# frosinastojanovska/image-captioning

Hardware: AMD Instinct MI355X
Metric: captions/sec (train step) on 1024px x 32RoI x 15tok synth (higher is better)
Workload: dtype f32 (split-bf16x3 products, fp32 accumulate: 73 of 85 conv layers on the bf16 pipe, the rest and the decoder exact fp32 MFMA); 1 GPU; BASELINE configs[2] (configs[3] at 8 GPUs): frozen ResNet-101+FPN fwd + PyramidROIAlign + RoI head + v2-inject decoder fwd/bwd + AMSGrad, 1024x1024 synth images, 32 RoI/img, 15-token captions, V=10000; backbone=resnet101, images_per_gpu=2, global_batch_images=2, parallelism=dp1, stage4_blocks=22, pipeline=encoder(i+1) || decoder(i), 2 HIP streams, rccl_ranks=1

## Files before the change

### image-captioning_amd/_lib.py

```python
import ctypes as C
import os

_HERE = os.path.dirname(os.path.abspath(__file__))
LIB_PATH = os.path.join(_HERE, "csrc", "libdcap_hip.so")

c_float_p = C.POINTER(C.c_float)
c_int32_p = C.POINTER(C.c_int32)
c_uint8_p = C.POINTER(C.c_uint8)


class GemmDesc(C.Structure):
    _fields_ = [("M", C.c_int), ("N", C.c_int), ("K", C.c_int),
                ("A", C.c_void_p), ("lda", C.c_int), ("a_trans", C.c_int),
                ("a_gather", C.c_void_p),
                ("B", C.c_void_p), ("ldb", C.c_int), ("b_trans", C.c_int),
                ("C", C.c_void_p), ("ldc", C.c_int),
                ("scale", C.c_void_p), ("shift", C.c_void_p),
                ("residual", C.c_void_p), ("ldr", C.c_int), ("res_rows", C.c_int),
                ("relu", C.c_int), ("accumulate", C.c_int), ("split_k", C.c_int)]


class GemmBf16Desc(C.Structure):
    _fields_ = [("M", C.c_int), ("N", C.c_int), ("K", C.c_int),
                ("A", C.c_void_p), ("lda", C.c_int), ("a_trans", C.c_int),
                ("a_gather", C.c_void_p), ("a_gather_rows", C.c_int),
                ("B", C.c_void_p), ("ldb", C.c_int), ("b_trans", C.c_int),
                ("C", C.c_void_p), ("ldc", C.c_int),
                ("Cb", C.c_void_p), ("ldcb", C.c_int),
                ("scale", C.c_void_p), ("shift", C.c_void_p),
                ("residual", C.c_void_p), ("ldr", C.c_int), ("res_rows", C.c_int),
                ("relu", C.c_int), ("accumulate", C.c_int), ("split_k", C.c_int)]


class ConvDesc(C.Structure):
    _fields_ = [("N", C.c_int), ("H", C.c_int), ("W", C.c_int), ("Cin", C.c_int),
                ("Cout", C.c_int), ("kh", C.c_int), ("kw", C.c_int), ("stride", C.c_int),
                ("pad_t", C.c_int), ("pad_l", C.c_int), ("Ho", C.c_int), ("Wo", C.c_int),
                ("x", C.c_void_p), ("w", C.c_void_p), ("y", C.c_void_p),
                ("scale", C.c_void_p), ("shift", C.c_void_p),
                ("residual", C.c_void_p), ("res_mode", C.c_int),
                ("relu", C.c_int), ("split_k", C.c_int), ("accumulate", C.c_int), ("math", C.c_int), ("w_wino", C.c_void_p), ("w_wino_b3", C.c_void_p)]


class ConvWgradBf16Desc(C.Structure):
    _fields_ = [("N", C.c_int), ("H", C.c_int), ("W", C.c_int), ("Cin", C.c_int),
                ("Cout", C.c_int), ("kh", C.c_int), ("kw", C.c_int), ("stride", C.c_int),
                ("pad_t", C.c_int), ("pad_l", C.c_int), ("Ho", C.c_int), ("Wo", C.c_int),
                ("x", C.c_void_p), ("dy", C.c_void_p), ("dw", C.c_void_p), ("accumulate", C.c_int), ("split_k", C.c_int)]


class ConvBf16Desc(C.Structure):
    _fields_ = [("N", C.c_int), ("H", C.c_int), ("W", C.c_int), ("Cin", C.c_int),
                ("Cout", C.c_int), ("kh", C.c_int), ("kw", C.c_int), ("stride", C.c_int),
                ("pad_t", C.c_int), ("pad_l", C.c_int), ("Ho", C.c_int), ("Wo", C.c_int),
                ("x", C.c_void_p), ("w", C.c_void_p), ("y", C.c_void_p), ("y_bf16", C.c_void_p),
                ("scale", C.c_void_p), ("shift", C.c_void_p), ("residual", C.c_void_p), ("res_mode", C.c_int),
                ("relu", C.c_int), ("split_k", C.c_int), ("tile", C.c_int)]


MATH_F32, MATH_BF16X3, MATH_BF16X2, MATH_BF16 = 0, 1, 2, 3


class RoiAlignDesc(C.Structure):
    _fields_ = [("B", C.c_int), ("R", C.c_int), ("C", C.c_int), ("pool", C.c_int),
                ("maps", C.c_void_p * 4), ("Hs", C.c_int * 4), ("Ws", C.c_int * 4),
                ("boxes", C.c_void_p), ("image_area", C.c_float),
                ("out", C.c_void_p), ("levels_out", C.c_void_p)]


class LstmFwdDesc(C.Structure):
    _fields_ = [("B", C.c_int), ("T", C.c_int), ("U", C.c_int),
                ("z", C.c_void_p), ("U_rec", C.c_void_p), ("mask", C.c_void_p),
                ("h_seq", C.c_void_p), ("c_seq", C.c_void_p), ("rec_masks", C.c_void_p)]


class LstmBwdDesc(C.Structure):
    _fields_ = [("B", C.c_int), ("T", C.c_int), ("U", C.c_int),
                ("z", C.c_void_p), ("U_rec", C.c_void_p), ("mask", C.c_void_p),
                ("h_seq", C.c_void_p), ("c_seq", C.c_void_p),
                ("dh_seq", C.c_void_p), ("dh_last", C.c_void_p),
                ("dz", C.c_void_p), ("dU_rec", C.c_void_p), ("accumulate_dU", C.c_int), ("rec_masks", C.c_void_p)]


class SoftmaxCeDesc(C.Structure):
    _fields_ = [("M", C.c_int), ("V", C.c_int), ("ld", C.c_int),
                ("logits", C.c_void_p), ("targets", C.c_void_p),
                ("probs", C.c_void_p), ("loss_rows", C.c_void_p), ("dlogits", C.c_void_p),
                ("grad_scale", C.c_float), ("row_weights", C.c_void_p), ("keras_sparse", C.c_int)]


class VocabCeDesc(C.Structure):
    _fields_ = [("M", C.c_int), ("V", C.c_int), ("K", C.c_int), ("bf16", C.c_int),
                ("X", C.c_void_p), ("ldx", C.c_int), ("W", C.c_void_p), ("ldw", C.c_int),
                ("bias", C.c_void_p), ("targets", C.c_void_p), ("row_weights", C.c_void_p),
                ("grad_scale", C.c_float), ("keras_sparse", C.c_int), ("loss_rows", C.c_void_p),
                ("dlogits", C.c_void_p), ("lddl", C.c_int), ("dl_bf16", C.c_int), ("dbias", C.c_void_p), ("materialize_bf16", C.c_int)]


class VocabTop1Desc(C.Structure):
    _fields_ = [("M", C.c_int), ("V", C.c_int), ("K", C.c_int),
                ("X", C.c_void_p), ("ldx", C.c_int), ("W", C.c_void_p), ("ldw", C.c_int),
                ("bias", C.c_void_p), ("tokens", C.c_void_p),
                ("ids", C.c_void_p), ("ld_ids", C.c_int), ("probs", C.c_void_p), ("ld_probs", C.c_int), ("mask", C.c_void_p)]


class VocabTopkDesc(C.Structure):
    _fields_ = [("M", C.c_int), ("V", C.c_int), ("K", C.c_int), ("k", C.c_int),
                ("X", C.c_void_p), ("ldx", C.c_int), ("W", C.c_void_p), ("ldw", C.c_int),
                ("bias", C.c_void_p), ("ids", C.c_void_p), ("probs", C.c_void_p)]


class VocabTop1Bf16Desc(C.Structure):
    _fields_ = VocabTop1Desc._fields_ + [("tile", C.c_int)]


class VocabTopkBf16Desc(C.Structure):
    _fields_ = VocabTopkDesc._fields_ + [("tile", C.c_int)]


class BeamSelectDesc(C.Structure):
    _fields_ = [("R", C.c_int), ("k", C.c_int), ("nb", C.c_int), ("steps", C.c_int), ("j", C.c_int), ("log_score", C.c_int),
                ("cand_ids", C.c_void_p), ("cand_probs", C.c_void_p), ("scores_in", C.c_void_p), ("scores_out", C.c_void_p),
                ("parents", C.c_void_p), ("tokens_hist", C.c_void_p), ("tokens", C.c_void_p), ("mask", C.c_void_p),
                ("U", C.c_int), ("h_in", C.c_void_p), ("c_in", C.c_void_p), ("h_out", C.c_void_p), ("c_out", C.c_void_p)]


class LstmStepDesc(C.Structure):
    _fields_ = [("B", C.c_int), ("U", C.c_int),
                ("z", C.c_void_p), ("U_rec", C.c_void_p), ("U_packed", C.c_void_p),
                ("h_prev", C.c_void_p), ("c_prev", C.c_void_p), ("mask", C.c_void_p), ("h", C.c_void_p), ("c", C.c_void_p)]


class BnReluDesc(C.Structure):
    _fields_ = [("M", C.c_int), ("N", C.c_int), ("ld", C.c_int), ("acc", C.c_void_p),
                ("bias", C.c_void_p), ("gamma", C.c_void_p), ("beta", C.c_void_p), ("mean", C.c_void_p), ("var", C.c_void_p),
                ("eps", C.c_float), ("y", C.c_void_p), ("dy", C.c_void_p), ("dacc", C.c_void_p),
                ("dgamma", C.c_void_p), ("dbeta", C.c_void_p), ("dbias", C.c_void_p)]


class ProposalDesc(C.Structure):
    _fields_ = [("B", C.c_int), ("levels", C.c_int), ("anchors_per_loc", C.c_int),
                ("heads", C.c_void_p * 5), ("Hs", C.c_int * 5), ("Ws", C.c_int * 5), ("head_stride", C.c_int),
                ("anchors", C.c_void_p), ("A_total", C.c_int), ("std_dev", C.c_float * 4),
                ("image_h", C.c_float), ("image_w", C.c_float),
                ("pre_nms_limit", C.c_int), ("proposal_count", C.c_int), ("nms_threshold", C.c_float),
                ("proposals", C.c_void_p), ("scores_out", C.c_void_p), ("order_out", C.c_void_p), ("keep_out", C.c_void_p)]


class RpnLossDesc(C.Structure):
    _fields_ = [("levels", C.c_int), ("anchors_per_loc", C.c_int), ("head_stride", C.c_int),
                ("heads", C.c_void_p * 5), ("dheads", C.c_void_p * 5), ("Hs", C.c_int * 5), ("Ws", C.c_int * 5),
                ("n_sel", C.c_int), ("n_pos", C.c_int),
                ("sel_level", C.c_void_p), ("sel_index", C.c_void_p), ("sel_match", C.c_void_p),
                ("target_deltas", C.c_void_p), ("losses", C.c_void_p), ("counts_dev", C.c_void_p)]


class DetectionTargetsDesc(C.Structure):
    _fields_ = [("n_proposals", C.c_int), ("n_gt", C.c_int), ("n_rois", C.c_int), ("T", C.c_int),
                ("proposals", C.c_void_p), ("gt_boxes", C.c_void_p), ("gt_captions", C.c_void_p),
                ("max_positive", C.c_int), ("inv_ratio", C.c_float), ("shuffle", C.c_int),
                ("seed", C.c_uint32), ("offset", C.c_uint32), ("offset_dev", C.c_void_p),
                ("rois", C.c_void_p), ("captions", C.c_void_p), ("counts", C.c_void_p)]


class PwChainDesc(C.Structure):
    _fields_ = [("M", C.c_int), ("K1", C.c_int), ("N1", C.c_int), ("N2", C.c_int),
                ("x", C.c_void_p), ("w1", C.c_void_p), ("scale1", C.c_void_p), ("shift1", C.c_void_p), ("residual", C.c_void_p),
                ("relu1", C.c_int), ("y", C.c_void_p), ("w2", C.c_void_p), ("scale2", C.c_void_p), ("shift2", C.c_void_p),
                ("relu2", C.c_int), ("z", C.c_void_p), ("w1_b3", C.c_void_p), ("w2_b3", C.c_void_p)]


class RegSegments(C.Structure):
    _fields_ = [("start", C.c_void_p), ("coef", C.c_void_p), ("mask", C.c_void_p), ("nseg", C.c_int)]


class AmsgradDesc(C.Structure):
    _fields_ = [("n", C.c_size_t), ("p", C.c_void_p), ("g", C.c_void_p), ("m", C.c_void_p),
                ("v", C.c_void_p), ("vhat", C.c_void_p),
                ("lr_t", C.c_float), ("beta1", C.c_float), ("beta2", C.c_float), ("eps", C.c_float),
                ("grad_scale", C.c_float), ("gnorm_sq", C.c_void_p), ("clipnorm", C.c_float),
                ("p_bf16", C.c_void_p), ("n_bf16", C.c_size_t), ("lr_t_dev", C.c_void_p), ("reg", C.POINTER(RegSegments))]


SYMBOLS = {
    "dc_version": (C.c_int, []),
    "dc_last_error": (C.c_char_p, []),
    "dc_gemm_workspace_bytes": (C.c_size_t, [C.POINTER(GemmDesc)]),
    "dc_gemm_f32": (C.c_int, [C.POINTER(GemmDesc), C.c_void_p, C.c_size_t, C.c_void_p]),
    "dc_gemm_bf16_workspace_bytes": (C.c_size_t, [C.POINTER(GemmBf16Desc)]),
    "dc_gemm_bf16_tile": (C.c_int, [C.POINTER(GemmBf16Desc), C.POINTER(C.c_int)]),
    "dc_gemm_bf16": (C.c_int, [C.POINTER(GemmBf16Desc), C.c_void_p, C.c_size_t, C.c_void_p]),
    "dc_conv2d_wgrad_bf16_workspace_bytes": (C.c_size_t, [C.POINTER(ConvWgradBf16Desc)]),
    "dc_conv2d_wgrad_bf16_tile": (C.c_int, [C.POINTER(ConvWgradBf16Desc), C.POINTER(C.c_int)]),
    "dc_conv2d_wgrad_bf16": (C.c_int, [C.POINTER(ConvWgradBf16Desc), C.c_void_p, C.c_size_t, C.c_void_p]),
    "dc_conv2d_bf16_workspace_bytes": (C.c_size_t, [C.POINTER(ConvBf16Desc)]),
    "dc_conv2d_bf16_tile": (C.c_int, [C.POINTER(ConvBf16Desc), C.POINTER(C.c_int)]),
    "dc_conv2d_bf16": (C.c_int, [C.POINTER(ConvBf16Desc), C.c_void_p, C.c_size_t, C.c_void_p]),
    "dc_cast_f32_bf16": (C.c_int, [C.c_void_p, C.c_void_p, C.c_size_t, C.c_void_p]),
    "dc_cast_bf16_f32": (C.c_int, [C.c_void_p, C.c_void_p, C.c_size_t, C.c_void_p]),
    "dc_cast_f32_bf16_2d": (C.c_int, [C.c_void_p, C.c_int, C.c_void_p, C.c_int, C.c_int, C.c_int, C.c_int, C.c_void_p]),
    "dc_split_bf16x3_f32": (C.c_int, [C.c_void_p, C.c_void_p, C.c_size_t, C.c_void_p]),
    "dc_conv2d_workspace_bytes": (C.c_size_t, [C.POINTER(ConvDesc)]),
    "dc_conv2d_nhwc_f32": (C.c_int, [C.POINTER(ConvDesc), C.c_void_p, C.c_size_t, C.c_void_p]),
    "dc_conv2d_tile_config": (C.c_int, [C.POINTER(ConvDesc), C.POINTER(C.c_int), C.POINTER(C.c_int), C.POINTER(C.c_int)]),
    "dc_conv2d_is_pointwise": (C.c_int, [C.POINTER(ConvDesc)]),
    "dc_conv2d_winograd_weight_bytes": (C.c_size_t, [C.c_int, C.c_int]),
    "dc_conv2d_winograd_pack_f32": (C.c_int, [C.c_void_p, C.c_void_p, C.c_int, C.c_int, C.c_void_p]),
    "dc_pw_chain_supported": (C.c_int, [C.c_int, C.c_int, C.c_int]),
    "dc_pw_chain_pack_f32": (C.c_int, [C.c_void_p, C.c_void_p, C.c_int, C.c_int, C.c_void_p]),
    "dc_pw_chain_pack_b3": (C.c_int, [C.c_void_p, C.c_void_p, C.c_int, C.c_int, C.c_void_p]),
    "dc_pw_chain_f32": (C.c_int, [C.POINTER(PwChainDesc), C.c_void_p]),
    "dc_pw_chain_kernel_name": (C.c_int, [C.POINTER(PwChainDesc), C.c_char_p, C.c_size_t]),
    "dc_conv2d_winograd_b3_weight_bytes": (C.c_size_t, [C.c_int, C.c_int]),
    "dc_conv2d_winograd_pack_b3": (C.c_int, [C.c_void_p, C.c_void_p, C.c_int, C.c_int, C.c_void_p]),
    "dc_conv2d_kernel_name": (C.c_int, [C.POINTER(ConvDesc), C.c_char_p, C.c_size_t]),
    "dc_conv2d_wgrad_workspace_bytes": (C.c_size_t, [C.POINTER(ConvDesc)]),
    "dc_conv2d_wgrad_f32": (C.c_int, [C.POINTER(ConvDesc), C.c_void_p, C.c_size_t, C.c_void_p]),
    "dc_roi_align_pyramid_bwd_f32": (C.c_int, [C.POINTER(RoiAlignDesc), C.c_void_p]),
    "dc_downsample2x_sum_f32": (C.c_int, [C.c_void_p, C.c_void_p, C.c_int, C.c_int, C.c_int, C.c_int, C.c_int, C.c_void_p]),
    "dc_downsample2x_sum_dual_f32": (C.c_int, [C.c_void_p, C.c_void_p, C.c_void_p, C.c_int, C.c_int, C.c_int, C.c_int, C.c_int, C.c_void_p]),
    "dc_maxpool2x2s2_f32": (C.c_int, [C.c_void_p, C.c_void_p, C.c_int, C.c_int, C.c_int, C.c_int, C.c_void_p]),
    "dc_maxpool3x3s2_same_f32": (C.c_int, [C.c_void_p, C.c_void_p, C.c_int, C.c_int, C.c_int, C.c_int, C.c_void_p]),
    "dc_mold_image_padded_f32": (C.c_int, [C.c_void_p, C.c_void_p, C.c_int, C.c_int, C.c_int, C.c_int, C.c_float, C.c_float, C.c_float, C.c_void_p]),
    "dc_mold_image_rgbx_f32": (C.c_int, [C.c_void_p, C.c_void_p, C.c_int, C.c_int, C.c_int,
                                         C.c_float, C.c_float, C.c_float, C.c_void_p]),
    "dc_roi_align_pyramid_f32": (C.c_int, [C.POINTER(RoiAlignDesc), C.c_void_p]),
    "dc_subsample2_f32": (C.c_int, [C.c_void_p, C.c_void_p, C.c_int, C.c_int, C.c_int, C.c_int, C.c_void_p]),
    "dc_proposals_workspace_bytes": (C.c_size_t, [C.POINTER(ProposalDesc)]),
    "dc_proposals_f32": (C.c_int, [C.POINTER(ProposalDesc), C.c_void_p, C.c_size_t, C.c_void_p]),
    "dc_lstm_seq_workspace_bytes": (C.c_size_t, [C.c_int, C.c_int, C.c_int]),
    "dc_lstm_seq_fwd_f32": (C.c_int, [C.POINTER(LstmFwdDesc), C.c_void_p, C.c_size_t, C.c_void_p]),
    "dc_lstm_seq_bwd_f32": (C.c_int, [C.POINTER(LstmBwdDesc), C.c_void_p, C.c_size_t, C.c_void_p]),
    "dc_lstm_pack_urec_f32": (C.c_int, [C.c_void_p, C.c_int, C.c_void_p, C.c_void_p]),
    "dc_lstm_step_workspace_bytes": (C.c_size_t, [C.c_int, C.c_int]),
    "dc_lstm_step_f32": (C.c_int, [C.POINTER(LstmStepDesc), C.c_void_p, C.c_size_t, C.c_void_p]),
    "dc_softmax_ce_f32": (C.c_int, [C.POINTER(SoftmaxCeDesc), C.c_void_p]),
    "dc_vocab_ce_workspace_bytes": (C.c_size_t, [C.POINTER(VocabCeDesc)]),
    "dc_vocab_ce": (C.c_int, [C.POINTER(VocabCeDesc), C.c_void_p, C.c_size_t, C.c_void_p]),
    "dc_vocab_top1_workspace_bytes": (C.c_size_t, [C.c_int, C.c_int]),
    "dc_vocab_top1_f32": (C.c_int, [C.POINTER(VocabTop1Desc), C.c_void_p, C.c_size_t, C.c_void_p]),
    "dc_vocab_topk_workspace_bytes": (C.c_size_t, [C.c_int, C.c_int, C.c_int]),
    "dc_vocab_topk_f32": (C.c_int, [C.POINTER(VocabTopkDesc), C.c_void_p, C.c_size_t, C.c_void_p]),
    "dc_vocab_topk_bf16_tile": (C.c_int, [C.c_int, C.c_int, C.c_int]),
    "dc_vocab_top1_bf16_workspace_bytes": (C.c_size_t, [C.c_int, C.c_int, C.c_int, C.c_int]),
    "dc_vocab_topk_bf16_workspace_bytes": (C.c_size_t, [C.c_int, C.c_int, C.c_int, C.c_int, C.c_int]),
    "dc_vocab_top1_bf16": (C.c_int, [C.POINTER(VocabTop1Bf16Desc), C.c_void_p, C.c_size_t, C.c_void_p]),
    "dc_vocab_topk_bf16": (C.c_int, [C.POINTER(VocabTopkBf16Desc), C.c_void_p, C.c_size_t, C.c_void_p]),
    "dc_beam_select_f32": (C.c_int, [C.POINTER(BeamSelectDesc), C.c_void_p]),
    "dc_beam_backtrace": (C.c_int, [C.c_void_p, C.c_void_p, C.c_int, C.c_int, C.c_int, C.c_void_p, C.c_void_p]),
    "dc_argmax_rows_f32": (C.c_int, [C.c_void_p, C.c_int, C.c_int, C.c_int, C.c_void_p, C.c_void_p]),
    "dc_gather_rows_f32": (C.c_int, [C.c_void_p, C.c_int, C.c_void_p, C.c_void_p, C.c_int, C.c_int, C.c_int, C.c_void_p]),
    "dc_bn_relu_fwd_f32": (C.c_int, [C.POINTER(BnReluDesc), C.c_void_p]),
    "dc_bn_relu_bwd_f32": (C.c_int, [C.POINTER(BnReluDesc), C.c_void_p]),
    "dc_conv_weight_dgrad_pack_f32": (C.c_int, [C.c_void_p, C.c_void_p, C.c_int, C.c_int, C.c_int, C.c_int, C.c_void_p]),
    "dc_rpn_loss_grad_f32": (C.c_int, [C.POINTER(RpnLossDesc), C.c_void_p]),
    "dc_scatter2_add_f32": (C.c_int, [C.c_void_p, C.c_void_p, C.c_int, C.c_int, C.c_int, C.c_int, C.c_void_p]),
    "dc_detection_targets_f32": (C.c_int, [C.POINTER(DetectionTargetsDesc), C.c_void_p]),
    "dc_caption_tables_i32": (C.c_int, [C.c_void_p, C.c_int, C.c_int, C.c_void_p, C.c_void_p, C.c_void_p, C.c_void_p, C.c_void_p, C.c_void_p]),
    "dc_set_persistent_cus": (C.c_int, [C.c_int]),
    "dc_get_persistent_cus": (C.c_int, []),
    "dc_l2_reg_workspace_bytes": (C.c_size_t, [C.c_size_t]),
    "dc_l2_reg_f32": (C.c_int, [C.c_void_p, C.c_void_p, C.c_void_p, C.c_void_p, C.c_size_t, C.c_void_p, C.c_void_p, C.c_size_t, C.c_void_p]),
    "dc_axpy_f32": (C.c_int, [C.c_float, C.c_void_p, C.c_void_p, C.c_size_t, C.c_void_p]),
    "dc_relu_bwd_f32": (C.c_int, [C.c_void_p, C.c_void_p, C.c_void_p, C.c_int, C.c_int, C.c_int, C.c_void_p]),
    "dc_relu_bwd_dual_f32": (C.c_int, [C.c_void_p, C.c_void_p, C.c_void_p, C.c_void_p, C.c_size_t, C.c_void_p]),
    "dc_fold_time_f32": (C.c_int, [C.c_void_p, C.c_int, C.c_int, C.c_int, C.c_int, C.c_void_p, C.c_int, C.c_void_p]),
    "dc_colsum_workspace_bytes": (C.c_size_t, [C.c_int, C.c_int, C.c_int]),
    "dc_colsum_f32": (C.c_int, [C.c_void_p, C.c_int, C.c_int, C.c_int, C.c_void_p, C.c_int, C.c_void_p, C.c_size_t, C.c_void_p]),
    "dc_sumsq_workspace_bytes": (C.c_size_t, [C.c_size_t]),
    "dc_sumsq_f32": (C.c_int, [C.c_void_p, C.c_size_t, C.c_void_p, C.c_int, C.c_void_p, C.c_size_t, C.c_void_p]),
    "dc_mean_f32": (C.c_int, [C.c_void_p, C.c_size_t, C.c_void_p, C.c_void_p]),
    "dc_bn_fold_f32": (C.c_int, [C.c_void_p] * 5 + [C.c_float, C.c_void_p, C.c_void_p, C.c_int, C.c_void_p]),
    "dc_bn_bwd_f32": (C.c_int, [C.c_void_p] * 8 + [C.c_long, C.c_int, C.c_void_p]),
    "dc_mul_f32": (C.c_int, [C.c_void_p, C.c_void_p, C.c_void_p, C.c_size_t, C.c_void_p]),
    "dc_maxpool3x3s2_same_bwd_f32": (C.c_int, [C.c_void_p] * 4 + [C.c_int] * 4 + [C.c_void_p]),
    "dc_dropout_mask_f32": (C.c_int, [C.c_void_p, C.c_size_t, C.c_float, C.c_uint32, C.c_uint32, C.c_void_p, C.c_void_p]),
    "dc_amsgrad_step_f32": (C.c_int, [C.POINTER(AmsgradDesc), C.c_void_p]),
    "dc_zero_fill": (C.c_int, [C.c_void_p, C.c_size_t, C.c_void_p]),
    "dc_reg_sumsq_workspace_bytes": (C.c_size_t, [C.c_size_t]),
    "dc_reg_sumsq_f32": (C.c_int, [C.c_void_p, C.c_void_p, C.POINTER(RegSegments), C.c_size_t, C.c_void_p, C.c_void_p, C.c_void_p, C.c_size_t, C.c_void_p]),
}

ABI_VERSION = 600
_lib = None


class DcapError(RuntimeError):
    pass


def load():
    global _lib
    if _lib is not None:
        return _lib
    path = os.environ.get("DCAP_LIB", LIB_PATH)
    if not os.path.exists(path):
        raise DcapError("%s is missing: build it with `python __graft_entry__.py` "
                        "(hipcc --offload-arch=gfx950); there is no CPU fallback" % path)
    import torch
    lib = C.CDLL(path)
    for name, (res, args) in SYMBOLS.items():
        fn = getattr(lib, name)
        fn.restype = res
        fn.argtypes = args
    got = lib.dc_version()
    if got // 100 != ABI_VERSION // 100:
        raise DcapError("%s is ABI version %d, these bindings are for %d: rebuild it (python __graft_entry__.py)" % (path, got, ABI_VERSION))
    _lib = lib
    return lib


def check(rc, what):
    if rc != 0:
        msg = load().dc_last_error()
        raise DcapError("%s failed (code %d): %s" % (what, rc, msg.decode() if msg else ""))
```

### image-captioning_amd/csrc/conv_wino.hip

```cpp
#include "igemm_bf16s.h"
#include <algorithm>

namespace dcap {
namespace wino {

constexpr int NTHREADS = 256;

struct Args {
    const float* x;
    const f4* u;
    float* y;
    const float* scale;
    const float* shift;
    int N, H, W, Cin, Cout, relu;
    int gy, gx, groups;
    unsigned x_bytes, u_bytes;
};

__global__ void wino_pack_kernel(const float* __restrict__ w, float* __restrict__ u, int Cin, int Cout) {
    const long total = (long)Cin * Cout;
    const int NTG = Cout / 32, KC = Cin / 16;
    for (long idx = (long)blockIdx.x * blockDim.x + threadIdx.x; idx < total; idx += (long)gridDim.x * blockDim.x) {
        const int cin = (int)(idx % Cin), cout = (int)(idx / Cin);
        float g[3][3];
#pragma unroll
        for (int t = 0; t < 9; ++t) g[t / 3][t % 3] = w[((long)cout * 9 + t) * Cin + cin];
        float gg[4][3];
#pragma unroll
        for (int c = 0; c < 3; ++c) {
            gg[0][c] = g[0][c];
            gg[1][c] = 0.5f * (g[0][c] + g[1][c] + g[2][c]);
            gg[2][c] = 0.5f * (g[0][c] - g[1][c] + g[2][c]);
            gg[3][c] = g[2][c];
        }
        const int ntg = cout >> 5, i = cout & 31, kc = cin >> 4, kk = cin & 15, h = kk >> 3, j = (kk & 7) >> 2, e = kk & 3;
#pragma unroll
        for (int a = 0; a < 4; ++a) {
            const float r[4] = {gg[a][0], 0.5f * (gg[a][0] + gg[a][1] + gg[a][2]), 0.5f * (gg[a][0] - gg[a][1] + gg[a][2]), gg[a][2]};
#pragma unroll
            for (int b = 0; b < 4; ++b) {
                const int xi = 4 * a + b;
                u[((((long)(xi * NTG + ntg) * KC + kc) * 2 + j) * 64 + (h * 32 + i)) * 4 + e] = r[b];
            }
        }
    }
}

__global__ void wino_pack_b3_kernel(const float* __restrict__ w, unsigned short* __restrict__ u, int Cin, int Cout) {
    const long total = (long)Cin * Cout;
    const int NTG = Cout / 32, KC = Cin / 16;
    for (long idx = (long)blockIdx.x * blockDim.x + threadIdx.x; idx < total; idx += (long)gridDim.x * blockDim.x) {
        const int cin = (int)(idx % Cin), cout = (int)(idx / Cin);
        float g[3][3];
#pragma unroll
        for (int t = 0; t < 9; ++t) g[t / 3][t % 3] = w[((long)cout * 9 + t) * Cin + cin];
        float gg[4][3];
#pragma unroll
        for (int c = 0; c < 3; ++c) {
            gg[0][c] = g[0][c];
            gg[1][c] = 0.5f * (g[0][c] + g[1][c] + g[2][c]);
            gg[2][c] = 0.5f * (g[0][c] - g[1][c] + g[2][c]);
            gg[3][c] = g[2][c];
        }
        const int ntg = cout >> 5, i = cout & 31, kc = cin >> 4, kk = cin & 15, h = kk >> 3, jj = kk & 7;
#pragma unroll
        for (int a = 0; a < 4; ++a) {
            const float r[4] = {gg[a][0], 0.5f * (gg[a][0] + gg[a][1] + gg[a][2]), 0.5f * (gg[a][0] - gg[a][1] + gg[a][2]), gg[a][2]};
#pragma unroll
            for (int b = 0; b < 4; ++b) {
                const int xi = 4 * a + b;
                float x = r[b];
#pragma unroll
                for (int piece = 0; piece < 3; ++piece) {
                    const unsigned short pb = __builtin_bit_cast(unsigned short, (__bf16)x);
                    x -= __uint_as_float((unsigned)pb << 16);
                    u[((((long)(xi * NTG + ntg) * KC + kc) * 3 + piece) * 64 + (h * 32 + i)) * 8 + jj] = pb;
                }
            }
        }
    }
}

__device__ __forceinline__ unsigned img32_addr(int xi, int tile, int chunk) {
    return (unsigned)((((xi * 32 + tile) << 3) + (chunk ^ ((tile >> 1) & 7))) << 4);
}
__device__ __forceinline__ void bt_cols(const f4 (&t)[4], f4 (&v)[4]) {
    v[0] = t[0] - t[2];
    v[1] = t[1] + t[2];
    v[2] = t[2] - t[1];
    v[3] = t[1] - t[3];
}

namespace wp {
constexpr int PW = 18, NDMA = 6;
__device__ __forceinline__ int patch_index(int y, int x) { return y * PW + (x >> 1) + (PW / 2) * (x & 1); }
__device__ __forceinline__ int patch_swizzle(int y, int x) { return ((x >> 2) & 1) | (((y >> 1) & 3) << 1); }
template <int HALVES>
struct Cfg {
    static constexpr int NT = 256 * HALVES, TGY = 4 * HALVES, TGX = 8, PH = 2 * TGY + 2, NPIX = PH * PW, SLOTS = NPIX * 8;
    static constexpr int BUF = 32768 * HALVES;
    static constexpr int LDS_BYTES = 2 * BUF;
    static_assert(NDMA * NT >= SLOTS && NDMA * NT * 16 <= BUF, "patch buffer; the kernel issues the pieces three per step");
};
}

typedef unsigned u32x4 __attribute__((ext_vector_type(4)));

__device__ __forceinline__ void split8(const f4& va, const f4& vb, u32x4& p0, u32x4& p1, u32x4& p2) {
    unsigned a0, a1, a2, b0, b1, b2, c0, c1, c2, d0, d1, d2;
    split_pair(va[0], va[1], a0, a1, a2);
    split_pair(va[2], va[3], b0, b1, b2);
    split_pair(vb[0], vb[1], c0, c1, c2);
    split_pair(vb[2], vb[3], d0, d1, d2);
    p0 = u32x4{a0, b0, c0, d0};
    p1 = u32x4{a1, b1, c1, d1};
    p2 = u32x4{a2, b2, c2, d2};
}
__device__ __forceinline__ f32x16 mfma_b(const u32x4& a, const u32x4& b, const f32x16& c) {
    return __builtin_amdgcn_mfma_f32_32x32x16_bf16(__builtin_bit_cast(bf16x8, a), __builtin_bit_cast(bf16x8, b), c, 0, 0, 0);
}

template <int HALVES, bool B3, int NCH = 1>
__device__ __forceinline__ void wino_body(const Args& a) {
    static_assert(NCH == 1 || (NCH == 2 && HALVES == 1 && B3), "64-channel items: the split-bf16 32-tile kernel only");
    using namespace wp;
    typedef Cfg<HALVES> C;
    constexpr int NT64 = C::NT, SLOTS = C::SLOTS, BUF = C::BUF;
    extern __shared__ __attribute__((aligned(16))) char smem[];
    const int tid = threadIdx.x, lane = tid & 63;
    const int wave = __builtin_amdgcn_readfirstlane(tid >> 6);
    const int wa = wave & 3, th = wave >> 2;
    const int gpi = a.gy * a.gx;
    const int NTG = a.Cout >> 5, KC = a.Cin >> 4, KP = a.Cin >> 5;
    const int total = a.groups * (NTG / NCH);
    const __amdgpu_buffer_rsrc_t rsrc = __builtin_amdgcn_make_buffer_rsrc(const_cast<float*>(a.x), 0, (int)a.x_bytes, 0x00020000);

    int nb, img, gyi, gxi;
    unsigned doff[NDMA];
    const f4* ubase;
    unsigned ubyte3;
    auto setup = [&](int item) {
        const int bid = xcd_remap(item, total);
        nb = bid / a.groups;
        const int g = bid - nb * a.groups;
        img = g / gpi;
        const int gr = g - img * gpi;
        gyi = gr / a.gx;
        gxi = gr - gyi * a.gx;
#pragma unroll
        for (int n = 0; n < NDMA; ++n) {
            const int s = n * NT64 + tid, pq = s >> 3, py = pq / PW, rem = pq - py * PW;
            const int px = rem < PW / 2 ? 2 * rem : 2 * (rem - PW / 2) + 1;
            const int iy = gyi * 2 * C::TGY - 1 + py, ix = gxi * 2 * C::TGX - 1 + px;
            const bool in = s < SLOTS && (unsigned)iy < (unsigned)a.H && (unsigned)ix < (unsigned)a.W;
            const int c8 = (s & 7) ^ patch_swizzle(py, px);
            doff[n] = in ? (unsigned)(((((long)img * a.H + iy) * a.W + ix) * a.Cin + 4 * c8) * 4) : kOobOffset;
        }
        ubase = a.u + lane + (((long)(4 * wa) * NTG + nb) * KC << 7);
        ubyte3 = (unsigned)((4 * wa) * NTG + NCH * nb) * (unsigned)KC * 3072u;
    };
    auto issue_dma_pieces = [&](int pair, int buf, int n0, int n1) {
#pragma unroll
        for (int n = n0; n < n1; ++n)
            __builtin_amdgcn_raw_ptr_buffer_load_lds(rsrc, (__attribute__((address_space(3))) void*)(smem + buf * BUF + (n * NT64 + wave * 64) * 16), 16,
                                                     (int)doff[n], pair * 128, 0, 0);
    };
    auto issue_dma = [&](int pair, int buf) { issue_dma_pieces(pair, buf, 0, NDMA); };
    const long ustep = (long)NTG * KC << 7;
    auto load_u_part = [&](f4 (&dst)[4][2], int kc, int b0, int b1) {
#pragma unroll
        for (int b = b0; b < b1; ++b) {
            const f4* p = ubase + b * ustep + ((long)kc << 7);
            dst[b][0] = p[0];
            dst[b][1] = p[64];
        }
    };
    auto load_u = [&](f4 (&dst)[4][2], int kc) { load_u_part(dst, kc, 0, 4); };
    const __amdgpu_buffer_rsrc_t rsrc_u = __builtin_amdgcn_make_buffer_rsrc(const_cast<f4*>(a.u), 0, (int)a.u_bytes, 0x00020000);
    const unsigned ustep3 = (unsigned)NTG * KC * 3 * 1024u;
    auto load_u3 = [&](u32x4 (&dst)[3], int kc, int b, int hc) {
        const unsigned so = __builtin_amdgcn_readfirstlane(ubyte3 + (unsigned)b * ustep3 + (unsigned)(hc * KC + kc) * 3072u);
        dst[0] = __builtin_bit_cast(u32x4, buf_f4s(rsrc_u, (unsigned)lane * 16u, so));
        dst[1] = __builtin_bit_cast(u32x4, buf_f4s(rsrc_u, (unsigned)lane * 16u, so + 1024u));
        dst[2] = __builtin_bit_cast(u32x4, buf_f4s(rsrc_u, (unsigned)lane * 16u, so + 2048u));
    };

    const int fi = lane & 31, fh = lane >> 5;
    const int tile = 32 * th + fi, tyl = tile >> 3, txl = tile & 7;
    const int r1 = (wa == 0) ? 0 : (wa == 2 ? 2 : 1), r2 = (wa == 0 || wa == 1) ? 2 : (wa == 2 ? 1 : 3);
    const float sgn = (wa == 1) ? 1.f : -1.f;
    unsigned paddr[2][4];
#pragma unroll
    for (int rr = 0; rr < 2; ++rr)
#pragma unroll
        for (int c = 0; c < 4; ++c) {
            const int py = 2 * tyl + (rr ? r2 : r1), px = 2 * txl + c;
            paddr[rr][c] = (unsigned)(patch_index(py, px) * 128 + (((2 * fh) ^ patch_swizzle(py, px)) << 4));
        }
    auto read_d = [&](f4 (&d)[2][4], int st) {
        const unsigned k = (unsigned)(((st & 1) << 4) ^ ((st >> 1) << 6));
#pragma unroll
        for (int rr = 0; rr < 2; ++rr)
#pragma unroll
            for (int c = 0; c < 4; ++c) d[rr][c] = *reinterpret_cast<const f4*>(smem + (paddr[rr][c] ^ k));
    };
    auto transform = [&](const f4 (&d)[2][4], f4 (&v)[4]) {
        f4 t[4];
#pragma unroll
        for (int c = 0; c < 4; ++c) t[c] = d[1][c] * sgn + d[0][c];
        bt_cols(t, v);
    };

    int item = blockIdx.x;
    if (item >= total) return;
    setup(item);
    issue_dma(0, 0);
    f4 ub[2][4][2];
    u32x4 u3[4][3];
    u32x4 w0[2][2], w1[2], w2[2];
    auto load_piece = [&](u32x4& dst, int kc, int b, int hc, int piece) {
        const unsigned so = __builtin_amdgcn_readfirstlane(ubyte3 + (unsigned)b * ustep3 + (unsigned)(hc * KC + kc) * 3072u + (unsigned)piece * 1024u);
        dst = __builtin_bit_cast(u32x4, buf_f4s(rsrc_u, (unsigned)lane * 16u, so));
    };
    auto load_u3_first = [&]() {
        if constexpr (NCH == 2) {
#pragma unroll
            for (int hc = 0; hc < 2; ++hc) {
                load_piece(w0[0][hc], 0, 0, hc, 0);
                load_piece(w1[hc], 0, 0, hc, 1);
                load_piece(w2[hc], 0, 0, hc, 2);
                load_piece(w0[1][hc], 0, 1, hc, 0);
            }
        } else {
#pragma unroll
            for (int b = 0; b < 4; ++b) load_u3(u3[b], 0, b, 0);
        }
    };
    if constexpr (B3) {
        load_u3_first();
    } else {
        load_u(ub[0], 0);
    }
    for (;;) {
        f32x16 acc[NCH][4];
#pragma unroll
        for (int hc = 0; hc < NCH; ++hc)
#pragma unroll
            for (int b = 0; b < 4; ++b)
#pragma unroll
                for (int r = 0; r < 16; ++r) acc[hc][b][r] = 0.f;
        auto pair = [&](int p, auto more_c) {
            constexpr bool more = decltype(more_c)::value;
            asm volatile("s_waitcnt vmcnt(0)" ::: "memory");
            __syncthreads();
            if constexpr (B3 && NCH == 2) {
                f4 t0[4], t1[4];
                u32x4 V[2][3];
                auto fetch_col = [&](int hf, int c) {
                    const unsigned ka = (unsigned)(hf << 6), kb = ka ^ 16u;
                    const f4 a0 = *reinterpret_cast<const f4*>(smem + (paddr[0][c] ^ ka));
                    const f4 a1 = *reinterpret_cast<const f4*>(smem + (paddr[1][c] ^ ka));
                    const f4 b0 = *reinterpret_cast<const f4*>(smem + (paddr[0][c] ^ kb));
                    const f4 b1 = *reinterpret_cast<const f4*>(smem + (paddr[1][c] ^ kb));
                    t0[c] = a1 * sgn + a0;
                    t1[c] = b1 * sgn + b0;
                };
                auto prep = [&](u32x4 (&dst)[3], int b) {
                    const f4 va = b == 0 ? t0[0] - t0[2] : (b == 1 ? t0[1] + t0[2] : (b == 2 ? t0[2] - t0[1] : t0[1] - t0[3]));
                    const f4 vb = b == 0 ? t1[0] - t1[2] : (b == 1 ? t1[1] + t1[2] : (b == 2 ? t1[2] - t1[1] : t1[1] - t1[3]));
                    split8(va, vb, dst[0], dst[1], dst[2]);
                };
                fetch_col(0, 0);
                fetch_col(0, 2);
                prep(V[0], 0);
#pragma unroll
                for (int q = 0; q < 8; ++q) {
                    const int b = q & 3;
                    __builtin_amdgcn_sched_barrier(0);
                    if constexpr (more) if (q < NDMA) issue_dma_pieces(p + 1, (p + 1) & 1, q, q + 1);
                    const u32x4 (&vq)[3] = V[q & 1];
                    const int kc1 = min(2 * p + ((q + 1) >> 2), KC - 1), kc2 = min(2 * p + ((q + 2) >> 2), KC - 1);
#pragma unroll
                    for (int hc = 0; hc < 2; ++hc) acc[hc][b] = mfma_b(w0[q & 1][hc], vq[2], acc[hc][b]);
#pragma unroll
                    for (int hc = 0; hc < 2; ++hc) acc[hc][b] = mfma_b(w1[hc], vq[1], acc[hc][b]);
#pragma unroll
                    for (int hc = 0; hc < 2; ++hc) acc[hc][b] = mfma_b(w2[hc], vq[0], acc[hc][b]);
#pragma unroll
                    for (int hc = 0; hc < 2; ++hc) load_piece(w2[hc], kc1, (q + 1) & 3, hc, 2);
#pragma unroll
                    for (int hc = 0; hc < 2; ++hc) acc[hc][b] = mfma_b(w1[hc], vq[0], acc[hc][b]);
#pragma unroll
                    for (int hc = 0; hc < 2; ++hc) load_piece(w1[hc], kc1, (q + 1) & 3, hc, 1);
#pragma unroll
                    for (int hc = 0; hc < 2; ++hc) acc[hc][b] = mfma_b(w0[q & 1][hc], vq[1], acc[hc][b]);
#pragma unroll
                    for (int hc = 0; hc < 2; ++hc) acc[hc][b] = mfma_b(w0[q & 1][hc], vq[0], acc[hc][b]);
#pragma unroll
                    for (int hc = 0; hc < 2; ++hc) load_piece(w0[q & 1][hc], kc2, (q + 2) & 3, hc, 0);
                    if (q == 0) fetch_col(0, 1);
                    if (q == 1) { fetch_col(0, 3); fetch_col(1, 0); }
                    if (q == 2) fetch_col(1, 2);
                    if (q == 3) fetch_col(1, 1);
                    if (q == 4) fetch_col(1, 3);
                    if (q < 7) prep(V[(q + 1) & 1], (q + 1) & 3);
#pragma unroll
                    for (int m = 0; m < 12; ++m) {
                        __builtin_amdgcn_sched_group_barrier(0x008, 1, 0);
                        __builtin_amdgcn_sched_group_barrier(0x020, 1, 0);
                        __builtin_amdgcn_sched_group_barrier(0x002, 6, 0);
                    }
                    __builtin_amdgcn_sched_barrier(0);
                }
#pragma unroll
                for (int rr = 0; rr < 2; ++rr)
#pragma unroll
                    for (int c = 0; c < 4; ++c) paddr[rr][c] ^= (unsigned)BUF;
                return;
            } else if constexpr (B3) {
                f4 dA[2][4], dB[2][4], t0[4], t1[4];
                u32x4 V[2][3];
                auto make_t = [&]() {
#pragma unroll
                    for (int c = 0; c < 4; ++c) {
                        t0[c] = dA[1][c] * sgn + dA[0][c];
                        t1[c] = dB[1][c] * sgn + dB[0][c];
                    }
                };
                auto prep = [&](u32x4 (&dst)[3], int b) {
                    const f4 va = b == 0 ? t0[0] - t0[2] : (b == 1 ? t0[1] + t0[2] : (b == 2 ? t0[2] - t0[1] : t0[1] - t0[3]));
                    const f4 vb = b == 0 ? t1[0] - t1[2] : (b == 1 ? t1[1] + t1[2] : (b == 2 ? t1[2] - t1[1] : t1[1] - t1[3]));
                    split8(va, vb, dst[0], dst[1], dst[2]);
                };
                read_d(dA, 0);
                read_d(dB, 1);
                make_t();
                prep(V[0], 0);
#pragma unroll
                for (int q = 0; q < 8; ++q) {
                    const int half = q >> 2, b = q & 3;
                    if (q == 1) read_d(dA, 2);
                    if (q == 2) read_d(dB, 3);
                    __builtin_amdgcn_sched_barrier(0);
                    if constexpr (more) if (q < NDMA) issue_dma_pieces(p + 1, (p + 1) & 1, q, q + 1);
                    const u32x4 (&vq)[3] = V[q & 1];
                    acc[0][b] = mfma_b(u3[b][0], vq[2], acc[0][b]);
                    acc[0][b] = mfma_b(u3[b][1], vq[1], acc[0][b]);
                    acc[0][b] = mfma_b(u3[b][2], vq[0], acc[0][b]);
                    acc[0][b] = mfma_b(u3[b][1], vq[0], acc[0][b]);
                    acc[0][b] = mfma_b(u3[b][0], vq[1], acc[0][b]);
                    acc[0][b] = mfma_b(u3[b][0], vq[0], acc[0][b]);
                    if (q == 3) make_t();
                    if (q < 7) prep(V[(q + 1) & 1], (q + 1) & 3);
                    load_u3(u3[b], min(2 * p + half + 1, KC - 1), b, 0);
#pragma unroll
                    for (int m = 0; m < 6; ++m) {
                        __builtin_amdgcn_sched_group_barrier(0x008, 1, 0);
                        __builtin_amdgcn_sched_group_barrier(0x020, 1, 0);
                        if (q == 3) __builtin_amdgcn_sched_group_barrier(0x002, 15, 0);
                        else __builtin_amdgcn_sched_group_barrier(0x002, 9, 0);
                    }
                    __builtin_amdgcn_sched_barrier(0);
                }
#pragma unroll
                for (int rr = 0; rr < 2; ++rr)
#pragma unroll
                    for (int c = 0; c < 4; ++c) paddr[rr][c] ^= (unsigned)BUF;
                return;
            }
            f4 d[2][4], vcur[4], vnext[4];
            read_d(d, 0);
            transform(d, vcur);
#pragma unroll
            for (int st = 0; st < 4; ++st) {
                const int half = st >> 1, j = st & 1;
                if (st < 3) read_d(d, st + 1);
                __builtin_amdgcn_sched_barrier(0);
                if constexpr (more) if (st < 2) issue_dma_pieces(p + 1, (p + 1) & 1, 3 * st, 3 * st + 3);
                load_u_part(ub[half ^ 1], min(2 * p + half + 1, KC - 1), 2 * j, 2 * j + 2);
#pragma unroll
                for (int e = 0; e < 2; ++e)
#pragma unroll
                    for (int b = 0; b < 4; ++b) acc[0][b] = __builtin_amdgcn_mfma_f32_32x32x2f32(ub[half][b][j][e], vcur[b][e], acc[0][b], 0, 0, 0);
#pragma unroll
                for (int m = 0; m < 8; ++m) {
                    __builtin_amdgcn_sched_group_barrier(0x008, 1, 0);
                    __builtin_amdgcn_sched_group_barrier(0x020, 1, 0);
                }
                __builtin_amdgcn_sched_barrier(0);
                if (st < 3) transform(d, vnext);
#pragma unroll
                for (int e = 2; e < 4; ++e)
#pragma unroll
                    for (int b = 0; b < 4; ++b) acc[0][b] = __builtin_amdgcn_mfma_f32_32x32x2f32(ub[half][b][j][e], vcur[b][e], acc[0][b], 0, 0, 0);
                if (st < 3) {
#pragma unroll
                    for (int m = 0; m < 8; ++m) {
                        __builtin_amdgcn_sched_group_barrier(0x008, 1, 0);
                        __builtin_amdgcn_sched_group_barrier(0x002, 4, 0);
                    }
                }
                __builtin_amdgcn_sched_barrier(0);
                if (st < 3) {
#pragma unroll
                    for (int b = 0; b < 4; ++b) vcur[b] = vnext[b];
                }
            }
#pragma unroll
            for (int rr = 0; rr < 2; ++rr)
#pragma unroll
                for (int c = 0; c < 4; ++c) paddr[rr][c] ^= (unsigned)BUF;
        };
        for (int p = 0; p < KP - 1; ++p) pair(p, std::true_type{});
        pair(KP - 1, std::false_type{});
        if (KP & 1) {
#pragma unroll
            for (int rr = 0; rr < 2; ++rr)
#pragma unroll
                for (int c = 0; c < 4; ++c) paddr[rr][c] ^= (unsigned)BUF;
        }

        const int onb = nb, oimg = img, ogy = gyi, ogx = gxi;
        const int next = item + (int)gridDim.x;
        const int oq = tid & 7, ocout = onb * (32 * NCH) + 4 * oq;
        f4 sc[NCH], sh[NCH];
#pragma unroll
        for (int hc = 0; hc < NCH; ++hc) {
            sc[hc] = a.scale ? *reinterpret_cast<const f4*>(a.scale + ocout + 32 * hc) : (f4)(1.f);
            sh[hc] = a.shift ? *reinterpret_cast<const f4*>(a.shift + ocout + 32 * hc) : (f4)(0.f);
        }
        __syncthreads();
        if (next < total) {
            setup(next);
            issue_dma(0, 0);
            if constexpr (B3) {
                load_u3_first();
            } else {
                load_u(ub[0], 0);
            }
        }
#pragma unroll
        for (int hc = 0; hc < NCH; ++hc) {
            if (hc) __syncthreads();
            {
                const f32x16 s0 = acc[hc][0] + acc[hc][1] + acc[hc][2], s1 = acc[hc][1] - acc[hc][2] - acc[hc][3];
#pragma unroll
                for (int gq = 0; gq < 4; ++gq) {
                    const f4 m0 = {s0[4 * gq], s0[4 * gq + 1], s0[4 * gq + 2], s0[4 * gq + 3]};
                    const f4 m1 = {s1[4 * gq], s1[4 * gq + 1], s1[4 * gq + 2], s1[4 * gq + 3]};
                    *reinterpret_cast<f4*>(smem + BUF + th * 32768 + img32_addr(2 * wa, fi, 2 * gq + fh)) = m0;
                    *reinterpret_cast<f4*>(smem + BUF + th * 32768 + img32_addr(2 * wa + 1, fi, 2 * gq + fh)) = m1;
                }
            }
            __syncthreads();
            {
                const int oth = tid >> 8, ti = (tid >> 3) & 31;
                f4 sv[4][2];
#pragma unroll
                for (int r = 0; r < 4; ++r)
#pragma unroll
                    for (int qx = 0; qx < 2; ++qx) sv[r][qx] = *reinterpret_cast<const f4*>(smem + BUF + oth * 32768 + img32_addr(2 * r + qx, ti, oq));
                const int otile = 32 * oth + ti, ty = ogy * C::TGY + (otile >> 3), tx = ogx * C::TGX + (otile & 7), cout = ocout + 32 * hc;
#pragma unroll
                for (int qx = 0; qx < 2; ++qx) {
                    const f4 o[2] = {sv[0][qx] + sv[1][qx] + sv[2][qx], sv[1][qx] - sv[2][qx] - sv[3][qx]};
#pragma unroll
                    for (int pr = 0; pr < 2; ++pr) {
                        f4 val = o[pr] * sc[hc] + sh[hc];
                        if (a.relu) val = f4{fmaxf(val[0], 0.f), fmaxf(val[1], 0.f), fmaxf(val[2], 0.f), fmaxf(val[3], 0.f)};
                        if (2 * ty + pr < a.H && 2 * tx + qx < a.W)
                            *reinterpret_cast<f4*>(a.y + (((long)oimg * a.H + 2 * ty + pr) * a.W + 2 * tx + qx) * a.Cout + cout) = val;
                    }
                }
            }
        }
        if (next >= total) break;
        item = next;
    }
}

__global__ __launch_bounds__(512, 1) void wino64_kernel(Args a) { wino_body<2, false>(a); }
__global__ __launch_bounds__(256, 2) void wino32_kernel(Args a) { wino_body<1, false>(a); }
__global__ __launch_bounds__(512, 1) void wino64b_kernel(Args a) { wino_body<2, true>(a); }
template <int NCH>
__global__ __launch_bounds__(256, 2) void wino32b_kernel(Args a) { wino_body<1, true, NCH>(a); }
template __global__ void wino32b_kernel<1>(Args);
template __global__ void wino32b_kernel<2>(Args);

}

static bool wino_shape_ok(const dc_conv_desc* d, const void* u) {
    return u != nullptr && d->math == DC_MATH_F32 && d->kh == 3 && d->kw == 3 && d->stride == 1 && d->pad_t == 1 && d->pad_l == 1 &&
           d->Ho == d->H && d->Wo == d->W && d->Cin % 32 == 0 && d->Cout % 32 == 0 && d->res_mode == 0 && d->split_k <= 1 && aligned16(d->y) &&
           aligned16(u) && (!d->scale || aligned16(d->scale)) && (!d->shift || aligned16(d->shift)) &&
           (size_t)d->N * d->H * d->W * d->Cin * sizeof(float) < (1ull << 31);
}

static bool wino_b3(const dc_conv_desc* d) { return wino_shape_ok(d, d->w_wino_b3); }
bool conv_winograd_supported(const dc_conv_desc* d) { return wino_b3(d) || wino_shape_ok(d, d->w_wino); }
bool conv_winograd_split_bf16(const dc_conv_desc* d) { return wino_b3(d); }

static int wino_force() {
    static const int force = env_int("DCAP_WINO_TILES", 0);
    return force;
}

static std::atomic<int> g_persistent_cus{-1};
static int persistent_cus() {
    int v = g_persistent_cus.load(std::memory_order_relaxed);
    if (v < 0) {
        static const int env = env_int("DCAP_WINO_CUS", kNumCU);
        v = env;
    }
    v = std::max(8, std::min(v, kNumCU));
    return v / 8 * 8;
}

int conv_winograd_tiles(const dc_conv_desc* d) {
    const int force = wino_force();
    if (force == 32 || force == 64) return force;
    if (wino_b3(d)) return 32;
    const int th = (d->H + 1) / 2, tw = (d->W + 1) / 2;
    const long items64 = (long)d->N * ((th + 7) / 8) * ((tw + 7) / 8) * (d->Cout / 32);
    return items64 >= kNumCU ? 64 : 32;
}

static int wino_cout_force() {
    static const int force = env_int("DCAP_WINO_COUT", 0);
    return force;
}

static int conv_winograd_cout(const dc_conv_desc* d) {
    if (!wino_b3(d) || conv_winograd_tiles(d) != 32 || d->Cout % 64) return 32;
    const int force = wino_cout_force();
    if (force == 32 || force == 64) return force;
    const int th = (d->H + 1) / 2, tw = (d->W + 1) / 2;
    const long items = (long)d->N * ((th + 3) / 4) * ((tw + 7) / 8) * (d->Cout / 64);
    return items >= 2 * kNumCU ? 64 : 32;
}

int conv2d_winograd(const dc_conv_desc* d, hipStream_t s) {
    wino::Args a;
    a.x = d->x;
    const bool b3 = wino_b3(d);
    a.u = b3 ? reinterpret_cast<const f4*>(d->w_wino_b3) : reinterpret_cast<const f4*>(d->w_wino);
    a.y = d->y;
    a.scale = d->scale;
    a.shift = d->shift;
    a.N = d->N; a.H = d->H; a.W = d->W; a.Cin = d->Cin; a.Cout = d->Cout; a.relu = d->relu;
    const int th = (d->H + 1) / 2, tw = (d->W + 1) / 2;
    const size_t x_bytes = (size_t)d->N * d->H * d->W * d->Cin * sizeof(float);
    DC_REQUIRE(x_bytes < (1ull << 31), DC_EINVAL, "dc_conv2d (winograd): the input tensor has %zu bytes, the kernel addresses < 2 GiB", x_bytes);
    a.x_bytes = (unsigned)x_bytes;
    a.u_bytes = (unsigned)((size_t)16 * d->Cin * d->Cout * (b3 ? 6 : 4));
    const bool big = conv_winograd_tiles(d) == 64;
    a.gy = (th + (big ? 8 : 4) - 1) / (big ? 8 : 4);
    a.gx = (tw + 7) / 8;
    a.groups = d->N * a.gy * a.gx;
    const bool wide = b3 && !big && conv_winograd_cout(d) == 64;
    const long items = (long)a.groups * (d->Cout / (wide ? 64 : 32));
    DC_REQUIRE(items < (1l << 31), DC_EINVAL, "dc_conv2d (winograd): grid too large");
    const int per_cu = big ? 1 : 2;
    const long full = (long)per_cu * kNumCU;
    const long slots = items >= 8 * full ? per_cu * persistent_cus() : full;
    const unsigned grid = items >= slots ? (unsigned)slots : (unsigned)std::max<long>(8, items / 8 * 8);
    if (b3 && big) {
        DC_ENSURE_DYN_LDS(wino::wino64b_kernel, wino::wp::Cfg<2>::LDS_BYTES);
        hipLaunchKernelGGL(wino::wino64b_kernel, dim3(grid), dim3(wino::wp::Cfg<2>::NT), wino::wp::Cfg<2>::LDS_BYTES, s, a);
    } else if (wide) {
        DC_ENSURE_DYN_LDS((&wino::wino32b_kernel<2>), wino::wp::Cfg<1>::LDS_BYTES);
        hipLaunchKernelGGL((wino::wino32b_kernel<2>), dim3(grid), dim3(wino::wp::Cfg<1>::NT), wino::wp::Cfg<1>::LDS_BYTES, s, a);
    } else if (b3) {
        DC_ENSURE_DYN_LDS((&wino::wino32b_kernel<1>), wino::wp::Cfg<1>::LDS_BYTES);
        hipLaunchKernelGGL((wino::wino32b_kernel<1>), dim3(grid), dim3(wino::wp::Cfg<1>::NT), wino::wp::Cfg<1>::LDS_BYTES, s, a);
    } else if (big) {
        DC_ENSURE_DYN_LDS(wino::wino64_kernel, wino::wp::Cfg<2>::LDS_BYTES);
        hipLaunchKernelGGL(wino::wino64_kernel, dim3(grid), dim3(wino::wp::Cfg<2>::NT), wino::wp::Cfg<2>::LDS_BYTES, s, a);
    } else {
        DC_ENSURE_DYN_LDS(wino::wino32_kernel, wino::wp::Cfg<1>::LDS_BYTES);
        hipLaunchKernelGGL(wino::wino32_kernel, dim3(grid), dim3(wino::wp::Cfg<1>::NT), wino::wp::Cfg<1>::LDS_BYTES, s, a);
    }
    return check_launch("dc_conv2d (winograd)");
}

}

using namespace dcap;

extern "C" size_t dc_conv2d_winograd_weight_bytes(int Cin, int Cout) {
    if (Cin <= 0 || Cout <= 0 || Cin % 32 || Cout % 32) return 0;
    return (size_t)16 * Cin * Cout * sizeof(float);
}

extern "C" int dc_conv2d_winograd_pack_f32(const float* w, float* u, int Cin, int Cout, void* stream) {
    DC_REQUIRE(w && u, DC_EINVAL, "dc_conv2d_winograd_pack: null pointer");
    DC_REQUIRE(Cin > 0 && Cout > 0 && Cin % 32 == 0 && Cout % 32 == 0, DC_EINVAL, "dc_conv2d_winograd_pack: Cin and Cout must be multiples of 32");
    DC_REQUIRE(aligned16(u), DC_EALIGN, "dc_conv2d_winograd_pack: u must be 16-byte aligned");
    const long total = (long)Cin * Cout;
    const int blocks = (int)std::min<long>((total + 255) / 256, 4096);
    hipLaunchKernelGGL(wino::wino_pack_kernel, dim3(blocks), dim3(256), 0, static_cast<hipStream_t>(stream), w, u, Cin, Cout);
    return check_launch("dc_conv2d_winograd_pack_f32");
}

extern "C" size_t dc_conv2d_winograd_b3_weight_bytes(int Cin, int Cout) {
    if (Cin <= 0 || Cout <= 0 || Cin % 32 || Cout % 32) return 0;
    return (size_t)16 * Cin * Cout * 3 * sizeof(uint16_t);
}

extern "C" int dc_conv2d_winograd_pack_b3(const float* w, uint16_t* u, int Cin, int Cout, void* stream) {
    DC_REQUIRE(w && u, DC_EINVAL, "dc_conv2d_winograd_pack_b3: null pointer");
    DC_REQUIRE(Cin > 0 && Cout > 0 && Cin % 32 == 0 && Cout % 32 == 0, DC_EINVAL, "dc_conv2d_winograd_pack_b3: Cin and Cout must be multiples of 32");
    DC_REQUIRE(aligned16(u), DC_EALIGN, "dc_conv2d_winograd_pack_b3: u must be 16-byte aligned");
    const long total = (long)Cin * Cout;
    const int blocks = (int)std::min<long>((total + 255) / 256, 4096);
    hipLaunchKernelGGL(wino::wino_pack_b3_kernel, dim3(blocks), dim3(256), 0, static_cast<hipStream_t>(stream), w, u, Cin, Cout);
    return check_launch("dc_conv2d_winograd_pack_b3");
}

extern "C" int dc_set_persistent_cus(int n) {
    DC_REQUIRE(n == 0 || (n >= 8 && n <= kNumCU), DC_EINVAL, "dc_set_persistent_cus: 0 (default: DCAP_WINO_CUS or all 256) or 8..256, got %d", n);
    dcap::g_persistent_cus.store(n == 0 ? -1 : n, std::memory_order_relaxed);
    return DC_OK;
}

extern "C" int dc_get_persistent_cus(void) { return dcap::persistent_cus(); }
```

### image-captioning_amd/csrc/dcap_internal.h

```cpp
#pragma once
#include <hip/hip_runtime.h>
#include <stdint.h>
#include <stdio.h>
#include <stdarg.h>
#include <stdlib.h>
#include <atomic>
#include "../../include/dcap.h"

namespace dcap {

void set_error(const char* fmt, ...);

#define DC_ENSURE_DYN_LDS(fn, bytes)                                                                                                  \
    do {                                                                                                                              \
        static std::atomic<unsigned long long> dc_done_{0};                                                                           \
        int dc_dev_ = 0;                                                                                                              \
        (void)hipGetDevice(&dc_dev_);                                                                                                 \
        const unsigned long long dc_bit_ = 1ull << (dc_dev_ & 63);                                                                    \
        if (!(dc_done_.load(std::memory_order_acquire) & dc_bit_)) {                                                                  \
            (void)hipFuncSetAttribute(reinterpret_cast<const void*>(fn), hipFuncAttributeMaxDynamicSharedMemorySize, (bytes));        \
            dc_done_.fetch_or(dc_bit_, std::memory_order_release);                                                                    \
        }                                                                                                                             \
    } while (0)

inline int check_launch(const char* what) {
    hipError_t e = hipGetLastError();
    if (e != hipSuccess) {
        set_error("%s: %s", what, hipGetErrorString(e));
        return DC_ELAUNCH;
    }
    return DC_OK;
}

inline int env_int(const char* name, int dflt) {
    const char* e = getenv(name);
    return e ? atoi(e) : dflt;
}

inline bool aligned16(const void* p) { return (reinterpret_cast<uintptr_t>(p) & 15u) == 0; }

#define DC_REQUIRE(cond, code, ...)            \
    do {                                       \
        if (!(cond)) {                         \
            ::dcap::set_error(__VA_ARGS__);    \
            return (code);                     \
        }                                      \
    } while (0)

constexpr int kNumCU = 256;
constexpr int kNumXCD = 8;

__device__ __forceinline__ int xcd_remap(int bid, int nblk) {
    const int q = nblk / kNumXCD, r = nblk % kNumXCD, xcd = bid % kNumXCD;
    return (xcd < r ? xcd * (q + 1) : r * (q + 1) + (xcd - r) * q) + bid / kNumXCD;
}

static __global__ __launch_bounds__(256) void zero_fill_kernel(unsigned* __restrict__ p, size_t words) {
    for (size_t i = (size_t)blockIdx.x * 256 + threadIdx.x; i < words; i += (size_t)gridDim.x * 256) p[i] = 0u;
}
inline int zero_fill_async(void* p, size_t bytes, hipStream_t s) {
    if (bytes == 0) return DC_OK;
    if ((reinterpret_cast<uintptr_t>(p) & 3u) || (bytes & 3u)) {
        set_error("zero_fill: pointer and size must be multiples of 4");
        return DC_EALIGN;
    }
    const size_t words = bytes / 4;
    const int blocks = (int)((words + 1023) / 1024 < 2048 ? (words + 1023) / 1024 : 2048);
    hipLaunchKernelGGL(zero_fill_kernel, dim3(blocks > 0 ? blocks : 1), dim3(256), 0, s, static_cast<unsigned*>(p), words);
    return check_launch("zero_fill_kernel");
}

__device__ __forceinline__ unsigned philox2x32(unsigned c0, unsigned c1, unsigned key) {
#pragma unroll
    for (int r = 0; r < 10; ++r) {
        const unsigned long long p = (unsigned long long)0xD256D193u * c0;
        const unsigned hi = (unsigned)(p >> 32), lo = (unsigned)p;
        c0 = hi ^ key ^ c1;
        c1 = lo;
        key += 0x9E3779B9u;
    }
    return c0;
}

}
```

### image-captioning_amd/csrc/roialign.hip

```cpp
#include "dcap_internal.h"
#include <math.h>
#include <algorithm>

#pragma clang fp contract(off)
namespace dcap {
__device__ __forceinline__ float mul_rn(float a, float b) { return a * b; }
__device__ __forceinline__ float add_rn(float a, float b) { return a + b; }
__device__ __forceinline__ float sub_rn(float a, float b) { return a - b; }
__device__ __forceinline__ float div_rn(float a, float b) { return a / b; }
}

namespace dcap {

__device__ __forceinline__ int roi_level(float y1, float x1, float y2, float x2, float image_area) {
    const float h = sub_rn(y2, y1), w = sub_rn(x2, x1);
    const float ratio = div_rn(__fsqrt_rn(mul_rn(h, w)), div_rn(224.0f, __fsqrt_rn(image_area)));
    const float lvl = div_rn(logf(ratio), logf(2.0f));
    if (!(lvl > -100.f)) return 2;
    const int r = (int)rintf(lvl);
    return min(5, max(2, 4 + r));
}

__global__ __launch_bounds__(256) void roi_align_kernel(dc_roialign_desc d) {
    const int wave = (blockIdx.x * 256 + threadIdx.x) >> 6, lane = threadIdx.x & 63;
    const int bins = d.pool * d.pool;
    const int total = d.B * d.R * bins;
    if (wave >= total) return;
    const int box = wave / bins, bin = wave - box * bins;
    const int py = bin / d.pool, px = bin - py * d.pool;
    const float4 bx = reinterpret_cast<const float4*>(d.boxes)[box];
    const int lvl = roi_level(bx.x, bx.y, bx.z, bx.w, d.image_area);
    if (d.levels_out && bin == 0 && lane == 0) d.levels_out[box] = lvl;
    const int li = lvl - 2;
    const int H = d.Hs[li], W = d.Ws[li], C4 = d.C >> 2;
    const float* fm = d.maps[li] + (long)(box / d.R) * H * W * d.C;
    float4* out = reinterpret_cast<float4*>(d.out) + (long)wave * C4;

    const float hs = (d.pool > 1) ? div_rn(mul_rn(sub_rn(bx.z, bx.x), (float)(H - 1)), (float)(d.pool - 1)) : 0.f;
    const float ws = (d.pool > 1) ? div_rn(mul_rn(sub_rn(bx.w, bx.y), (float)(W - 1)), (float)(d.pool - 1)) : 0.f;
    const float in_y = (d.pool > 1) ? add_rn(mul_rn(bx.x, (float)(H - 1)), mul_rn((float)py, hs))
                                    : mul_rn(mul_rn(0.5f, add_rn(bx.x, bx.z)), (float)(H - 1));
    const float in_x = (d.pool > 1) ? add_rn(mul_rn(bx.y, (float)(W - 1)), mul_rn((float)px, ws))
                                    : mul_rn(mul_rn(0.5f, add_rn(bx.y, bx.w)), (float)(W - 1));
    const bool ok = (in_y >= 0.f) && (in_y <= (float)(H - 1)) && (in_x >= 0.f) && (in_x <= (float)(W - 1));
    if (!ok) {
        for (int c = lane; c < C4; c += 64) out[c] = make_float4(0.f, 0.f, 0.f, 0.f);
        return;
    }
    const int top = (int)floorf(in_y), bot = (int)ceilf(in_y), left = (int)floorf(in_x), right = (int)ceilf(in_x);
    const float ly = in_y - (float)top, lx = in_x - (float)left;
    const float4* tl = reinterpret_cast<const float4*>(fm + ((long)top * W + left) * d.C);
    const float4* tr = reinterpret_cast<const float4*>(fm + ((long)top * W + right) * d.C);
    const float4* bl = reinterpret_cast<const float4*>(fm + ((long)bot * W + left) * d.C);
    const float4* br = reinterpret_cast<const float4*>(fm + ((long)bot * W + right) * d.C);
    for (int c = lane; c < C4; c += 64) {
        const float4 a = tl[c], b = tr[c], e = bl[c], f = br[c];
        float4 o;
#define DC_LERP(k)                                  \
    {                                               \
        const float t = a.k + (b.k - a.k) * lx;     \
        const float u = e.k + (f.k - e.k) * lx;     \
        o.k = t + (u - t) * ly;                     \
    }
        DC_LERP(x) DC_LERP(y) DC_LERP(z) DC_LERP(w)
        out[c] = o;
    }
}

__device__ __forceinline__ float roi_sample(float lo, float hi, int p, int n, int pool) {
    if (pool > 1) {
        const float step = div_rn(mul_rn(sub_rn(hi, lo), (float)(n - 1)), (float)(pool - 1));
        return add_rn(mul_rn(lo, (float)(n - 1)), mul_rn((float)p, step));
    }
    return mul_rn(mul_rn(0.5f, add_rn(lo, hi)), (float)(n - 1));
}

constexpr int RA_MAX_POOL = 16;

__global__ __launch_bounds__(256) void roi_align_bwd_gather_kernel(dc_roialign_desc d, int li, long wave0) {
    const int lane = threadIdx.x & 63;
    const long wv = wave0 + (((long)blockIdx.x * 256 + threadIdx.x) >> 6);
    const int H = d.Hs[li], W = d.Ws[li];
    const long per_img = (long)H * W;
    if (wv >= (long)d.B * per_img) return;
    const int img = (int)(wv / per_img);
    const int pix = (int)(wv - (long)img * per_img);
    const int y = pix / W, x = pix - y * W;
    const float4* boxes = reinterpret_cast<const float4*>(d.boxes) + (long)img * d.R;
    const int bins = d.pool * d.pool;
    float4 acc[4];
    const int C4 = d.C >> 2, nchunk = (C4 + 63) >> 6;
#pragma unroll
    for (int k = 0; k < 4; ++k) acc[k] = make_float4(0.f, 0.f, 0.f, 0.f);
    bool any = false;
    for (int b0 = 0; b0 < d.R; b0 += 64) {
        const int bi = b0 + lane;
        bool hit = false;
        if (bi < d.R) {
            const float4 bx = boxes[bi];
            if (roi_level(bx.x, bx.y, bx.z, bx.w, d.image_area) - 2 == li) {
                const float ya = roi_sample(bx.x, bx.z, 0, H, d.pool), yb = roi_sample(bx.x, bx.z, d.pool - 1, H, d.pool);
                const float xa = roi_sample(bx.y, bx.w, 0, W, d.pool), xb = roi_sample(bx.y, bx.w, d.pool - 1, W, d.pool);
                hit = fminf(ya, yb) < (float)y + 1.f && fmaxf(ya, yb) > (float)y - 1.f && fminf(xa, xb) < (float)x + 1.f && fmaxf(xa, xb) > (float)x - 1.f;
            }
        }
        unsigned long long m = __ballot(hit);
        while (m) {
            const int j = __ffsll((long long)m) - 1;
            m &= m - 1;
            const int box = b0 + j;
            const float4 bx = boxes[box];
            float wys[RA_MAX_POOL], wxs[RA_MAX_POOL];
#pragma unroll 1
            for (int p = 0; p < d.pool; ++p) {
                const float iy = roi_sample(bx.x, bx.z, p, H, d.pool), ix = roi_sample(bx.y, bx.w, p, W, d.pool);
                float wy = 0.f, wx = 0.f;
                if (iy >= 0.f && iy <= (float)(H - 1)) {
                    const float ly = iy - floorf(iy);
                    if ((int)floorf(iy) == y) wy += 1.f - ly;
                    if ((int)ceilf(iy) == y) wy += ly;
                } else {
                    wy = -1.f;
                }
                if (ix >= 0.f && ix <= (float)(W - 1)) {
                    const float lx = ix - floorf(ix);
                    if ((int)floorf(ix) == x) wx += 1.f - lx;
                    if ((int)ceilf(ix) == x) wx += lx;
                } else {
                    wx = -1.f;
                }
                wys[p] = wy;
                wxs[p] = wx;
            }
            const float* go = d.out + ((long)(img * d.R + box) * bins) * d.C;
#pragma unroll 1
            for (int py = 0; py < d.pool; ++py) {
                if (!(wys[py] > 0.f)) continue;
#pragma unroll 1
                for (int px = 0; px < d.pool; ++px) {
                    if (!(wxs[px] > 0.f)) continue;
                    const float wgt = wys[py] * wxs[px];
                    const float4* row = reinterpret_cast<const float4*>(go + (long)(py * d.pool + px) * d.C);
#pragma unroll
                    for (int k = 0; k < 4; ++k)
                        if (k < nchunk && lane + 64 * k < C4) {
                            const float4 g = row[lane + 64 * k];
                            acc[k].x += g.x * wgt; acc[k].y += g.y * wgt; acc[k].z += g.z * wgt; acc[k].w += g.w * wgt;
                        }
                    any = true;
                }
            }
        }
    }
    if (!any) return;
    float4* dst = reinterpret_cast<float4*>(const_cast<float*>(d.maps[li]) + ((long)img * per_img + pix) * d.C);
#pragma unroll
    for (int k = 0; k < 4; ++k)
        if (k < nchunk && lane + 64 * k < C4) {
            float4 v = dst[lane + 64 * k];
            v.x += acc[k].x; v.y += acc[k].y; v.z += acc[k].z; v.w += acc[k].w;
            dst[lane + 64 * k] = v;
        }
}

}

using namespace dcap;

extern "C" int dc_roi_align_pyramid_bwd_f32(const dc_roialign_desc* d, void* stream) {
    DC_REQUIRE(d && d->boxes && d->out, DC_EINVAL, "dc_roi_align_pyramid_bwd: null pointer");
    DC_REQUIRE(d->B > 0 && d->R > 0 && d->pool > 0 && d->pool <= RA_MAX_POOL && d->C > 0 && (d->C & 3) == 0 && d->C <= 1024, DC_EINVAL,
               "dc_roi_align_pyramid_bwd: bad B/R/pool/C (pool <= 16, C a multiple of 4 and <= 1024)");
    for (int l = 0; l < 4; ++l) {
        DC_REQUIRE(d->maps[l] && d->Hs[l] > 0 && d->Ws[l] > 0, DC_EINVAL, "dc_roi_align_pyramid_bwd: bad map %d", l);
        DC_REQUIRE(aligned16(d->maps[l]), DC_EALIGN, "dc_roi_align_pyramid_bwd: gradient map %d not 16-byte aligned", l);
    }
    DC_REQUIRE(aligned16(d->boxes) && aligned16(d->out), DC_EALIGN, "dc_roi_align_pyramid_bwd: boxes / dout not 16-byte aligned");
    for (int l = 0; l < 4; ++l) {
        const long waves = (long)d->B * d->Hs[l] * d->Ws[l];
        for (long w0 = 0; w0 < waves; w0 += 4L * 0x40000000) {
            const long n = std::min(waves - w0, 4L * 0x40000000);
            hipLaunchKernelGGL(roi_align_bwd_gather_kernel, dim3((unsigned)((n + 3) / 4)), dim3(256), 0, static_cast<hipStream_t>(stream), *d, l, w0);
        }
        int rc = check_launch("roi_align_bwd_gather_kernel");
        if (rc) return rc;
    }
    return DC_OK;
}

extern "C" int dc_roi_align_pyramid_f32(const dc_roialign_desc* d, void* stream) {
    DC_REQUIRE(d && d->boxes && d->out, DC_EINVAL, "dc_roi_align_pyramid: null pointer");
    DC_REQUIRE(d->B > 0 && d->R > 0 && d->pool > 0 && d->C > 0 && (d->C & 3) == 0, DC_EINVAL, "dc_roi_align_pyramid: bad B/R/pool/C");
    for (int l = 0; l < 4; ++l) {
        DC_REQUIRE(d->maps[l] && d->Hs[l] > 0 && d->Ws[l] > 0, DC_EINVAL, "dc_roi_align_pyramid: bad feature map %d", l);
        DC_REQUIRE(aligned16(d->maps[l]), DC_EALIGN, "dc_roi_align_pyramid: feature map %d not 16-byte aligned", l);
    }
    DC_REQUIRE(aligned16(d->boxes) && aligned16(d->out), DC_EALIGN, "dc_roi_align_pyramid: boxes/out not 16-byte aligned");
    const long waves = (long)d->B * d->R * d->pool * d->pool;
    const int blocks = (int)((waves + 3) / 4);
    hipLaunchKernelGGL(roi_align_kernel, dim3(blocks), dim3(256), 0, static_cast<hipStream_t>(stream), *d);
    return check_launch("roi_align_kernel");
}
```

### image-captioning_amd/encoder.py

```python
import ctypes as C

import numpy as np
import torch

from . import _lib, ops, step_graph
from ._lib import ConvBf16Desc, ConvDesc, PwChainDesc, check
from .layers import ConvSpec, resnet_fpn_convs
from .packing import fold_bn, pack_conv_kernel, pack_stem_kernel


DEFAULT_CONV_MATH = "f32"


def conv_math_mode(math=None):
    import os
    name = math if math is not None else os.environ.get("DCAP_CONV_MATH", DEFAULT_CONV_MATH)
    try:
        return {"f32": _lib.MATH_F32, "bf16x3": _lib.MATH_BF16X3, "bf16x2": _lib.MATH_BF16X2, "bf16": _lib.MATH_BF16}[name]
    except KeyError:
        raise ValueError("conv math must be 'f32', 'bf16x3', 'bf16x2' or 'bf16', got %r" % (name,))


def conv_math_name(mode):
    return {_lib.MATH_F32: "f32", _lib.MATH_BF16X3: "bf16x3", _lib.MATH_BF16X2: "bf16x2", _lib.MATH_BF16: "bf16"}.get(mode, str(mode))


def fuse_rpn_head(weights, channels=None):
    k = np.concatenate([weights["rpn_class_raw/kernel"], weights["rpn_bbox_pred/kernel"]], axis=3).astype(np.float32)
    b = np.concatenate([weights["rpn_class_raw/bias"], weights["rpn_bbox_pred/bias"]]).astype(np.float32)
    pad = (channels or k.shape[3]) - k.shape[3]
    if pad < 0:
        raise ValueError("rpn head needs %d channels, got %d" % (k.shape[3], channels))
    if pad:
        k = np.concatenate([k, np.zeros(k.shape[:3] + (pad,), np.float32)], axis=3)
        b = np.concatenate([b, np.zeros(pad, np.float32)])
    return k, b


class EncoderPlan:
    feat_channels = 256
    fast_bf16 = False

    def __init__(self, weights, batch, height, width, device, stage4_blocks=22,
                 mean_pixel=(123.7, 116.8, 103.9), use_graph=True, rpn=None, external=None, math=None, external_bn=None, train_stages=(),
                 winograd=None, wino_products=None, pw_chain=None, layer_math=None):
        if height % 64 or width % 64:
            raise ValueError("Image size must be dividable by 2 at least 6 times (got %dx%d)" % (height, width))
        self.lib = _lib.load()
        self.math = conv_math_mode(math)
        import os
        self.fast_bf16 = self.math == _lib.MATH_BF16
        self.winograd = (os.environ.get("DCAP_WINOGRAD", "1") != "0") if winograd is None else bool(winograd)
        self.wino_products = wino_products or os.environ.get("DCAP_WINO_PRODUCTS", "b3")
        if self.wino_products not in ("b3", "f32"):
            raise ValueError("wino_products must be 'b3' or 'f32'")
        self.pw_chain = (os.environ.get("DCAP_PW_CHAIN", "1") != "0") if pw_chain is None else bool(pw_chain)
        self.layer_math = (os.environ.get("DCAP_LAYER_MATH", "1") != "0") if layer_math is None else bool(layer_math)
        self._wchain = {}
        self._wwino = {}
        self._twin = {}
        self._wb = {}
        self.B, self.H, self.W = batch, height, width
        self.device = torch.device(device)
        self.mean_pixel = [float(v) for v in mean_pixel]
        self.stage4_blocks = stage4_blocks
        self.use_graph = bool(use_graph)
        self._steps = {}
        self._specs = {s.name: s for s in resnet_fpn_convs(stage4_blocks)}
        self.rpn = rpn
        self._external = dict(external or {})
        self._external_bn = dict(external_bn or {})
        self.train_stages = tuple(sorted(train_stages))
        self.saved = {}
        for name, bnp in self._external_bn.items():
            n = bnp["gamma"].numel()
            sc, sh = torch.empty(n, dtype=torch.float32, device=self.device), torch.empty(n, dtype=torch.float32, device=self.device)
            kern = self._external[name][0]
            self._external[name] = (kern, sc, sh)
        if rpn is not None:
            a = len(rpn["ratios"])
            self.head_channels = hc = int(rpn.get("head_channels", 6 * a))
            self._specs["rpn_conv_shared"] = ConvSpec("rpn_conv_shared", None, 3, 256, 512, 1, "same")
            self._specs["rpn_head"] = ConvSpec("rpn_head", None, 1, 512, hc, 1, "valid")
            if "rpn_head" not in self._external:
                weights = dict(weights)
                weights["rpn_head/kernel"], weights["rpn_head/bias"] = fuse_rpn_head(weights, hc)
        self._w = {}
        self._upload(weights)
        self._build()

    def _upload(self, W):
        dev = self.device
        for s in self._specs.values():
            if s.name in self._external:
                self._w[s.name] = self._external[s.name]
                continue
            k = np.asarray(W[s.name + "/kernel"], np.float32)
            if tuple(k.shape) != (s.k, s.k, s.cin, s.cout):
                raise ValueError("%s/kernel has shape %s, expected %s" % (s.name, k.shape, (s.k, s.k, s.cin, s.cout)))
            packed = pack_stem_kernel(k) if s.name == "conv1" else pack_conv_kernel(k)
            bias = np.asarray(W[s.name + "/bias"], np.float32)
            if s.bn:
                scale, shift = fold_bn(W[s.bn + "/gamma"], W[s.bn + "/beta"], W[s.bn + "/moving_mean"],
                                       W[s.bn + "/moving_variance"], bias)
                sc = torch.tensor(scale, device=dev)
            else:
                sc, shift = None, bias
            self._w[s.name] = (torch.tensor(packed, device=dev), sc, torch.tensor(shift, device=dev))

    def _buf(self, h, w, c):
        t = torch.empty((self.B, h, w, c), dtype=torch.float32, device=self.device)
        self._bufs.append(t)
        return t

    def _bf(self, t):
        k = t.data_ptr()
        if k not in self._twin:
            self._twin[k] = torch.empty(tuple(t.shape), dtype=torch.bfloat16, device=self.device)
        return self._twin[k]

    def bf16_of(self, t):
        return self._twin.get(t.data_ptr()) if self.fast_bf16 else None

    def _conv_bf16(self, name, x, y, residual, res_mode, relu, f32, bf16):
        s = self._specs[name]
        wp, sc, sh = self._w[name]
        N, H, W, Cin = x.shape
        _, Ho, Wo, Cout = y.shape
        if x.data_ptr() not in self._twin:
            raise RuntimeError("%s: its input has no bf16 twin (the producing op must be built with bf16=True)" % name)
        if name not in self._wb:
            if name in self._external:
                self._wb[name] = torch.empty(tuple(wp.shape), dtype=torch.bfloat16, device=self.device)
                self._ops.append(("cast", wp, self._wb[name]))
            else:
                self._wb[name] = ops.to_bf16(wp)
        pad = (s.k - 1) // 2 if s.padding == "same" else (3 if s.padding == "pad3" else 0)
        d = ConvBf16Desc()
        d.N, d.H, d.W, d.Cin = N, H, W, Cin
        d.Cout, d.kh, d.kw, d.stride, d.pad_t, d.pad_l, d.Ho, d.Wo = Cout, s.k, s.k, s.stride, pad, pad, Ho, Wo
        d.x, d.w = self._twin[x.data_ptr()].data_ptr(), self._wb[name].data_ptr()
        d.y = y.data_ptr() if f32 else None
        d.y_bf16 = self._bf(y).data_ptr() if bf16 else None
        d.scale = None if sc is None else sc.data_ptr()
        d.shift = sh.data_ptr()
        d.residual = None if residual is None else residual.data_ptr()
        d.res_mode, d.relu, d.split_k = res_mode, int(relu), 0
        self._ws_bytes = max(self._ws_bytes, self.lib.dc_conv2d_bf16_workspace_bytes(C.byref(d)))
        self._ops.append(("bconv", d, name))
        self.flops += 2.0 * N * Ho * Wo * Cout * s.k * s.k * s.cin

    def _conv(self, name, x, y, residual=None, res_mode=0, relu=True, f32=True, bf16=False):
        s = self._specs[name]
        if self.fast_bf16 and s.cin % 64 == 0 and s.stride in (1, 2) and (s.padding != "same" or s.stride == 1):
            return self._conv_bf16(name, x, y, residual, res_mode, relu, f32, bf16)
        wp, sc, sh = self._w[name]
        N, H, W, Cin = x.shape
        _, Ho, Wo, Cout = y.shape
        d = ConvDesc()
        d.N, d.H, d.W, d.Cin = N, H, W, Cin
        if s.padding == "same":
            pad = (s.k - 1) // 2 if s.stride == 1 else None
            if pad is None:
                raise ValueError("strided SAME conv is not on this path")
        elif s.padding == "pad3":
            pad = 3
        else:
            pad = 0
        d.Cout, d.kh, d.kw, d.stride, d.pad_t, d.pad_l, d.Ho, d.Wo = Cout, s.k, s.k, s.stride, pad, pad, Ho, Wo
        d.x, d.w, d.y = x.data_ptr(), wp.data_ptr(), y.data_ptr()
        d.scale = None if sc is None else sc.data_ptr()
        d.shift = sh.data_ptr()
        d.residual = None if residual is None else residual.data_ptr()
        d.res_mode, d.relu, d.split_k, d.math = res_mode, int(relu), 0, self._layer_math(s, name)
        use_wino = (self.winograd and self.math in (_lib.MATH_F32, _lib.MATH_BF16X3, _lib.MATH_BF16X2) and s.k == 3 and s.stride == 1 and
                    s.padding == "same" and residual is None and name not in self._external and Cin % 32 == 0 and Cout % 32 == 0 and
                    wp.shape[1] == 9 * Cin)
        if use_wino:
            if name not in self._wwino:
                self._wwino[name] = (ops.winograd_pack_b3 if self.wino_products == "b3" else ops.winograd_pack)(wp, Cin, Cout)
            if self.wino_products == "b3":
                d.w_wino_b3 = self._wwino[name].data_ptr()
            else:
                d.w_wino = self._wwino[name].data_ptr()
            d.math = _lib.MATH_F32
        self._ws_bytes = max(self._ws_bytes, self.lib.dc_conv2d_workspace_bytes(C.byref(d)))
        self._ops.append(("conv", d, name))
        if self.fast_bf16 and bf16:
            self._ops.append(("cast", y, self._bf(y)))
        self.flops += 2.0 * N * Ho * Wo * Cout * s.k * s.k * s.cin

    def _layer_math(self, s, name):
        if self.math != _lib.MATH_F32 or not self.layer_math or name in self._external:
            return self.math
        if s.k == 7 and s.cin == 3:
            return _lib.MATH_BF16X3
        if s.k != 1:
            return self.math
        if s.stride == 2 and s.cout >= 512 and s.cout > s.cin:
            return _lib.MATH_BF16X3
        if s.stride == 1 and 128 <= s.cin <= 512 and s.cout >= 256:
            return _lib.MATH_BF16X3
        return self.math

    def _chain_ok(self, name_c, name_a, mid, cout, pixels):
        sc, sa = self._specs[name_c], self._specs[name_a]
        if cout >= 512 and pixels < 32 * 192:
            return False
        return (self.pw_chain and self.math == _lib.MATH_F32 and not self.fast_bf16 and sc.k == 1 and sa.k == 1 and sc.stride == 1 and sa.stride == 1
                and name_c not in self._external and name_a not in self._external and ops.pw_chain_supported(mid, cout, mid))

    def _chain(self, name_c, x, y, residual, name_a, z):
        (w1, sc1, sh1), (w2, sc2, sh2) = self._w[name_c], self._w[name_a]
        b3 = self.wino_products == "b3" and x.shape[3] >= 128
        for n, w in ((name_c, w1), (name_a, w2)):
            if n not in self._wchain:
                self._wchain[n] = (ops.pw_chain_pack_b3 if b3 else ops.pw_chain_pack)(w)
        N, H, W, K1 = x.shape
        d = PwChainDesc()
        d.M, d.K1, d.N1, d.N2 = N * H * W, K1, y.shape[3], z.shape[3]
        d.x, d.shift1, d.y = x.data_ptr(), sh1.data_ptr(), y.data_ptr()
        if b3:
            d.w1_b3, d.w2_b3 = self._wchain[name_c].data_ptr(), self._wchain[name_a].data_ptr()
        else:
            d.w1, d.w2 = self._wchain[name_c].data_ptr(), self._wchain[name_a].data_ptr()
        d.scale1 = None if sc1 is None else sc1.data_ptr()
        d.residual = None if residual is None else residual.data_ptr()
        d.shift2, d.z = sh2.data_ptr(), z.data_ptr()
        d.scale2 = None if sc2 is None else sc2.data_ptr()
        d.relu1 = d.relu2 = 1
        self._ops.append(("chain", d, name_c + "+" + name_a))
        self.flops += 2.0 * d.M * (d.K1 * d.N1 + d.N1 * d.N2)

    def _build(self):
        B, H, W = self.B, self.H, self.W
        self._ops, self._ws_bytes, self.flops, self._bufs = [], 0, 0.0, []
        self._twin, self._wb = {}, {}
        self.images = torch.empty((B, H, W, 3), dtype=torch.uint8, device=self.device)
        rgbx = torch.empty((B, H, W, 4), dtype=torch.float32, device=self.device)
        for name, bnp in self._external_bn.items():
            _, sc, sh = self._external[name]
            self._ops.append(("bnfold", bnp, sc, sh))
        self._ops.append(("mold", self.images, rgbx))
        c1 = self._buf(H // 2, W // 2, 64)
        self._conv("conv1", rgbx, c1)
        x = self._buf(H // 4, W // 4, 64)
        self._ops.append(("pool", c1, x))
        if self.fast_bf16:
            self._ops.append(("cast", x, self._bf(x)))
        self.saved[1] = dict(rgbx=rgbx, c1=c1, pooled=x)

        def stage(s, blocks, mid, cout, stride, x):
            h, w = x.shape[1] // stride, x.shape[2] // stride
            keep = s in self.train_stages
            if not keep:
                m1, m2, sc = self._buf(h, w, mid), self._buf(h, w, mid), self._buf(h, w, cout)
                pp = [self._buf(h, w, cout), self._buf(h, w, cout)]
            final = self._buf(h, w, cout)
            self.saved[s] = []
            pending = None
            for i, blk in enumerate(blocks):
                cn = "res%d%s_branch" % (s, blk)
                if keep:
                    m1, m2 = self._buf(h, w, mid), self._buf(h, w, mid)
                    sc = self._buf(h, w, cout) if i == 0 else None
                    out = final if i == len(blocks) - 1 else self._buf(h, w, cout)
                    self.saved[s].append(dict(name=cn, x=x, m1=m1, m2=m2, sc=sc, out=out, stride=stride if i == 0 else 1))
                else:
                    out = final if i == len(blocks) - 1 else pp[i & 1]
                if pending is not None:
                    self._chain(pending[0], pending[1], x, pending[2], cn + "2a", m1)
                    pending = None
                else:
                    self._conv(cn + "2a", x, m1, f32=keep, bf16=True)
                self._conv(cn + "2b", m1, m2, f32=keep, bf16=True)
                res = x
                if i == 0:
                    self._conv(cn + "1", x, sc, relu=False)
                    res = sc
                nxt = "res%d%s_branch2a" % (s, blocks[i + 1]) if i + 1 < len(blocks) else None
                if nxt is not None and not keep and self._chain_ok(cn + "2c", nxt, mid, cout, x.shape[0] * m2.shape[1] * m2.shape[2]):
                    pending = (cn + "2c", m2, res)
                else:
                    self._conv(cn + "2c", m2, out, residual=res, res_mode=1, bf16=True)
                x = out
            return x

        C2 = stage(2, "abc", 64, 256, 1, x)
        C3 = stage(3, "abcd", 128, 512, 2, C2)
        C4 = stage(4, ["a"] + [chr(98 + i) for i in range(self.stage4_blocks)], 256, 1024, 2, C3)
        C5 = stage(5, "abc", 512, 2048, 2, C4)
        self.C = (C2, C3, C4, C5)
        self._n_trunk = len(self._ops)
        self.pre = None
        t5, t4 = self._buf(H // 32, W // 32, 256), self._buf(H // 16, W // 16, 256)
        t3, t2 = self._buf(H // 8, W // 8, 256), self._buf(H // 4, W // 4, 256)
        self._conv("fpn_c5p5", C5, t5, relu=False, bf16=True)
        self._conv("fpn_c4p4", C4, t4, residual=t5, res_mode=2, relu=False, bf16=True)
        self._conv("fpn_c3p3", C3, t3, residual=t4, res_mode=2, relu=False, bf16=True)
        self._conv("fpn_c2p2", C2, t2, residual=t3, res_mode=2, relu=False, bf16=True)
        P2, P3 = self._buf(H // 4, W // 4, 256), self._buf(H // 8, W // 8, 256)
        P4, P5 = self._buf(H // 16, W // 16, 256), self._buf(H // 32, W // 32, 256)
        rp = self.rpn is not None
        self._conv("fpn_p2", t2, P2, relu=False, bf16=rp)
        self._conv("fpn_p3", t3, P3, relu=False, bf16=rp)
        self._conv("fpn_p4", t4, P4, relu=False, bf16=rp)
        self._conv("fpn_p5", t5, P5, relu=False, bf16=rp)
        self.P = (P2, P3, P4, P5)
        self.pre = (t2, t3, t4, t5)
        if self.rpn is not None:
            from .utils import generate_pyramid_anchors
            P6 = self._buf(H // 64, W // 64, 256)
            self._ops.append(("sub2", P5, P6))
            if self.fast_bf16:
                self._ops.append(("cast", P6, self._bf(P6)))
            self.P6 = P6
            self.rpn_heads, self.rpn_shared = [], []
            for p in (P2, P3, P4, P5, P6):
                sh = self._buf(p.shape[1], p.shape[2], 512)
                hd = self._buf(p.shape[1], p.shape[2], self.head_channels)
                self._conv("rpn_conv_shared", p, sh, bf16=True)
                self._conv("rpn_head", sh, hd, relu=False)
                self.rpn_heads.append(hd)
                self.rpn_shared.append(sh)
            shapes = [[-(-H // st), -(-W // st)] for st in self.rpn["strides"]]
            anchors = generate_pyramid_anchors(self.rpn["scales"], self.rpn["ratios"], shapes, self.rpn["strides"],
                                               self.rpn.get("anchor_stride", 1)).astype(np.float32)
            self.anchors = torch.tensor(anchors, device=self.device)
        self._bufs.append(rgbx)
        self._ws = torch.empty(max(self._ws_bytes, 16), dtype=torch.uint8, device=self.device)

    def _run_ops(self, lo=0, hi=None):
        lib = self.lib
        stream = C.c_void_p(torch.cuda.current_stream().cuda_stream)
        wsp, wsb = C.c_void_p(self._ws.data_ptr()), self._ws.numel()
        for op in self._ops[lo:hi]:
            kind = op[0]
            if kind == "conv":
                rc = lib.dc_conv2d_nhwc_f32(C.byref(op[1]), wsp, wsb, stream)
                if rc:
                    check(rc, "dc_conv2d_nhwc_f32(%s)" % op[2])
            elif kind == "chain":
                rc = lib.dc_pw_chain_f32(C.byref(op[1]), stream)
                if rc:
                    check(rc, "dc_pw_chain_f32(%s)" % op[2])
            elif kind == "bconv":
                rc = lib.dc_conv2d_bf16(C.byref(op[1]), wsp, wsb, stream)
                if rc:
                    check(rc, "dc_conv2d_bf16(%s)" % op[2])
            elif kind == "cast":
                ops.to_bf16(op[1], out=op[2])
            elif kind == "bnfold":
                b = op[1]
                ops.bn_fold(b["gamma"], b["beta"], b["bias"], b["mean"], b["var"], op[2], op[3])
            elif kind == "mold":
                ops.mold_image_rgbx(op[1], self.mean_pixel, out=op[2])
            elif kind == "sub2":
                ops.subsample2(op[1], out=op[2])
            else:
                ops.maxpool3x3s2_same(op[1], out=op[2])

    def conv_table(self):
        rows = []
        for op in self._ops:
            if op[0] == "chain":
                d, buf = op[1], C.create_string_buffer(64)
                check(self.lib.dc_pw_chain_kernel_name(C.byref(d), buf, 64), "dc_pw_chain_kernel_name")
                rows.append((op[2], 2.0 * d.M * (d.K1 * d.N1 + d.N1 * d.N2), 32, d.N1, 1, buf.value.decode()))
                continue
            if op[0] != "conv":
                continue
            d, bm, bn, sk = op[1], C.c_int(), C.c_int(), C.c_int()
            check(self.lib.dc_conv2d_tile_config(C.byref(d), C.byref(bm), C.byref(bn), C.byref(sk)), "dc_conv2d_tile_config")
            buf = C.create_string_buffer(128)
            check(self.lib.dc_conv2d_kernel_name(C.byref(d), buf, 128), "dc_conv2d_kernel_name")
            s = self._specs[op[2]]
            rows.append((op[2], 2.0 * d.N * d.Ho * d.Wo * d.Cout * s.k * s.k * s.cin, bm.value, bn.value, sk.value, buf.value.decode()))
        return rows

    def conv_algorithmic_bytes(self):
        out = {}
        for op in self._ops:
            if op[0] == "chain":
                d = op[1]
                out[op[2]] = 4.0 * (d.M * (d.K1 + (2 if d.residual else 1) * d.N1 + d.N2) + d.K1 * d.N1 + d.N1 * d.N2)
                continue
            if op[0] != "conv":
                continue
            d, s = op[1], self._specs[op[2]]
            wbytes = ((16 * (6 if self.wino_products == "b3" else 4)) if op[2] in self._wwino else s.k * s.k * 4) * d.Cin * s.cout
            b = 4.0 * d.N * d.H * d.W * d.Cin + 4.0 * d.N * d.Ho * d.Wo * d.Cout + wbytes
            if d.res_mode == 1:
                b += 4.0 * d.N * d.Ho * d.Wo * d.Cout
            elif d.res_mode == 2:
                b += 1.0 * d.N * d.Ho * d.Wo * d.Cout
            out[op[2]] = b
        return out

    def time_convs(self, reps=3, beside=None):
        lib = self.lib
        stream = C.c_void_p(torch.cuda.current_stream().cuda_stream)
        wsp, wsb = C.c_void_p(self._ws.data_ptr()), self._ws.numel()
        convs = [op for op in self._ops if op[0] in ("conv", "chain")]
        acc = [0.0] * len(convs)
        for _ in range(reps):
            self._run_ops()
            torch.cuda.synchronize()
            if beside is not None:
                beside()
            evs = []
            for op in convs:
                e0, e1 = torch.cuda.Event(enable_timing=True), torch.cuda.Event(enable_timing=True)
                e0.record()
                rc = lib.dc_pw_chain_f32(C.byref(op[1]), stream) if op[0] == "chain" else lib.dc_conv2d_nhwc_f32(C.byref(op[1]), wsp, wsb, stream)
                e1.record()
                if rc:
                    check(rc, "dc_conv2d_nhwc_f32(%s)" % op[2])
                evs.append((e0, e1))
            torch.cuda.synchronize()
            for i, (e0, e1) in enumerate(evs):
                acc[i] += e0.elapsed_time(e1)
        return [(op[2], a / reps) for op, a in zip(convs, acc)]

    def time_bconvs(self, reps=3):
        lib = self.lib
        stream = C.c_void_p(torch.cuda.current_stream().cuda_stream)
        wsp, wsb = C.c_void_p(self._ws.data_ptr()), self._ws.numel()
        convs = [op for op in self._ops if op[0] == "bconv"]
        acc = [0.0] * len(convs)
        for _ in range(reps):
            self._run_ops()
            torch.cuda.synchronize()
            evs = []
            for op in convs:
                e0, e1 = torch.cuda.Event(enable_timing=True), torch.cuda.Event(enable_timing=True)
                e0.record()
                rc = lib.dc_conv2d_bf16(C.byref(op[1]), wsp, wsb, stream)
                e1.record()
                if rc:
                    check(rc, "dc_conv2d_bf16(%s)" % op[2])
                evs.append((e0, e1))
            torch.cuda.synchronize()
            for i, (e0, e1) in enumerate(evs):
                acc[i] += e0.elapsed_time(e1)
        rows = []
        for op, a in zip(convs, acc):
            d, sk = op[1], C.c_int(0)
            tile = int(lib.dc_conv2d_bf16_tile(C.byref(d), C.byref(sk)))
            rows.append((op[2], 2.0 * d.N * d.Ho * d.Wo * d.Cout * d.kh * d.kw * d.Cin, a / reps, tile, int(sk.value)))
        return rows

    def forward(self, images_u8=None):
        if images_u8 is not None:
            self.images.copy_(images_u8, non_blocking=bool(images_u8.is_cuda or images_u8.is_pinned()))
        self._run_part("all", self._run_ops)
        return self.P

    def _run_part(self, part, body):
        if not self.use_graph:
            body()
            return
        cs = self._steps.get(part)
        if cs is None:
            cs = self._steps[part] = step_graph.CapturedStep()
        cs.run(body, warm_calls=1, propagate=True)

    def forward_trunk(self, images_u8=None):
        if self._external_bn:
            raise RuntimeError("forward_trunk: this plan folds trainable BatchNorm layers inside the backbone pass; use forward()")
        if images_u8 is not None:
            self.images.copy_(images_u8, non_blocking=bool(images_u8.is_cuda or images_u8.is_pinned()))
        self._run_part("trunk", lambda: self._run_ops(0, self._n_trunk))
        return self.C

    def forward_top(self):
        self._run_part("top", lambda: self._run_ops(self._n_trunk, None))
        return self.P

    def proposals(self, debug=False):
        if self.rpn is None:
            raise RuntimeError("this plan was built without the RPN")
        r = self.rpn
        return ops.rpn_proposals(self.rpn_heads, self.anchors, (self.H, self.W), r["proposal_count"], r["nms_threshold"],
                                 r.get("bbox_std", (0.1, 0.1, 0.2, 0.2)), anchors_per_loc=len(r["ratios"]), debug=debug,
                                 head_stride=self.head_channels)

    def normalize_boxes(self, rois_px):
        hw = np.array([self.H, self.W, self.H, self.W], np.float32)
        if isinstance(rois_px, torch.Tensor):
            rois_px = rois_px.detach().cpu().numpy()
        return torch.tensor(np.asarray(rois_px, np.float32) / hw, device=self.device).contiguous()

    def roi_features(self, rois_px=None, out=None, boxes_norm=None):
        boxes = boxes_norm if boxes_norm is not None else self.normalize_boxes(rois_px)
        return ops.roi_align_pyramid(list(self.P), boxes, float(self.H * self.W), 7, out=out)


class Vgg16Plan(EncoderPlan):
    feat_channels = 512

    def __init__(self, weights, batch, height, width, device, mean_pixel=(123.7, 116.8, 103.9), use_graph=True, math=None, winograd=None,
                 wino_products=None):
        from .layers import vgg16_convs
        import os
        if height % 16 or width % 16:
            raise ValueError("Image size must be dividable by 16 (got %dx%d)" % (height, width))
        self.lib = _lib.load()
        self.math = conv_math_mode(math)
        self.winograd = (os.environ.get("DCAP_WINOGRAD", "1") != "0") if winograd is None else bool(winograd)
        self.wino_products = wino_products or os.environ.get("DCAP_WINO_PRODUCTS", "b3")
        self._wwino = {}
        self.layer_math = False
        self.B, self.H, self.W = batch, height, width
        self.device = torch.device(device)
        self.mean_pixel = [float(v) for v in mean_pixel]
        self.use_graph = use_graph
        self._steps = {}
        self._specs = {s.name: s for s in vgg16_convs()}
        self.rpn = None
        self._external = {}
        self._w = {}
        self._upload(weights)
        self._build()

    def _upload(self, W):
        dev = self.device
        for s in self._specs.values():
            k = np.asarray(W[s.name + "/kernel"], np.float32)
            if tuple(k.shape) != (s.k, s.k, s.cin, s.cout):
                raise ValueError("%s/kernel has shape %s, expected %s" % (s.name, k.shape, (s.k, s.k, s.cin, s.cout)))
            if s.cin == 3:
                k = np.concatenate([k, np.zeros((s.k, s.k, 29, s.cout), np.float32)], axis=2)
            self._w[s.name] = (torch.tensor(pack_conv_kernel(k), device=dev), None,
                               torch.tensor(np.asarray(W[s.name + "/bias"], np.float32), device=dev))

    def _build(self):
        B, H, W = self.B, self.H, self.W
        self._ops, self._ws_bytes, self.flops, self._bufs = [], 0, 0.0, []
        self.images = torch.empty((B, H, W, 3), dtype=torch.uint8, device=self.device)
        x32 = torch.empty((B, H, W, 32), dtype=torch.float32, device=self.device)
        self._bufs += [x32]
        self._ops.append(("mold32", self.images, x32))
        x, h, w = x32, H, W
        for b, (n, cout) in enumerate(((2, 64), (2, 128), (3, 256), (3, 512), (3, 512)), 1):
            for i in range(1, n + 1):
                y = self._buf(h, w, cout)
                self._conv("block%d_conv%d" % (b, i), x, y)
                x = y
            if b < 5:
                h, w = h // 2, w // 2
                y = self._buf(h, w, cout)
                self._ops.append(("pool2", x, y))
                x = y
        self.C = (x,)
        self.P = (x, x, x, x)
        self.pre = None
        self._ws = torch.empty(max(self._ws_bytes, 16), dtype=torch.uint8, device=self.device)

    def _run_ops(self):
        lib = self.lib
        stream = C.c_void_p(torch.cuda.current_stream().cuda_stream)
        wsp, wsb = C.c_void_p(self._ws.data_ptr()), self._ws.numel()
        for op in self._ops:
            kind = op[0]
            if kind == "conv":
                rc = lib.dc_conv2d_nhwc_f32(C.byref(op[1]), wsp, wsb, stream)
                if rc:
                    check(rc, "dc_conv2d_nhwc_f32(%s)" % op[2])
            elif kind == "mold32":
                ops.mold_image_padded(op[1], self.mean_pixel, out=op[2])
            else:
                ops.maxpool2x2s2(op[1], out=op[2])

    def roi_features(self, rois_px=None, out=None, boxes_norm=None):
        boxes = boxes_norm if boxes_norm is not None else self.normalize_boxes(rois_px)
        return ops.roi_align_pyramid(list(self.P), boxes, float(self.H * self.W), 7, out=out)
```

### image-captioning_amd/modified_dense_model.py

```python
import numpy as np
import torch

from . import utils
from .encoder import EncoderPlan
from .layers import resnet_fpn_convs


class BatchNorm(object):
    """Marker for the reference's BatchNorm(training=False) layer (modified_dense_model.py BatchNorm):
    frozen statistics are folded into the conv epilogue (packing.fold_bn); nothing to run."""


def compose_image_meta(image_id, image_shape, window):
    return utils.compose_image_meta(image_id, image_shape, window)


def mold_image(images, config):
    return utils.mold_image(images, config)


def load_weight_file(filepath):
    if filepath.endswith(".npz"):
        with np.load(filepath) as z:
            return {k: z[k] for k in z.files}
    if filepath.endswith(".h5") or filepath.endswith(".hdf5"):
        from .hdf5_lite import load_keras_weights
        return load_keras_weights(filepath)
    raise ValueError("unknown weight file type: %s" % filepath)


def save_weight_file(filepath, weights, layer_groups=None, group_member_order=None):
    if filepath.endswith(".h5") or filepath.endswith(".hdf5"):
        from .hdf5_lite import save_keras_weights
        save_keras_weights(filepath, weights, layer_groups=layer_groups, group_member_order=group_member_order)
    else:
        np.savez(filepath, **weights)


class DenseImageCapRCNN(object):
    def __init__(self, mode, config, model_dir, use_generated_rois=False, device=None, stage4_blocks=22, conv_math=None):
        assert mode in ['training', 'inference']
        if mode == 'training':
            raise NotImplementedError("the joint training graph (dense_img_cap/dense_model.py) is a SURVEY 8(f) 'next' row")
        self.mode = mode
        self.config = config
        self.model_dir = model_dir
        self.use_generated_rois = use_generated_rois
        self.stage4_blocks = stage4_blocks
        self.conv_math = conv_math
        self.device = torch.device(device if device is not None else "cuda:%d" % torch.cuda.current_device())
        self._weights = None
        self._plans = {}

    def weight_names(self):
        names = []
        for s in resnet_fpn_convs(self.stage4_blocks):
            names += [s.name + "/kernel", s.name + "/bias"]
            if s.bn:
                names += [s.bn + "/" + w for w in ("gamma", "beta", "moving_mean", "moving_variance")]
        if self.use_generated_rois:
            for n in ("rpn_conv_shared", "rpn_class_raw", "rpn_bbox_pred"):
                names += [n + "/kernel", n + "/bias"]
        return names

    def _rpn_config(self):
        if not self.use_generated_rois:
            return None
        c = self.config
        return dict(scales=c.RPN_ANCHOR_SCALES, ratios=c.RPN_ANCHOR_RATIOS, strides=c.BACKBONE_STRIDES,
                    anchor_stride=c.RPN_ANCHOR_STRIDE, bbox_std=[float(v) for v in c.RPN_BBOX_STD_DEV],
                    nms_threshold=c.RPN_NMS_THRESHOLD, proposal_count=c.POST_NMS_ROIS_INFERENCE)

    def set_weights(self, weights):
        missing = [n for n in self.weight_names() if n not in weights]
        if missing:
            raise KeyError("encoder weights missing: %s ..." % missing[:5])
        self._weights = {n: np.asarray(weights[n], np.float32) for n in self.weight_names()}
        self._plans = {}

    def load_weights(self, filepath, by_name=False, exclude=None):
        loaded = load_weight_file(filepath)
        cur = dict(self._weights or {})
        for k, v in loaded.items():
            if exclude and k.split("/")[0] in exclude:
                continue
            cur[k] = v
        self.set_weights(cur)

    def plan(self, batch, h, w):
        key = (batch, h, w)
        if key not in self._plans:
            if self._weights is None:
                raise RuntimeError("load_weights()/set_weights() must be called before inference")
            self._plans[key] = EncoderPlan(self._weights, batch, h, w, self.device, self.stage4_blocks,
                                           self.config.MEAN_PIXEL, rpn=self._rpn_config(), math=self.conv_math)
        return self._plans[key]

    def extract_features(self, images_u8, rois_px=None):
        imgs = torch.as_tensor(images_u8)
        B, H, W, _ = imgs.shape
        p = self.plan(B, H, W)
        p.forward(imgs)
        if self.use_generated_rois:
            self.last_proposals = p.proposals()
            return p.roi_features(boxes_norm=self.last_proposals)
        return p.roi_features(rois_px)

    def mold_inputs(self, images):
        molded, metas, windows = [], [], []
        for image in images:
            m, window, scale, padding = utils.resize_image(image, min_dim=self.config.IMAGE_MIN_DIM,
                                                           max_dim=self.config.IMAGE_MAX_DIM,
                                                           padding=self.config.IMAGE_PADDING)
            molded.append(m)
            metas.append(compose_image_meta(0, image.shape, window))
            windows.append(window)
        return np.stack(molded), np.stack(metas), np.stack(windows)

    def generate_captions(self, images, rois=None, verbose=0, device_features=False):
        assert self.mode == "inference", "Create model in inference mode."
        assert len(images) == self.config.BATCH_SIZE, "len(images) must be equal to BATCH_SIZE"
        molded, metas, windows = self.mold_inputs(images)
        rois = None if self.use_generated_rois else np.asarray(rois, np.float32)
        feats = self.extract_features(molded, rois)
        feats = feats.clone() if device_features else feats.cpu().numpy()
        n = self.config.POST_NMS_ROIS_INFERENCE
        results = [{"features": feats[i][:n]} for i in range(len(images))]
        if self.use_generated_rois:
            props = self.last_proposals.cpu().numpy()
            for i, r in enumerate(results):
                r["rois"] = props[i][:n]
        return results

    def train(self, *a, **k):
        raise NotImplementedError("joint training is a SURVEY 8(f) 'next' row")
```

### image-captioning_amd/ops.py

```python
import contextlib
import ctypes as C
import os

import numpy as np

import torch

from . import _lib
from ._lib import (PwChainDesc, ConvBf16Desc, AmsgradDesc, DetectionTargetsDesc, BnReluDesc, ConvDesc, ConvWgradBf16Desc, GemmBf16Desc, VocabCeDesc, ProposalDesc, RpnLossDesc, GemmDesc, LstmBwdDesc, LstmFwdDesc, RoiAlignDesc,
                   SoftmaxCeDesc, VocabTop1Desc, VocabTopkDesc, VocabTop1Bf16Desc, VocabTopkBf16Desc, BeamSelectDesc, LstmStepDesc, check)


def _stream():
    return C.c_void_p(torch.cuda.current_stream().cuda_stream)


def _ptr(t):
    return None if t is None else C.c_void_p(t.data_ptr())


def _chk(t, dtype=torch.float32, name="tensor"):
    if not t.is_cuda:
        raise _lib.DcapError("%s must live on the GPU (no CPU path exists)" % name)
    if t.dtype != dtype:
        raise _lib.DcapError("%s must be %s, got %s" % (name, dtype, t.dtype))
    if t.dim() > 0 and t.stride(-1) != 1:
        raise _lib.DcapError("%s must be contiguous along its last dimension" % name)
    return t


class no_gc_during_capture(object):

    def __enter__(self):
        import gc
        gc.collect()
        self._was = gc.isenabled()
        gc.disable()
        return self

    def __exit__(self, *exc):
        import gc
        if self._was:
            gc.enable()
        return False


class _Workspace:

    def __init__(self):
        self.buf = {}
        self.hi = {}
        self._seen = None

    def get(self, nbytes, device):
        if nbytes == 0:
            return None, 0
        device = torch.device(device)
        if device.index is None:
            device = torch.device("cuda", torch.cuda.current_device())
        key = (device, torch.cuda.current_stream(device).cuda_stream)
        hi = max(self.hi.get(device, 0), nbytes)
        self.hi[device] = hi
        b = self.buf.get(key)
        if b is None or b.numel() < nbytes:
            want = hi if torch.cuda.is_current_stream_capturing() else nbytes + nbytes // 4
            b = torch.empty(max(want, 1 << 20), dtype=torch.uint8, device=device)
            self.buf[key] = b
        if self._seen is not None:
            held = self._seen.setdefault(key, [])
            if not any(h is b for h in held):
                held.append(b)
        return b, b.numel()

    @contextlib.contextmanager
    def handed_out(self):
        self._seen = seen = {}
        try:
            yield seen
        finally:
            self._seen = None

    def release(self, stream):
        for key in [k for k in self.buf if k[1] == stream.cuda_stream]:
            del self.buf[key]


WORKSPACE = _Workspace()


def gemm(A, B, out=None, a_trans=False, b_trans=False, gather=None, scale=None, shift=None,
         residual=None, res_rows=0, relu=False, accumulate=False, split_k=0):
    lib = _lib.load()
    _chk(A, name="A"), _chk(B, name="B")
    if a_trans:
        K, M = (gather.numel() if gather is not None else A.shape[0]), A.shape[1]
    elif gather is not None:
        M, K = gather.numel(), A.shape[1]
    else:
        M, K = A.shape
    N = B.shape[0] if b_trans else B.shape[1]
    kb = B.shape[1] if b_trans else B.shape[0]
    if kb != K:
        raise _lib.DcapError("gemm: inner dimensions differ (%d vs %d)" % (K, kb))
    if out is None:
        out = torch.empty((M, N), dtype=torch.float32, device=A.device)
    _chk(out, name="out")
    if tuple(out.shape) != (M, N):
        raise _lib.DcapError("gemm: out has shape %s, expected %s" % (tuple(out.shape), (M, N)))
    d = GemmDesc()
    d.M, d.N, d.K = M, N, K
    d.A, d.lda, d.a_trans = A.data_ptr(), A.stride(0), int(a_trans)
    d.a_gather = None if gather is None else _chk(gather, torch.int32, "gather").data_ptr()
    d.B, d.ldb, d.b_trans = B.data_ptr(), B.stride(0), int(b_trans)
    d.C, d.ldc = out.data_ptr(), out.stride(0)
    d.scale = None if scale is None else _chk(scale, name="scale").data_ptr()
    d.shift = None if shift is None else _chk(shift, name="shift").data_ptr()
    if residual is not None:
        _chk(residual, name="residual")
        d.residual, d.ldr, d.res_rows = residual.data_ptr(), residual.stride(0), int(res_rows)
    d.relu, d.accumulate, d.split_k = int(relu), int(accumulate), int(split_k)
    ws, wsb = WORKSPACE.get(lib.dc_gemm_workspace_bytes(C.byref(d)), A.device)
    check(lib.dc_gemm_f32(C.byref(d), _ptr(ws), wsb, _stream()), "dc_gemm_f32")
    return out


BF16 = torch.bfloat16


def from_bf16(x, out):
    lib = _lib.load()
    if not (x.is_contiguous() and out.is_contiguous()) or x.numel() != out.numel():
        raise _lib.DcapError("from_bf16: contiguous tensors of one size")
    check(lib.dc_cast_bf16_f32(_ptr(_chk(x, BF16, "x")), _ptr(_chk(out, name="out")), x.numel(), _stream()), "dc_cast_bf16_f32")
    return out


def to_bf16(x, out=None, pad_cols=None):
    lib = _lib.load()
    _chk(x, name="x")
    if pad_cols is not None or (x.dim() == 2 and not x.is_contiguous()):
        rows, cols = x.shape
        co = cols if pad_cols is None else int(pad_cols)
        if out is None:
            out = torch.empty((rows, co), dtype=BF16, device=x.device)
        check(lib.dc_cast_f32_bf16_2d(_ptr(x), x.stride(0), _ptr(out), out.stride(0), rows, cols, co, _stream()), "dc_cast_f32_bf16_2d")
        return out
    if not x.is_contiguous():
        raise _lib.DcapError("to_bf16: x must be contiguous (or 2-D with unit column stride)")
    if out is None:
        out = torch.empty(x.shape, dtype=BF16, device=x.device)
    check(lib.dc_cast_f32_bf16(_ptr(x), _ptr(out), x.numel(), _stream()), "dc_cast_f32_bf16")
    return out


def gemm_bf16(A, B, out=None, out_bf16=None, a_trans=False, b_trans=False, gather=None, scale=None, shift=None,
              residual=None, res_rows=0, relu=False, accumulate=False, split_k=0, info=None):
    lib = _lib.load()
    _chk(A, BF16, "A"), _chk(B, BF16, "B")
    if a_trans:
        K, M = (gather.numel() if gather is not None else A.shape[0]), A.shape[1]
    elif gather is not None:
        M, K = gather.numel(), A.shape[1]
    else:
        M, K = A.shape
    N = B.shape[0] if b_trans else B.shape[1]
    kb = B.shape[1] if b_trans else B.shape[0]
    if kb != K:
        raise _lib.DcapError("gemm_bf16: inner dimensions differ (%d vs %d)" % (K, kb))
    if out is None and out_bf16 is None:
        out = torch.empty((M, N), dtype=torch.float32, device=A.device)
    d = GemmBf16Desc()
    d.M, d.N, d.K = M, N, K
    d.A, d.lda, d.a_trans = A.data_ptr(), A.stride(0), int(a_trans)
    if gather is not None:
        d.a_gather, d.a_gather_rows = _chk(gather, torch.int32, "gather").data_ptr(), A.shape[0]
    d.B, d.ldb, d.b_trans = B.data_ptr(), B.stride(0), int(b_trans)
    for t, name, dt in ((out, "out", torch.float32), (out_bf16, "out_bf16", BF16)):
        if t is not None and tuple(_chk(t, dt, name).shape) != (M, N):
            raise _lib.DcapError("gemm_bf16: %s has shape %s, expected %s" % (name, tuple(t.shape), (M, N)))
    if out is not None:
        d.C, d.ldc = out.data_ptr(), out.stride(0)
    if out_bf16 is not None:
        d.Cb, d.ldcb = out_bf16.data_ptr(), out_bf16.stride(0)
    d.scale = None if scale is None else _chk(scale, name="scale").data_ptr()
    d.shift = None if shift is None else _chk(shift, name="shift").data_ptr()
    if residual is not None:
        _chk(residual, name="residual")
        d.residual, d.ldr, d.res_rows = residual.data_ptr(), residual.stride(0), int(res_rows)
    d.relu, d.accumulate, d.split_k = int(relu), int(accumulate), int(split_k)
    if info is not None:
        sk = C.c_int(0)
        info["tile"] = int(lib.dc_gemm_bf16_tile(C.byref(d), C.byref(sk)))
        info["split_k"] = int(sk.value)
    ws, wsb = WORKSPACE.get(lib.dc_gemm_bf16_workspace_bytes(C.byref(d)), A.device)
    check(lib.dc_gemm_bf16(C.byref(d), _ptr(ws), wsb, _stream()), "dc_gemm_bf16")
    return out if out is not None else out_bf16


def conv2d(x, w_packed, kh, kw, stride, pad_t, pad_l, Ho, Wo, scale=None, shift=None, residual=None,
           res_mode=0, relu=False, out=None, split_k=0, math=0, w_wino=None, w_wino_b3=None, _name_only=False):
    lib = _lib.load()
    _chk(x, name="x"), _chk(w_packed, name="w")
    N, H, W, Cin = x.shape
    Cout = w_packed.shape[0]
    if not x.is_contiguous() or not w_packed.is_contiguous():
        raise _lib.DcapError("conv2d: x and w must be contiguous")
    if out is None:
        out = torch.empty((N, Ho, Wo, Cout), dtype=torch.float32, device=x.device)
    d = ConvDesc()
    d.N, d.H, d.W, d.Cin = N, H, W, Cin
    d.Cout, d.kh, d.kw, d.stride, d.pad_t, d.pad_l, d.Ho, d.Wo = Cout, kh, kw, stride, pad_t, pad_l, Ho, Wo
    d.x, d.w, d.y = x.data_ptr(), w_packed.data_ptr(), _chk(out, name="out").data_ptr()
    d.scale = None if scale is None else scale.data_ptr()
    d.shift = None if shift is None else shift.data_ptr()
    d.residual = None if residual is None else _chk(residual, name="residual").data_ptr()
    d.res_mode, d.relu, d.split_k, d.math = int(res_mode), int(relu), int(split_k), int(math)
    if w_wino is not None:
        if not w_wino.is_contiguous() or w_wino.numel() != 16 * Cin * Cout:
            raise _lib.DcapError("conv2d: w_wino must be the contiguous winograd_pack() of this layer's kernel (16*Cin*Cout floats)")
        d.w_wino = _chk(w_wino, name="w_wino").data_ptr()
    if w_wino_b3 is not None:
        if not w_wino_b3.is_contiguous() or w_wino_b3.numel() != 48 * Cin * Cout:
            raise _lib.DcapError("conv2d: w_wino_b3 must be the contiguous winograd_pack_b3() of this layer's kernel (48*Cin*Cout bf16)")
        d.w_wino_b3 = _chk(w_wino_b3, torch.int16, "w_wino_b3").data_ptr()
    if _name_only:
        buf = C.create_string_buffer(128)
        check(lib.dc_conv2d_kernel_name(C.byref(d), buf, 128), "dc_conv2d_kernel_name")
        return buf.value.decode()
    ws, wsb = WORKSPACE.get(lib.dc_conv2d_workspace_bytes(C.byref(d)), x.device)
    check(lib.dc_conv2d_nhwc_f32(C.byref(d), _ptr(ws), wsb, _stream()), "dc_conv2d_nhwc_f32")
    return out


def conv2d_kernel_name(*args, **kw):
    return conv2d(*args, _name_only=True, **kw)


def pw_chain_supported(k1, n1, n2):
    return bool(_lib.load().dc_pw_chain_supported(int(k1), int(n1), int(n2)))


def pw_chain_pack(w_packed, out=None):
    lib = _lib.load()
    _chk(w_packed, name="w")
    if w_packed.dim() != 2 or not w_packed.is_contiguous():
        raise _lib.DcapError("pw_chain_pack: w must be the contiguous packed 1x1 kernel [Cout, Cin]")
    if out is None:
        out = torch.empty_like(w_packed)
    check(lib.dc_pw_chain_pack_f32(_ptr(w_packed), _ptr(out), w_packed.shape[0], w_packed.shape[1], _stream()), "dc_pw_chain_pack_f32")
    return out


def pw_chain_pack_b3(w_packed, out=None):
    lib = _lib.load()
    _chk(w_packed, name="w")
    if w_packed.dim() != 2 or not w_packed.is_contiguous():
        raise _lib.DcapError("pw_chain_pack_b3: w must be the contiguous packed 1x1 kernel [Cout, Cin]")
    if out is None:
        out = torch.empty((w_packed.shape[0], 3 * w_packed.shape[1]), dtype=torch.int16, device=w_packed.device)
    check(lib.dc_pw_chain_pack_b3(_ptr(w_packed), _ptr(out), w_packed.shape[0], w_packed.shape[1], _stream()), "dc_pw_chain_pack_b3")
    return out


def pw_chain(x, w1f, shift1, w2f, shift2, scale1=None, scale2=None, residual=None, relu1=True, relu2=True, y=None, z=None):
    lib = _lib.load()
    K1 = x.shape[-1]
    M = x.numel() // K1
    N1, N2 = w1f.shape[0], w2f.shape[0]
    b3 = w1f.dtype == torch.int16
    if b3 != (w2f.dtype == torch.int16):
        raise _lib.DcapError("pw_chain: both kernels in the same form (pw_chain_pack or pw_chain_pack_b3)")
    if w1f.shape[1] != (3 if b3 else 1) * K1 or w2f.shape[1] != (3 if b3 else 1) * N1:
        raise _lib.DcapError("pw_chain: kernel shapes do not chain: x [.., %d], w1 %s, w2 %s" % (K1, tuple(w1f.shape), tuple(w2f.shape)))
    if y is None:
        y = torch.empty(tuple(x.shape[:-1]) + (N1,), dtype=torch.float32, device=x.device)
    if z is None:
        z = torch.empty(tuple(x.shape[:-1]) + (N2,), dtype=torch.float32, device=x.device)
    for t in (x, y, z) + (() if residual is None else (residual,)):
        if not t.is_contiguous():
            raise _lib.DcapError("pw_chain: tensors must be contiguous")
    d = PwChainDesc()
    d.M, d.K1, d.N1, d.N2 = M, K1, N1, N2
    d.x, d.shift1, d.y = _chk(x, name="x").data_ptr(), _chk(shift1, name="shift1").data_ptr(), _chk(y, name="y").data_ptr()
    d.shift2, d.z = _chk(shift2, name="shift2").data_ptr(), _chk(z, name="z").data_ptr()
    if b3:
        d.w1_b3, d.w2_b3 = _chk(w1f, torch.int16, "w1").data_ptr(), _chk(w2f, torch.int16, "w2").data_ptr()
    else:
        d.w1, d.w2 = _chk(w1f, name="w1").data_ptr(), _chk(w2f, name="w2").data_ptr()
    d.scale1 = None if scale1 is None else _chk(scale1, name="scale1").data_ptr()
    d.scale2 = None if scale2 is None else _chk(scale2, name="scale2").data_ptr()
    d.residual = None if residual is None else _chk(residual, name="residual").data_ptr()
    d.relu1, d.relu2 = int(relu1), int(relu2)
    check(lib.dc_pw_chain_f32(C.byref(d), _stream()), "dc_pw_chain_f32")
    return y, z


def winograd_pack_b3(w_packed, cin, cout, out=None):
    lib = _lib.load()
    _chk(w_packed, name="w")
    if not w_packed.is_contiguous() or w_packed.numel() != 9 * cin * cout:
        raise _lib.DcapError("winograd_pack_b3: w must be the contiguous packed 3x3 kernel [Cout, 9*Cin]")
    nbytes = lib.dc_conv2d_winograd_b3_weight_bytes(cin, cout)
    if nbytes == 0:
        raise _lib.DcapError("winograd_pack_b3: Cin and Cout must be multiples of 32")
    if out is None:
        out = torch.empty((nbytes // 2,), dtype=torch.int16, device=w_packed.device)
    check(lib.dc_conv2d_winograd_pack_b3(_ptr(w_packed), _ptr(out), cin, cout, _stream()), "dc_conv2d_winograd_pack_b3")
    return out


def winograd_pack(w_packed, cin, cout, out=None):
    lib = _lib.load()
    _chk(w_packed, name="w")
    if not w_packed.is_contiguous() or w_packed.numel() != 9 * cin * cout:
        raise _lib.DcapError("winograd_pack: w must be the contiguous packed 3x3 kernel [Cout, 9*Cin]")
    nbytes = lib.dc_conv2d_winograd_weight_bytes(cin, cout)
    if nbytes == 0:
        raise _lib.DcapError("winograd_pack: Cin and Cout must be multiples of 32")
    if out is None:
        out = torch.empty((nbytes // 4,), dtype=torch.float32, device=w_packed.device)
    check(lib.dc_conv2d_winograd_pack_f32(_ptr(w_packed), _ptr(out), cin, cout, _stream()), "dc_conv2d_winograd_pack_f32")
    return out


def split_bf16x3(x, out=None):
    lib = _lib.load()
    _chk(x, name="x")
    if not x.is_contiguous():
        raise _lib.DcapError("split_bf16x3: x must be contiguous")
    if out is None:
        out = torch.empty((3,) + tuple(x.shape), dtype=torch.int16, device=x.device)
    check(lib.dc_split_bf16x3_f32(_ptr(x), _ptr(out), x.numel(), _stream()), "dc_split_bf16x3_f32")
    return out


def conv2d_wgrad(x, dy, kh, kw, stride, pad_t, pad_l, out=None, split_k=0, accumulate=False):
    lib = _lib.load()
    _chk(x, name="x"), _chk(dy, name="dy")
    N, H, W, Cin = x.shape
    _, Ho, Wo, Cout = dy.shape
    if not x.is_contiguous() or not dy.is_contiguous():
        raise _lib.DcapError("conv2d_wgrad: x and dy must be contiguous")
    if out is None:
        out = torch.empty((Cout, kh * kw * Cin), dtype=torch.float32, device=x.device)
    d = ConvDesc()
    d.N, d.H, d.W, d.Cin = N, H, W, Cin
    d.Cout, d.kh, d.kw, d.stride, d.pad_t, d.pad_l, d.Ho, d.Wo = Cout, kh, kw, stride, pad_t, pad_l, Ho, Wo
    d.x, d.y, d.w, d.split_k = x.data_ptr(), dy.data_ptr(), _chk(out, name="dw").data_ptr(), int(split_k)
    d.accumulate = int(accumulate)
    ws, wsb = WORKSPACE.get(lib.dc_conv2d_wgrad_workspace_bytes(C.byref(d)), x.device)
    check(lib.dc_conv2d_wgrad_f32(C.byref(d), _ptr(ws), wsb, _stream()), "dc_conv2d_wgrad_f32")
    return out


def conv2d_wgrad_bf16(x, dy, kh, kw, stride, pad_t, pad_l, out=None, split_k=0, accumulate=False, info=None):
    lib = _lib.load()
    _chk(x, BF16, "x"), _chk(dy, BF16, "dy")
    N, H, W, Cin = x.shape
    _, Ho, Wo, Cout = dy.shape
    if not x.is_contiguous() or not dy.is_contiguous():
        raise _lib.DcapError("conv2d_wgrad_bf16: x and dy must be contiguous")
    if out is None:
        out = torch.empty((Cout, kh * kw * Cin), dtype=torch.float32, device=x.device)
    d = ConvWgradBf16Desc()
    d.N, d.H, d.W, d.Cin = N, H, W, Cin
    d.Cout, d.kh, d.kw, d.stride, d.pad_t, d.pad_l, d.Ho, d.Wo = Cout, kh, kw, stride, pad_t, pad_l, Ho, Wo
    d.x, d.dy, d.dw = x.data_ptr(), dy.data_ptr(), _chk(out, name="dw").data_ptr()
    d.accumulate, d.split_k = int(accumulate), int(split_k)
    if info is not None:
        sk = C.c_int(0)
        info["tile"] = int(lib.dc_conv2d_wgrad_bf16_tile(C.byref(d), C.byref(sk)))
        info["split_k"] = int(sk.value)
    ws, wsb = WORKSPACE.get(lib.dc_conv2d_wgrad_bf16_workspace_bytes(C.byref(d)), x.device)
    check(lib.dc_conv2d_wgrad_bf16(C.byref(d), _ptr(ws), wsb, _stream()), "dc_conv2d_wgrad_bf16")
    return out


def conv2d_bf16(x, w, kh, kw, stride, pad_t, pad_l, Ho, Wo, scale=None, shift=None, residual=None, res_mode=0, relu=False,
                out=None, out_bf16=None, want_f32=True, want_bf16=False, split_k=0, info=None, tile=0):
    lib = _lib.load()
    _chk(x, BF16, "x"), _chk(w, BF16, "w")
    N, H, W, Cin = x.shape
    Cout = w.shape[0]
    if not x.is_contiguous() or not w.is_contiguous() or w.shape[1] != kh * kw * Cin:
        raise _lib.DcapError("conv2d_bf16: x must be contiguous NHWC, w contiguous [Cout, kh*kw*Cin]")
    if out is None and want_f32:
        out = torch.empty((N, Ho, Wo, Cout), dtype=torch.float32, device=x.device)
    if out_bf16 is None and want_bf16:
        out_bf16 = torch.empty((N, Ho, Wo, Cout), dtype=BF16, device=x.device)
    d = ConvBf16Desc()
    d.N, d.H, d.W, d.Cin = N, H, W, Cin
    d.Cout, d.kh, d.kw, d.stride, d.pad_t, d.pad_l, d.Ho, d.Wo = Cout, kh, kw, stride, pad_t, pad_l, Ho, Wo
    d.x, d.w = x.data_ptr(), w.data_ptr()
    d.y = None if out is None else _chk(out, name="out").data_ptr()
    d.y_bf16 = None if out_bf16 is None else _chk(out_bf16, BF16, "out_bf16").data_ptr()
    d.scale = None if scale is None else _chk(scale, name="scale").data_ptr()
    d.shift = None if shift is None else _chk(shift, name="shift").data_ptr()
    d.residual = None if residual is None else _chk(residual, name="residual").data_ptr()
    d.res_mode, d.relu, d.split_k, d.tile = int(res_mode), int(relu), int(split_k), int(tile)
    if info is not None:
        sk = C.c_int(0)
        info["tile"] = int(lib.dc_conv2d_bf16_tile(C.byref(d), C.byref(sk)))
        info["split_k"] = int(sk.value)
    ws, wsb = WORKSPACE.get(lib.dc_conv2d_bf16_workspace_bytes(C.byref(d)), x.device)
    check(lib.dc_conv2d_bf16(C.byref(d), _ptr(ws), wsb, _stream()), "dc_conv2d_bf16")
    return out, out_bf16


def conv_bf16_supported(cin):
    return cin % 64 == 0


def wgrad_bf16_supported(x_shape, dy_shape):
    return x_shape[-1] % 128 == 0 and dy_shape[-1] % 8 == 0


def downsample2x_sum(fine, out=None, accumulate=False, out_bf16=None):
    lib = _lib.load()
    _chk(fine, name="fine")
    N, H, W, Cc = fine.shape
    if out is None:
        out = torch.empty((N, H // 2, W // 2, Cc), dtype=torch.float32, device=fine.device)
    check(lib.dc_downsample2x_sum_dual_f32(_ptr(fine), _ptr(out), None if out_bf16 is None else _ptr(_chk(out_bf16, BF16, "out_bf16")), N, H // 2, W // 2, Cc,
                                           int(accumulate), _stream()), "dc_downsample2x_sum_dual_f32")
    return out


def roi_align_pyramid_bwd(dmaps, boxes, image_area, dout, pool=7):
    lib = _lib.load()
    B, R, _ = boxes.shape
    d = RoiAlignDesc()
    d.B, d.R, d.C, d.pool = B, R, dmaps[0].shape[-1], pool
    for i, m in enumerate(dmaps):
        if not _chk(m, name="dmap").is_contiguous():
            raise _lib.DcapError("roi_align_bwd: gradient maps must be contiguous")
        d.maps[i] = m.data_ptr()
        d.Hs[i], d.Ws[i] = m.shape[1], m.shape[2]
    d.boxes, d.image_area = _chk(boxes, name="boxes").data_ptr(), float(image_area)
    d.out = _chk(dout, name="dout").data_ptr()
    check(lib.dc_roi_align_pyramid_bwd_f32(C.byref(d), _stream()), "dc_roi_align_pyramid_bwd_f32")
    return dmaps


def maxpool3x3s2_same(x, out=None):
    lib = _lib.load()
    _chk(x, name="x")
    N, H, W, Cc = x.shape
    if out is None:
        out = torch.empty((N, (H + 1) // 2, (W + 1) // 2, Cc), dtype=torch.float32, device=x.device)
    check(lib.dc_maxpool3x3s2_same_f32(_ptr(x), _ptr(out), N, H, W, Cc, _stream()), "dc_maxpool3x3s2_same_f32")
    return out


def maxpool2x2s2(x, out=None):
    lib = _lib.load()
    _chk(x, name="x")
    N, H, W, Cc = x.shape
    if out is None:
        out = torch.empty((N, H // 2, W // 2, Cc), dtype=torch.float32, device=x.device)
    check(lib.dc_maxpool2x2s2_f32(_ptr(x), _ptr(out), N, H, W, Cc, _stream()), "dc_maxpool2x2s2_f32")
    return out


def mold_image_rgbx(img_u8, mean_pixel, out=None):
    lib = _lib.load()
    _chk(img_u8, torch.uint8, "images")
    N, H, W, c = img_u8.shape
    if c != 3 or not img_u8.is_contiguous():
        raise _lib.DcapError("mold_image: images must be contiguous [N,H,W,3] uint8")
    if out is None:
        out = torch.empty((N, H, W, 4), dtype=torch.float32, device=img_u8.device)
    check(lib.dc_mold_image_rgbx_f32(_ptr(img_u8), _ptr(out), N, H, W, float(mean_pixel[0]), float(mean_pixel[1]),
                                     float(mean_pixel[2]), _stream()), "dc_mold_image_rgbx_f32")
    return out


def mold_image_padded(img_u8, mean_pixel, out):
    lib = _lib.load()
    _chk(img_u8, torch.uint8, "images"), _chk(out, name="out")
    N, H, W, c = img_u8.shape
    if c != 3 or not img_u8.is_contiguous() or not out.is_contiguous() or tuple(out.shape[:3]) != (N, H, W):
        raise _lib.DcapError("mold_image_padded: images contiguous [N,H,W,3] uint8, out contiguous [N,H,W,C]")
    check(lib.dc_mold_image_padded_f32(_ptr(img_u8), _ptr(out), N, H, W, out.shape[3], float(mean_pixel[0]), float(mean_pixel[1]),
                                       float(mean_pixel[2]), _stream()), "dc_mold_image_padded_f32")
    return out


def roi_align_pyramid(maps, boxes, image_area, pool=7, out=None, levels_out=None):
    lib = _lib.load()
    B, R, _ = boxes.shape
    Cc = maps[0].shape[-1]
    _chk(boxes, name="boxes")
    if not boxes.is_contiguous():
        raise _lib.DcapError("roi_align: boxes must be contiguous")
    if out is None:
        out = torch.empty((B, R, pool, pool, Cc), dtype=torch.float32, device=boxes.device)
    d = RoiAlignDesc()
    d.B, d.R, d.C, d.pool = B, R, Cc, pool
    for i, m in enumerate(maps):
        _chk(m, name="map")
        if not m.is_contiguous() or m.shape[0] != B or m.shape[-1] != Cc:
            raise _lib.DcapError("roi_align: feature maps must be contiguous [B,H,W,C]")
        d.maps[i] = m.data_ptr()
        d.Hs[i], d.Ws[i] = m.shape[1], m.shape[2]
    d.boxes, d.image_area, d.out = boxes.data_ptr(), float(image_area), out.data_ptr()
    d.levels_out = None if levels_out is None else _chk(levels_out, torch.int32, "levels").data_ptr()
    check(lib.dc_roi_align_pyramid_f32(C.byref(d), _stream()), "dc_roi_align_pyramid_f32")
    return out


def subsample2(x, out=None):
    lib = _lib.load()
    _chk(x, name="x")
    N, H, W, Cc = x.shape
    if out is None:
        out = torch.empty((N, (H + 1) // 2, (W + 1) // 2, Cc), dtype=torch.float32, device=x.device)
    check(lib.dc_subsample2_f32(_ptr(x), _ptr(out), N, H, W, Cc, _stream()), "dc_subsample2_f32")
    return out


def rpn_proposals(heads, anchors, image_hw, proposal_count, nms_threshold, std_dev=(0.1, 0.1, 0.2, 0.2), pre_nms_limit=6000,
                  anchors_per_loc=3, out=None, debug=False, head_stride=0):
    lib = _lib.load()
    B = heads[0].shape[0]
    d = ProposalDesc()
    d.B, d.levels, d.anchors_per_loc = B, len(heads), anchors_per_loc
    for i, h in enumerate(heads):
        if not _chk(h, name="head").is_contiguous() or h.shape[-1] != (head_stride or anchors_per_loc * 6):
            raise _lib.DcapError("rpn_proposals: heads must be contiguous [B,H,W,A*6] (or [B,H,W,head_stride])")
        d.heads[i] = h.data_ptr()
        d.Hs[i], d.Ws[i] = h.shape[1], h.shape[2]
    d.head_stride = int(head_stride)
    d.anchors, d.A_total = _chk(anchors, name="anchors").data_ptr(), anchors.shape[0]
    for i in range(4):
        d.std_dev[i] = float(std_dev[i])
    d.image_h, d.image_w = float(image_hw[0]), float(image_hw[1])
    d.pre_nms_limit, d.proposal_count, d.nms_threshold = int(pre_nms_limit), int(proposal_count), float(nms_threshold)
    dev = heads[0].device
    if out is None:
        out = torch.empty((B, proposal_count, 4), dtype=torch.float32, device=dev)
    d.proposals = out.data_ptr()
    extra = None
    if debug:
        k = min(pre_nms_limit, anchors.shape[0])
        extra = (torch.empty((B, anchors.shape[0]), dtype=torch.float32, device=dev),
                 torch.empty((B, k), dtype=torch.int32, device=dev),
                 torch.empty((B, proposal_count), dtype=torch.int32, device=dev))
        d.scores_out, d.order_out, d.keep_out = (t.data_ptr() for t in extra)
    ws, wsb = WORKSPACE.get(lib.dc_proposals_workspace_bytes(C.byref(d)), dev)
    check(lib.dc_proposals_f32(C.byref(d), _ptr(ws), wsb, _stream()), "dc_proposals_f32")
    return (out, extra) if debug else out


def _rec_masks(rec_masks, B, U):
    if rec_masks is None:
        return None
    if tuple(_chk(rec_masks, name="rec_masks").shape) != (4, B, U) or not rec_masks.is_contiguous():
        raise _lib.DcapError("rec_masks must be a contiguous float32 [4,B,U] tensor")
    return rec_masks.data_ptr()


def lstm_seq_fwd(z, U_rec, mask, B, T, h_seq=None, c_seq=None, rec_masks=None):
    lib = _lib.load()
    U = U_rec.shape[0]
    _chk(z, name="z"), _chk(U_rec, name="U_rec")
    if not z.is_contiguous() or not U_rec.is_contiguous() or tuple(z.shape) != (T * B, 4 * U):
        raise _lib.DcapError("lstm_seq_fwd: z must be contiguous [T*B,4U], U_rec contiguous [U,4U]")
    if h_seq is None:
        h_seq = torch.empty((T * B, U), dtype=torch.float32, device=z.device)
    if c_seq is None:
        c_seq = torch.empty((T * B, U), dtype=torch.float32, device=z.device)
    d = LstmFwdDesc()
    d.B, d.T, d.U = B, T, U
    d.z, d.U_rec = z.data_ptr(), U_rec.data_ptr()
    d.mask = None if mask is None else _chk(mask, torch.uint8, "mask").data_ptr()
    d.h_seq, d.c_seq = h_seq.data_ptr(), c_seq.data_ptr()
    d.rec_masks = _rec_masks(rec_masks, B, U)
    ws, wsb = WORKSPACE.get(lib.dc_lstm_seq_workspace_bytes(B, T, U), z.device)
    check(lib.dc_lstm_seq_fwd_f32(C.byref(d), _ptr(ws), wsb, _stream()), "dc_lstm_seq_fwd_f32")
    return h_seq, c_seq


def lstm_pack_urec(U_rec, out=None):
    _chk(U_rec, name="U_rec")
    lib = _lib.load()
    U = U_rec.shape[0]
    if not U_rec.is_contiguous() or tuple(U_rec.shape) != (U, 4 * U):
        raise _lib.DcapError("lstm_pack_urec: U_rec must be contiguous [U,4U]")
    if out is None:
        out = torch.empty((U, 4 * U), dtype=torch.float32, device=U_rec.device)
    if not _chk(out, name="out").is_contiguous() or out.numel() != 4 * U * U:
        raise _lib.DcapError("lstm_pack_urec: out must be a contiguous tensor of 4*U*U floats")
    check(lib.dc_lstm_pack_urec_f32(_ptr(U_rec), U, _ptr(out), _stream()), "dc_lstm_pack_urec_f32")
    return out


def lstm_step(z, U_rec, h_prev=None, c_prev=None, mask=None, h=None, c=None, U_packed=None):
    _chk(z, name="z"), _chk(U_rec, name="U_rec")
    lib = _lib.load()
    U = U_rec.shape[0]
    B = z.shape[0]
    if not z.is_contiguous() or not U_rec.is_contiguous() or tuple(z.shape) != (B, 4 * U) or tuple(U_rec.shape) != (U, 4 * U):
        raise _lib.DcapError("lstm_step: z must be contiguous [B,4U], U_rec contiguous [U,4U]")
    if (h_prev is None) != (c_prev is None):
        raise _lib.DcapError("lstm_step: h_prev and c_prev are both given or both None")
    h = torch.empty((B, U), dtype=torch.float32, device=z.device) if h is None else h
    c = torch.empty((B, U), dtype=torch.float32, device=z.device) if c is None else c
    for name, t in (("h_prev", h_prev), ("c_prev", c_prev), ("h", h), ("c", c)):
        if t is not None and (not _chk(t, name=name).is_contiguous() or tuple(t.shape) != (B, U)):
            raise _lib.DcapError("lstm_step: %s must be contiguous [B,U]" % name)
    if mask is not None and (not _chk(mask, torch.uint8, "mask").is_contiguous() or mask.numel() != B):
        raise _lib.DcapError("lstm_step: mask must be a contiguous uint8 [B] tensor")
    if U_packed is not None and (not _chk(U_packed, name="U_packed").is_contiguous() or U_packed.numel() != 4 * U * U):
        raise _lib.DcapError("lstm_step: U_packed must be lstm_pack_urec's contiguous 4*U*U floats")
    if B == 0:
        return h, c
    d = LstmStepDesc()
    d.B, d.U = B, U
    d.z, d.U_rec, d.U_packed = z.data_ptr(), U_rec.data_ptr(), _ptr(U_packed)
    d.h_prev, d.c_prev, d.mask = _ptr(h_prev), _ptr(c_prev), _ptr(mask)
    d.h, d.c = h.data_ptr(), c.data_ptr()
    ws, wsb = WORKSPACE.get(lib.dc_lstm_step_workspace_bytes(B, U), z.device)
    check(lib.dc_lstm_step_f32(C.byref(d), _ptr(ws), wsb, _stream()), "dc_lstm_step_f32")
    return h, c


def lstm_seq_bwd(z, U_rec, mask, h_seq, c_seq, B, T, dh_seq=None, dh_last=None, dz=None, dU=None, accumulate_dU=False, rec_masks=None):
    lib = _lib.load()
    U = U_rec.shape[0]
    if dz is None:
        dz = torch.empty((T * B, 4 * U), dtype=torch.float32, device=z.device)
    if dU is None:
        dU = torch.empty((U, 4 * U), dtype=torch.float32, device=z.device)
    elif dU is False:
        dU = None
    d = LstmBwdDesc()
    d.B, d.T, d.U = B, T, U
    d.z, d.U_rec = _chk(z, name="z").data_ptr(), _chk(U_rec, name="U_rec").data_ptr()
    d.mask = None if mask is None else _chk(mask, torch.uint8, "mask").data_ptr()
    d.h_seq, d.c_seq = h_seq.data_ptr(), c_seq.data_ptr()
    for name, t in (("dh_seq", dh_seq), ("dh_last", dh_last)):
        if t is not None and not _chk(t, name=name).is_contiguous():
            raise _lib.DcapError("lstm_seq_bwd: %s must be contiguous" % name)
    d.dh_seq = None if dh_seq is None else dh_seq.data_ptr()
    d.dh_last = None if dh_last is None else dh_last.data_ptr()
    d.dz, d.dU_rec, d.accumulate_dU = dz.data_ptr(), (None if dU is None else _chk(dU, name="dU").data_ptr()), int(accumulate_dU)
    d.rec_masks = _rec_masks(rec_masks, B, U)
    ws, wsb = WORKSPACE.get(lib.dc_lstm_seq_workspace_bytes(B, T, U), z.device)
    check(lib.dc_lstm_seq_bwd_f32(C.byref(d), _ptr(ws), wsb, _stream()), "dc_lstm_seq_bwd_f32")
    return dz, dU


def softmax_ce(logits, targets=None, probs=None, loss_rows=None, dlogits=None, grad_scale=1.0, row_weights=None,
               keras_sparse=False):
    lib = _lib.load()
    _chk(logits, name="logits")
    d = SoftmaxCeDesc()
    d.M, d.V, d.ld = logits.shape[0], logits.shape[1], logits.stride(0)
    d.logits = logits.data_ptr()
    d.targets = None if targets is None else _chk(targets, torch.int32, "targets").data_ptr()
    for name, t in (("probs", probs), ("dlogits", dlogits)):
        if t is not None and (_chk(t, name=name).stride(0) != logits.stride(0)):
            raise _lib.DcapError("softmax_ce: %s must share the logits' row stride" % name)
    d.probs = None if probs is None else probs.data_ptr()
    d.loss_rows = None if loss_rows is None else _chk(loss_rows, name="loss_rows").data_ptr()
    d.dlogits = None if dlogits is None else dlogits.data_ptr()
    d.grad_scale = float(grad_scale)
    d.row_weights = None if row_weights is None else _chk(row_weights, name="row_weights").data_ptr()
    d.keras_sparse = int(keras_sparse)
    check(lib.dc_softmax_ce_f32(C.byref(d), _stream()), "dc_softmax_ce_f32")


def vocab_ce_supported(X, W):
    K, V = W.shape
    if X.dtype == BF16:
        return W.dtype == BF16 and K % 8 == 0 and V % 8 == 0 and X.stride(0) % 8 == 0 and W.stride(0) % 8 == 0
    return K % 32 == 0 and V % 4 == 0 and V >= 4 and X.stride(0) % 4 == 0 and W.stride(0) % 4 == 0


def vocab_ce(X, W, bias, targets, loss_rows=None, dlogits=None, dbias=None, grad_scale=1.0, row_weights=None, keras_sparse=False,
             materialize_bf16=None):
    lib = _lib.load()
    bf = X.dtype == BF16
    _chk(X, BF16 if bf else torch.float32, "X"), _chk(W, BF16 if bf else torch.float32, "W")
    M, K = X.shape
    if W.shape[0] != K:
        raise _lib.DcapError("vocab_ce: inner dimensions differ (%d vs %d)" % (K, W.shape[0]))
    d = VocabCeDesc()
    d.M, d.V, d.K, d.bf16 = M, W.shape[1], K, int(bf)
    d.X, d.ldx, d.W, d.ldw = X.data_ptr(), X.stride(0), W.data_ptr(), W.stride(0)
    d.bias = None if bias is None else _chk(bias, name="bias").data_ptr()
    d.targets = _chk(targets, torch.int32, "targets").data_ptr()
    d.row_weights = None if row_weights is None else _chk(row_weights, name="row_weights").data_ptr()
    d.grad_scale, d.keras_sparse = float(grad_scale), int(keras_sparse)
    d.loss_rows = None if loss_rows is None else _chk(loss_rows, name="loss_rows").data_ptr()
    if dlogits is not None:
        if dlogits.dtype not in (torch.float32, BF16) or not dlogits.is_cuda or dlogits.stride(1) != 1 or dlogits.shape[0] != M:
            raise _lib.DcapError("vocab_ce: dlogits must be a float32 or bf16 device matrix with M rows")
        d.dlogits, d.lddl, d.dl_bf16 = dlogits.data_ptr(), dlogits.stride(0), int(dlogits.dtype == BF16)
    d.dbias = None if dbias is None else _chk(dbias, name="dbias").data_ptr()
    if materialize_bf16 is None:
        materialize_bf16 = os.environ.get("DCAP_VOCAB_MATERIALIZE", "1") != "0"
    d.materialize_bf16 = int(bool(materialize_bf16) and bf and dlogits is not None and dlogits.dtype == BF16)
    ws, wsb = WORKSPACE.get(lib.dc_vocab_ce_workspace_bytes(C.byref(d)), X.device)
    check(lib.dc_vocab_ce(C.byref(d), _ptr(ws), wsb, _stream()), "dc_vocab_ce")


def _row_out(t, M, dtype, name):
    if t is None:
        return None, 1
    if not t.is_cuda or t.dtype != dtype or t.dim() != 1 or t.shape[0] != M or (M > 1 and t.stride(0) < 1):
        raise _lib.DcapError("vocab_top1: %s must be a %s device vector of %d elements" % (name, dtype, M))
    return C.c_void_p(t.data_ptr()), max(1, t.stride(0))


def _vocab_operands(X, W, bias):
    M, K = X.shape
    V = W.shape[1]
    q = 8 if W.dtype == BF16 else 4
    Vp = (V + q - 1) // q * q
    esz = W.element_size()
    w_ok = (W.stride(0) % q == 0 and W.stride(0) >= Vp and W.data_ptr() % 16 == 0 and
            (W.storage_offset() + (K - 1) * W.stride(0) + Vp) * esz <= W.untyped_storage().nbytes())
    if not w_ok:
        Wp = torch.zeros((K, Vp), dtype=W.dtype, device=W.device)
        Wp[:, :V].copy_(W)
        W = Wp
    if X.stride(0) % q or X.data_ptr() % 16:
        X = torch.empty((M, K), dtype=X.dtype, device=X.device).copy_(X)
    if bias is not None and (bias.data_ptr() % 16 or not bias.is_contiguous()):
        bias = torch.empty((V,), dtype=torch.float32, device=bias.device).copy_(bias)
    return X, W, bias


def _vocab_args(fn, X, W, bias, tile=None):
    bf = X.dtype == BF16 or W.dtype == BF16
    dt = BF16 if bf else torch.float32
    _chk(X, dt, "X"), _chk(W, dt, "W")
    if bias is not None:
        _chk(bias, name="bias")
    lib = _lib.load()
    M, K = X.shape
    V = W.shape[1]
    if W.shape[0] != K:
        raise _lib.DcapError("%s: inner dimensions differ (%d vs %d)" % (fn, K, W.shape[0]))
    if K % (8 if bf else 32):
        raise _lib.DcapError("%s: K must be a multiple of %d, got %d" % (fn, 8 if bf else 32, K))
    if bias is not None and tuple(bias.shape) != (V,):
        raise _lib.DcapError("%s: bias must be [V]" % fn)
    if tile and not bf:
        raise _lib.DcapError("%s: tile= chooses between the bf16 kernels; float32 operands have one tile shape" % fn)
    return lib, M, K, V, bf


def vocab_topk_bf16_tile(M, V, K):
    return int(_lib.load().dc_vocab_topk_bf16_tile(int(M), int(V), int(K)))


def vocab_top1(X, W, bias=None, tokens=None, ids=None, probs=None, mask=None, tile=None):
    lib, M, K, V, bf = _vocab_args("vocab_top1", X, W, bias, tile)
    if tokens is None:
        tokens = torch.empty((M,), dtype=torch.int32, device=X.device)
    if not _chk(tokens, torch.int32, "tokens").is_contiguous() or tokens.numel() != M:
        raise _lib.DcapError("vocab_top1: tokens must be a contiguous int32 [M] tensor")
    if mask is not None and (not _chk(mask, torch.uint8, "mask").is_contiguous() or mask.numel() != M):
        raise _lib.DcapError("vocab_top1: mask must be a contiguous uint8 [M] tensor")
    ids_p, ld_ids = _row_out(ids, M, torch.int32, "ids")
    probs_p, ld_probs = _row_out(probs, M, torch.float32, "probs")
    if M == 0:
        return tokens
    X, W, bias = _vocab_operands(X, W, bias)
    d = VocabTop1Bf16Desc() if bf else VocabTop1Desc()
    d.M, d.V, d.K = M, V, K
    d.X, d.ldx, d.W, d.ldw = X.data_ptr(), X.stride(0), W.data_ptr(), W.stride(0)
    d.bias = _ptr(bias)
    d.tokens = tokens.data_ptr()
    d.ids, d.ld_ids, d.probs, d.ld_probs = ids_p, ld_ids, probs_p, ld_probs
    d.mask = _ptr(mask)
    if bf:
        d.tile = int(tile or 0)
        ws, wsb = WORKSPACE.get(lib.dc_vocab_top1_bf16_workspace_bytes(M, V, K, d.tile), X.device)
        check(lib.dc_vocab_top1_bf16(C.byref(d), _ptr(ws), wsb, _stream()), "dc_vocab_top1_bf16")
        return tokens
    ws, wsb = WORKSPACE.get(lib.dc_vocab_top1_workspace_bytes(M, V), X.device)
    check(lib.dc_vocab_top1_f32(C.byref(d), _ptr(ws), wsb, _stream()), "dc_vocab_top1_f32")
    return tokens


TOPK_MAX = 8


def vocab_topk(X, W, bias, k, ids=None, probs=None, tile=None):
    lib, M, K, V, bf = _vocab_args("vocab_topk", X, W, bias, tile)
    k = int(k)
    if not 1 <= k <= TOPK_MAX or V < k:
        raise _lib.DcapError("vocab_topk: need 1 <= k <= %d and V >= k, got k = %d, V = %d" % (TOPK_MAX, k, V))
    if ids is None:
        ids = torch.empty((M, k), dtype=torch.int32, device=X.device)
    if probs is None:
        probs = torch.empty((M, k), dtype=torch.float32, device=X.device)
    for name, t, dt in (("ids", ids, torch.int32), ("probs", probs, torch.float32)):
        if not _chk(t, dt, name).is_contiguous() or tuple(t.shape) != (M, k):
            raise _lib.DcapError("vocab_topk: %s must be a contiguous %s [M,k] tensor" % (name, dt))
    if M == 0:
        return ids, probs
    X, W, bias = _vocab_operands(X, W, bias)
    d = VocabTopkBf16Desc() if bf else VocabTopkDesc()
    d.M, d.V, d.K, d.k = M, V, K, k
    d.X, d.ldx, d.W, d.ldw = X.data_ptr(), X.stride(0), W.data_ptr(), W.stride(0)
    d.bias = _ptr(bias)
    d.ids, d.probs = ids.data_ptr(), probs.data_ptr()
    if bf:
        d.tile = int(tile or 0)
# ... 353 lines not shown
```

### image-captioning_amd/pipeline.py

```python
import os

import torch


class CaptionTrainPipeline(object):
    def __init__(self, plan, decoder, rois_per_image):
        self.plan, self.dec = plan, decoder
        dev = plan.device
        self.s_enc = torch.cuda.Stream(device=dev)
        self.s_dec = torch.cuda.Stream(device=dev)
        B = plan.B
        self.fc = fc = getattr(plan, "feat_channels", 256)
        self.feat = [torch.empty((B, rois_per_image, 7, 7, fc), dtype=torch.float32, device=dev) for _ in range(2)]
        self.ev_feat = [torch.cuda.Event() for _ in range(2)]
        self.ev_free = [torch.cuda.Event() for _ in range(2)]
        self.pending = None
        self.n = 0
        self.late_wait = os.environ.get("DCAP_PIPE_LATE_WAIT", "1") != "0"
        self._hold = []
        self.max_in_flight = 4
        cur = torch.cuda.current_stream(dev)
        self.s_enc.wait_stream(cur)
        self.s_dec.wait_stream(cur)

    def _encode(self, slot, images, boxes):
        with torch.cuda.stream(self.s_enc):
            if self.n >= 2 and not self.late_wait:
                self.s_enc.wait_event(self.ev_free[slot])
            self.plan.forward(images)
            if self.n >= 2 and self.late_wait:
                self.s_enc.wait_event(self.ev_free[slot])
            self.plan.roi_features(boxes_norm=boxes, out=self.feat[slot])
            self.ev_feat[slot].record(self.s_enc)

    def _decode(self, slot, tables):
        with torch.cuda.stream(self.s_dec):
            self.s_dec.wait_event(self.ev_feat[slot])
            f = self.feat[slot]
            loss = self.dec.train_step(f.view(-1, 7, 7, self.fc), tables)
            self.ev_free[slot].record(self.s_dec)
            for h in self._hold:
                if h[0] is tables and h[2] is None:
                    h[2] = torch.cuda.Event()
                    h[2].record(self.s_dec)
                    break
        return loss

    def _release(self):
        hold = self._hold
        while hold and hold[0][2] is not None and hold[0][2].query():
            hold.pop(0)
        while len(hold) > self.max_in_flight and hold[0][2] is not None:
            hold[0][2].synchronize()
            hold.pop(0)

    def step(self, images, boxes, tables):
        slot = self.n & 1
        self._release()
        self._hold.append([tables, (images, boxes), None])
        self._encode(slot, images, boxes)
        loss = None
        if self.pending is not None:
            loss = self._decode(*self.pending)
        self.pending = (slot, tables)
        self.n += 1
        return loss

    def flush(self):
        loss = None
        if self.pending is not None:
            loss = self._decode(*self.pending)
            self.pending = None
        cur = torch.cuda.current_stream(self.plan.device)
        cur.wait_stream(self.s_enc)
        cur.wait_stream(self.s_dec)
        return loss


class JointTrainPipeline(object):

    def __init__(self, model):
        inner = getattr(model, "inner_model", model)
        if inner.backbone_from is not None:
            raise ValueError("JointTrainPipeline: ResNet stages are trainable (backbone_from = %r): the backbone pass of the next batch depends on "
                             "this batch's update" % (inner.backbone_from,))
        self.model, self.inner = model, inner
        self.plans = inner.plan_pair()
        dev = inner.device
        self.s_trunk = torch.cuda.Stream(device=dev)
        self.s_copy = torch.cuda.Stream(device=dev)
        self.ev_trunk = [torch.cuda.Event(), torch.cuda.Event()]
        self.pending = None
        self.n = 0
        self._hold = []
        inner.use_step_graph = False

    def _trunk(self, j, images):
        dev = self.inner.device
        cur = torch.cuda.current_stream(dev)
        u8 = self.inner._images_u8(images)
        if not u8.is_cuda:
            with torch.cuda.stream(self.s_copy):
                u8 = u8.to(dev)
            self.s_trunk.wait_stream(self.s_copy)
            u8.record_stream(self.s_trunk)
            self._hold.append(u8)
        self.s_trunk.wait_stream(cur)
        with torch.cuda.stream(self.s_trunk):
            self.plans[j].forward_trunk(u8)
            self.ev_trunk[j].record(self.s_trunk)

    def _rest(self, inputs, j):
        torch.cuda.current_stream(self.inner.device).wait_event(self.ev_trunk[j])
        self.inner.use_plan(j)
        losses = self.inner.train_on_batch_device(inputs, trunk_done=True)
        return self.model.mean_over_towers(losses) if self.model is not self.inner else losses

    def step(self, inputs):
        j = self.n & 1
        if self.model is not self.inner:
            inputs = self.model.shard_inputs(inputs)
        self._hold = self._hold[-4:] + [inputs[0]]
        self._trunk(j, inputs[0])
        losses = None
        if self.pending is not None:
            losses = self._rest(*self.pending)
        self.pending = (inputs, j)
        self.n += 1
        return losses

    def flush(self):
        losses = None
        if self.pending is not None:
            losses = self._rest(*self.pending)
            self.pending = None
        torch.cuda.current_stream(self.inner.device).wait_stream(self.s_trunk)
        return losses
```

### include/dcap.h

```cpp
#ifndef DCAP_H
#define DCAP_H

#include <stddef.h>
#include <stdint.h>

#ifdef __cplusplus
extern "C" {
#endif

#define DC_OK            0
#define DC_EINVAL       -1
#define DC_EALIGN       -2
#define DC_EWORKSPACE   -3
#define DC_ELAUNCH      -4

#define DC_ABI_VERSION 600
int         dc_version(void);
const char* dc_last_error(void);

typedef struct {
    int M, N, K;
    const float*   A;  int lda;  int a_trans;
    const int32_t* a_gather;
    const float*   B;  int ldb;  int b_trans;
    float*         C;  int ldc;
    const float*   scale;
    const float*   shift;
    const float*   residual;  int ldr;
    int res_rows;
    int relu;
    int accumulate;
    int split_k;
} dc_gemm_desc;

size_t dc_gemm_workspace_bytes(const dc_gemm_desc* d);
int    dc_gemm_f32(const dc_gemm_desc* d, void* workspace, size_t workspace_bytes, void* stream);

typedef struct {
    int M, N, K;
    const uint16_t* A;  int lda;  int a_trans;
    const int32_t*  a_gather;  int a_gather_rows;
    const uint16_t* B;  int ldb;  int b_trans;
    float*          C;  int ldc;
    uint16_t*       Cb; int ldcb;
    const float*    scale;
    const float*    shift;
    const float*    residual;  int ldr;
    int res_rows;
    int relu;
    int accumulate;
    int split_k;
} dc_gemm_bf16_desc;

size_t dc_gemm_bf16_workspace_bytes(const dc_gemm_bf16_desc* d);
int    dc_gemm_bf16(const dc_gemm_bf16_desc* d, void* workspace, size_t workspace_bytes, void* stream);
int    dc_gemm_bf16_tile(const dc_gemm_bf16_desc* d, int* split_k);

typedef struct {
    int N, H, W, Cin;
    int Cout, kh, kw, stride, pad_t, pad_l;
    int Ho, Wo;
    const uint16_t* x;
    const uint16_t* dy;
    float* dw;
    int accumulate;
    int split_k;
} dc_conv_wgrad_bf16_desc;
size_t dc_conv2d_wgrad_bf16_workspace_bytes(const dc_conv_wgrad_bf16_desc* d);
int    dc_conv2d_wgrad_bf16(const dc_conv_wgrad_bf16_desc* d, void* workspace, size_t workspace_bytes, void* stream);
int    dc_conv2d_wgrad_bf16_tile(const dc_conv_wgrad_bf16_desc* d, int* split_k);

typedef struct {
    int N, H, W, Cin;
    int Cout, kh, kw, stride, pad_t, pad_l;
    int Ho, Wo;
    const uint16_t* x;
    const uint16_t* w;
    float*          y;
    uint16_t*       y_bf16;
    const float* scale;
    const float* shift;
    const float* residual;  int res_mode;
    int relu;
    int split_k;
    int tile;
} dc_conv_bf16_desc;
size_t dc_conv2d_bf16_workspace_bytes(const dc_conv_bf16_desc* d);
int    dc_conv2d_bf16(const dc_conv_bf16_desc* d, void* workspace, size_t workspace_bytes, void* stream);
int    dc_conv2d_bf16_tile(const dc_conv_bf16_desc* d, int* split_k);

int dc_cast_f32_bf16(const float* x, uint16_t* out, size_t n, void* stream);
int dc_cast_bf16_f32(const uint16_t* x, float* out, size_t n, void* stream);
int dc_cast_f32_bf16_2d(const float* x, int ld_in, uint16_t* out, int ld_out, int rows, int cols, int cols_out, void* stream);

#define DC_MATH_F32 0
#define DC_MATH_BF16X3 1
#define DC_MATH_BF16X2 2
#define DC_MATH_BF16 3
typedef struct {
    int N, H, W, Cin;
    int Cout, kh, kw, stride, pad_t, pad_l;
    int Ho, Wo;
    const float* x;
    const float* w;
    float*       y;
    const float* scale;
    const float* shift;
    const float* residual;  int res_mode;
    int relu;
    int split_k;
    int accumulate;
    int math;
    const float* w_wino;
    const uint16_t* w_wino_b3;
} dc_conv_desc;

int dc_split_bf16x3_f32(const float* x, uint16_t* out, size_t n, void* stream);
size_t dc_conv2d_workspace_bytes(const dc_conv_desc* d);
int    dc_conv2d_nhwc_f32(const dc_conv_desc* d, void* workspace, size_t workspace_bytes, void* stream);

int    dc_conv2d_tile_config(const dc_conv_desc* d, int* bm, int* bn, int* split_k);
int    dc_conv2d_kernel_name(const dc_conv_desc* d, char* buf, size_t buf_bytes);
int    dc_conv2d_is_pointwise(const dc_conv_desc* d);
size_t dc_conv2d_winograd_weight_bytes(int Cin, int Cout);
int    dc_conv2d_winograd_pack_f32(const float* w, float* u, int Cin, int Cout, void* stream);
size_t dc_conv2d_winograd_b3_weight_bytes(int Cin, int Cout);
int    dc_conv2d_winograd_pack_b3(const float* w, uint16_t* u, int Cin, int Cout, void* stream);
typedef struct {
    int M, K1, N1, N2;
    const float* x;
    const float* w1;
    const float* scale1;
    const float* shift1;
    const float* residual;
    int relu1;
    float* y;
    const float* w2;
    const float* scale2;
    const float* shift2;
    int relu2;
    float* z;
    const uint16_t* w1_b3;
    const uint16_t* w2_b3;
} dc_pw_chain_desc;
int dc_pw_chain_supported(int K1, int N1, int N2);
int dc_pw_chain_pack_f32(const float* w, float* out, int N, int K, void* stream);
int dc_pw_chain_pack_b3(const float* w, uint16_t* out, int N, int K, void* stream);
int dc_pw_chain_f32(const dc_pw_chain_desc* d, void* stream);
int dc_pw_chain_kernel_name(const dc_pw_chain_desc* d, char* buf, size_t buf_bytes);

int    dc_set_persistent_cus(int n);
int    dc_get_persistent_cus(void);

size_t dc_conv2d_wgrad_workspace_bytes(const dc_conv_desc* d);
int    dc_conv2d_wgrad_f32(const dc_conv_desc* d, void* workspace, size_t workspace_bytes, void* stream);

int dc_maxpool3x3s2_same_f32(const float* x, float* y, int N, int H, int W, int C, void* stream);

int dc_maxpool2x2s2_f32(const float* x, float* y, int N, int H, int W, int C, void* stream);

int dc_mold_image_rgbx_f32(const uint8_t* img, float* out, int N, int H, int W,
                           float mean_r, float mean_g, float mean_b, void* stream);
int dc_mold_image_padded_f32(const uint8_t* img, float* out, int N, int H, int W, int channels,
                             float mean_r, float mean_g, float mean_b, void* stream);

typedef struct {
    int B, R, C, pool;
    const float* maps[4];
    int Hs[4], Ws[4];
    const float* boxes;
    float image_area;
    float* out;
    int32_t* levels_out;
} dc_roialign_desc;

int dc_roi_align_pyramid_f32(const dc_roialign_desc* d, void* stream);

int dc_subsample2_f32(const float* x, float* y, int N, int H, int W, int C, void* stream);

typedef struct {
    int B, levels, anchors_per_loc;
    const float* heads[5];
    int Hs[5], Ws[5];
    int head_stride;
    const float* anchors;
    int A_total;
    float std_dev[4];
    float image_h, image_w;
    int pre_nms_limit, proposal_count;
    float nms_threshold;
    float* proposals;
    float* scores_out;
    int32_t* order_out;
    int32_t* keep_out;
} dc_proposal_desc;

size_t dc_proposals_workspace_bytes(const dc_proposal_desc* d);
int    dc_proposals_f32(const dc_proposal_desc* d, void* workspace, size_t workspace_bytes, void* stream);

int dc_roi_align_pyramid_bwd_f32(const dc_roialign_desc* d, void* stream);

int dc_downsample2x_sum_f32(const float* fine, float* out, int N, int Ho, int Wo, int C, int accumulate, void* stream);
int dc_downsample2x_sum_dual_f32(const float* fine, float* out, uint16_t* out_bf16, int N, int Ho, int Wo, int C, int accumulate, void* stream);

typedef struct {
    int B, T, U;
    float* z;
    const float* U_rec;
    const uint8_t* mask;
    float* h_seq;
    float* c_seq;
    const float* rec_masks;
} dc_lstm_fwd_desc;

size_t dc_lstm_seq_workspace_bytes(int B, int T, int U);
int    dc_lstm_seq_fwd_f32(const dc_lstm_fwd_desc* d, void* workspace, size_t workspace_bytes, void* stream);

typedef struct {
    int B, T, U;
    const float* z;
    const float* U_rec;
    const uint8_t* mask;
    const float* h_seq;
    const float* c_seq;
    const float* dh_seq;
    const float* dh_last;
    float* dz;
    float* dU_rec;
    int accumulate_dU;
    const float* rec_masks;
} dc_lstm_bwd_desc;

int dc_lstm_seq_bwd_f32(const dc_lstm_bwd_desc* d, void* workspace, size_t workspace_bytes, void* stream);

typedef struct {
    int B, U;
    float* z;
    const float* U_rec;
    const float* U_packed;
    const float* h_prev;
    const float* c_prev;
    const uint8_t* mask;
    float* h;
    float* c;
} dc_lstm_step_desc;

int    dc_lstm_pack_urec_f32(const float* U_rec, int U, float* U_packed, void* stream);
size_t dc_lstm_step_workspace_bytes(int B, int U);
int    dc_lstm_step_f32(const dc_lstm_step_desc* d, void* workspace, size_t workspace_bytes, void* stream);

typedef struct {
    int M, V, ld;
    const float* logits;
    const int32_t* targets;
    float* probs;
    float* loss_rows;
    float* dlogits;
    float grad_scale;
    const float* row_weights;
    int keras_sparse;
} dc_softmax_ce_desc;

int dc_softmax_ce_f32(const dc_softmax_ce_desc* d, void* stream);

typedef struct {
    int M, V, K;
    int bf16;
    const void* X;  int ldx;
    const void* W;  int ldw;
    const float* bias;
    const int32_t* targets;
    const float* row_weights;
    float grad_scale;
    int keras_sparse;
    float* loss_rows;
    void* dlogits;  int lddl;  int dl_bf16;
    float* dbias;
    int materialize_bf16;
} dc_vocab_ce_desc;

size_t dc_vocab_ce_workspace_bytes(const dc_vocab_ce_desc* d);
int    dc_vocab_ce(const dc_vocab_ce_desc* d, void* workspace, size_t workspace_bytes, void* stream);

typedef struct {
    int M, V, K;
    const float* X;  int ldx;
    const float* W;  int ldw;
    const float* bias;
    int32_t* tokens;
    int32_t* ids;    int ld_ids;
    float* probs;    int ld_probs;
    uint8_t* mask;
} dc_vocab_top1_desc;

size_t dc_vocab_top1_workspace_bytes(int M, int V);
int    dc_vocab_top1_f32(const dc_vocab_top1_desc* d, void* workspace, size_t workspace_bytes, void* stream);

typedef struct {
    int M, V, K, k;
    const float* X;  int ldx;
    const float* W;  int ldw;
    const float* bias;
    int32_t* ids;
    float* probs;
} dc_vocab_topk_desc;

size_t dc_vocab_topk_workspace_bytes(int M, int V, int k);
int    dc_vocab_topk_f32(const dc_vocab_topk_desc* d, void* workspace, size_t workspace_bytes, void* stream);

typedef struct {
    int M, V, K;
    const void* X;   int ldx;
    const void* W;   int ldw;
    const float* bias;
    int32_t* tokens;
    int32_t* ids;    int ld_ids;
    float* probs;    int ld_probs;
    uint8_t* mask;
    int tile;
} dc_vocab_top1_bf16_desc;

typedef struct {
    int M, V, K, k;
    const void* X;   int ldx;
    const void* W;   int ldw;
    const float* bias;
    int32_t* ids;
    float* probs;
    int tile;
} dc_vocab_topk_bf16_desc;

int    dc_vocab_topk_bf16_tile(int M, int V, int K);
size_t dc_vocab_top1_bf16_workspace_bytes(int M, int V, int K, int tile);
size_t dc_vocab_topk_bf16_workspace_bytes(int M, int V, int K, int k, int tile);
int    dc_vocab_top1_bf16(const dc_vocab_top1_bf16_desc* d, void* workspace, size_t workspace_bytes, void* stream);
int    dc_vocab_topk_bf16(const dc_vocab_topk_bf16_desc* d, void* workspace, size_t workspace_bytes, void* stream);

typedef struct {
    int R, k, nb, steps, j, log_score;
    const int32_t* cand_ids;
    const float* cand_probs;
    const float* scores_in;
    float* scores_out;
    int32_t* parents;
    int32_t* tokens_hist;
    int32_t* tokens;
    uint8_t* mask;
    int U;
    const float* h_in;
    const float* c_in;
    float* h_out;
    float* c_out;
} dc_beam_select_desc;

int    dc_beam_select_f32(const dc_beam_select_desc* d, void* stream);
int    dc_beam_backtrace(const int32_t* parents, const int32_t* tokens_hist, int steps, int R, int k, int32_t* seq, void* stream);

int dc_argmax_rows_f32(const float* x, int M, int V, int ld, int32_t* out, void* stream);

int dc_gather_rows_f32(const float* src, int ld_src, const int32_t* idx, float* out, int ld_out,
                       int n_rows, int width, void* stream);

typedef struct {
    int M, N, ld;
    const float* acc;
    const float* bias; const float* gamma; const float* beta; const float* mean; const float* var;
    float eps;
    float* y;
    const float* dy;
    float* dacc;
    float* dgamma; float* dbeta; float* dbias;
} dc_bn_relu_desc;

int dc_bn_relu_fwd_f32(const dc_bn_relu_desc* d, void* stream);
int dc_bn_relu_bwd_f32(const dc_bn_relu_desc* d, void* stream);

int dc_conv_weight_dgrad_pack_f32(const float* w, float* out, int Cout, int kh, int kw, int Cin, void* stream);
typedef struct {
    int levels, anchors_per_loc, head_stride;
    const float* heads[5];
    float*       dheads[5];
    int Hs[5], Ws[5];
    int n_sel, n_pos;
    const int32_t* sel_level;
    const int32_t* sel_index;
    const int32_t* sel_match;
    const float*   target_deltas;
    float* losses;
    const int32_t* counts_dev;
} dc_rpn_loss_desc;
int dc_rpn_loss_grad_f32(const dc_rpn_loss_desc* d, void* stream);
int dc_scatter2_add_f32(const float* coarse, float* fine, int N, int Hc, int Wc, int C, void* stream);
typedef struct {
    int n_proposals, n_gt, n_rois, T;
    const float*   proposals;
    const float*   gt_boxes;
    const int32_t* gt_captions;
    int   max_positive;
    float inv_ratio;
    int   shuffle;
    uint32_t seed, offset;
    const uint32_t* offset_dev;
    float*   rois;
    int32_t* captions;
    int32_t* counts;
} dc_detection_targets_desc;
int dc_detection_targets_f32(const dc_detection_targets_desc* d, void* stream);
int dc_caption_tables_i32(const int32_t* captions, int B, int T, int32_t* ids_tm, uint8_t* mask, int32_t* targets_tm, float* row_weights,
                          int32_t* live_count, void* stream);
size_t dc_l2_reg_workspace_bytes(size_t n);
int dc_l2_reg_f32(const float* w, const float* coef, const float* mask, float* grad, size_t n, float* loss, void* workspace,
                  size_t workspace_bytes, void* stream);

int dc_axpy_f32(float a, const float* x, float* y, size_t n, void* stream);

int dc_relu_bwd_f32(const float* dy, const float* y, float* out, int M, int N, int ld, void* stream);
int dc_relu_bwd_dual_f32(const float* dy, const float* y, float* out, uint16_t* out_bf16, size_t n, void* stream);

int dc_fold_time_f32(const float* x, int T, int B, int N, int ld, float* out, int ld_out, void* stream);

size_t dc_colsum_workspace_bytes(int M, int N, int ld);
int dc_colsum_f32(const float* x, int M, int N, int ld, float* out, int accumulate, void* workspace, size_t workspace_bytes,
                  void* stream);

size_t dc_sumsq_workspace_bytes(size_t n);
int dc_sumsq_f32(const float* x, size_t n, float* out, int accumulate, void* workspace, size_t workspace_bytes, void* stream);

int dc_dropout_mask_f32(float* out, size_t n, float rate, uint32_t seed, uint32_t offset, const uint32_t* offset_dev, void* stream);

int dc_bn_fold_f32(const float* gamma, const float* beta, const float* bias, const float* mean, const float* var, float eps,
                   float* scale, float* shift, int n, void* stream);
int dc_bn_bwd_f32(const float* dz, const float* a, const float* b, const float* gamma, const float* beta, const float* scale,
                  float* dacc, float* dzn, long rows, int channels, void* stream);
int dc_mul_f32(const float* a, const float* b, float* out, size_t n, void* stream);
int dc_maxpool3x3s2_same_bwd_f32(const float* x, const float* y, const float* dy, float* dx, int N, int H, int W, int C, void* stream);

int dc_zero_fill(void* p, size_t bytes, void* stream);

int dc_mean_f32(const float* x, size_t n, float* out, void* stream);

typedef struct {
    const int32_t* start;
    const float* coef;
    const float* mask;
    int nseg;
} dc_reg_segments;

typedef struct {
    size_t n;
    float* p;
    const float* g;
    float* m;
    float* v;
    float* vhat;
    float lr_t, beta1, beta2, eps;
    float grad_scale;
    const float* gnorm_sq;
    float clipnorm;
    uint16_t* p_bf16;
    size_t n_bf16;
    const float* lr_t_dev;
    const dc_reg_segments* reg;
} dc_amsgrad_desc;

int dc_amsgrad_step_f32(const dc_amsgrad_desc* d, void* stream);

size_t dc_reg_sumsq_workspace_bytes(size_t n);
int dc_reg_sumsq_f32(const float* w, const float* g, const dc_reg_segments* reg, size_t n, float* loss, float* gnorm_sq, void* workspace,
                     size_t workspace_bytes, void* stream);

#ifdef __cplusplus
}
#endif
#endif
```

Before: 11530 captions/s.

## Compute FPN output convs only on tile groups touched by RoI samples

Adds a kernel that marks which Winograd tile groups of each pyramid level are sampled by RoIAlign bins, compacts them into per-level lists, and a list-driven Winograd kernel that computes the 3x3 FPN output conv only on those groups. The pipeline's encoder then runs a sparse forward (laterals plus RoI-driven convs) before RoIAlign instead of the full FPN. This avoids computing P2-P5 output features that are never read, which matters with only 32 RoIs per image. The cost is an extra marking/compaction kernel, a device-side count that drives a fixed-size grid, and reliance on the RoIs being known before the convs run.

After: 12510 captions/s (median of 6 runs). +8.5%, better.

```diff
diff --git a/image-captioning_amd/_lib.py b/image-captioning_amd/_lib.py
--- a/image-captioning_amd/_lib.py
+++ b/image-captioning_amd/_lib.py
@@ -66,6 +66,12 @@
                 ("maps", C.c_void_p * 4), ("Hs", C.c_int * 4), ("Ws", C.c_int * 4),
                 ("boxes", C.c_void_p), ("image_area", C.c_float),
                 ("out", C.c_void_p), ("levels_out", C.c_void_p)]
+
+
+class RoiGroupsDesc(C.Structure):
+    _fields_ = [("B", C.c_int), ("R", C.c_int), ("pool", C.c_int), ("Hs", C.c_int * 4), ("Ws", C.c_int * 4),
+                ("boxes", C.c_void_p), ("image_area", C.c_float),
+                ("marks", C.c_void_p), ("lists", C.c_void_p * 4), ("counts", C.c_void_p)]
 
 
 class LstmFwdDesc(C.Structure):
@@ -225,6 +231,9 @@
     "dc_mold_image_rgbx_f32": (C.c_int, [C.c_void_p, C.c_void_p, C.c_int, C.c_int, C.c_int,
                                          C.c_float, C.c_float, C.c_float, C.c_void_p]),
     "dc_roi_align_pyramid_f32": (C.c_int, [C.POINTER(RoiAlignDesc), C.c_void_p]),
+    "dc_roi_tile_groups": (C.c_int, [C.POINTER(RoiGroupsDesc), C.c_void_p]),
+    "dc_conv2d_winograd_group_count": (C.c_int, [C.c_int, C.c_int]),
+    "dc_conv2d_winograd_groups_f32": (C.c_int, [C.POINTER(ConvDesc), C.c_void_p, C.c_void_p, C.c_void_p]),
     "dc_subsample2_f32": (C.c_int, [C.c_void_p, C.c_void_p, C.c_int, C.c_int, C.c_int, C.c_int, C.c_void_p]),
     "dc_proposals_workspace_bytes": (C.c_size_t, [C.POINTER(ProposalDesc)]),
     "dc_proposals_f32": (C.c_int, [C.POINTER(ProposalDesc), C.c_void_p, C.c_size_t, C.c_void_p]),
diff --git a/image-captioning_amd/csrc/conv_wino.hip b/image-captioning_amd/csrc/conv_wino.hip
--- a/image-captioning_amd/csrc/conv_wino.hip
+++ b/image-captioning_amd/csrc/conv_wino.hip
@@ -15,6 +15,8 @@
     int N, H, W, Cin, Cout, relu;
     int gy, gx, groups;
     unsigned x_bytes, u_bytes;
+    const int* glist;
+    const int* gcount;
 };
 
 __global__ void wino_pack_kernel(const float* __restrict__ w, float* __restrict__ u, int Cin, int Cout) {
@@ -97,7 +99,7 @@
 __device__ __forceinline__ int patch_swizzle(int y, int x) { return ((x >> 2) & 1) | (((y >> 1) & 3) << 1); }
 template <int HALVES>
 struct Cfg {
-    static constexpr int NT = 256 * HALVES, TGY = 4 * HALVES, TGX = 8, PH = 2 * TGY + 2, NPIX = PH * PW, SLOTS = NPIX * 8;
+    static constexpr int NT = 256 * HALVES, TGY = kWinoTGY * HALVES, TGX = kWinoTGX, PH = 2 * TGY + 2, NPIX = PH * PW, SLOTS = NPIX * 8;
     static constexpr int BUF = 32768 * HALVES;
     static constexpr int LDS_BYTES = 2 * BUF;
     static_assert(NDMA * NT >= SLOTS && NDMA * NT * 16 <= BUF, "patch buffer; the kernel issues the pieces three per step");
@@ -120,9 +122,10 @@
     return __builtin_amdgcn_mfma_f32_32x32x16_bf16(__builtin_bit_cast(bf16x8, a), __builtin_bit_cast(bf16x8, b), c, 0, 0, 0);
 }
 
-template <int HALVES, bool B3, int NCH = 1>
+template <int HALVES, bool B3, int NCH = 1, bool LIST = false>
 __device__ __forceinline__ void wino_body(const Args& a) {
     static_assert(NCH == 1 || (NCH == 2 && HALVES == 1 && B3), "64-channel items: the split-bf16 32-tile kernel only");
+    static_assert(!LIST || (HALVES == 1 && B3), "list-driven item walk: the split-bf16 32-tile kernel only");
     using namespace wp;
     typedef Cfg<HALVES> C;
     constexpr int NT64 = C::NT, SLOTS = C::SLOTS, BUF = C::BUF;
@@ -132,7 +135,9 @@
     const int wa = wave & 3, th = wave >> 2;
     const int gpi = a.gy * a.gx;
     const int NTG = a.Cout >> 5, KC = a.Cin >> 4, KP = a.Cin >> 5;
-    const int total = a.groups * (NTG / NCH);
+    int groups = a.groups;
+    if constexpr (LIST) groups = min(max(*a.gcount, 0), a.groups);
+    const int total = groups * (NTG / NCH);
     const __amdgpu_buffer_rsrc_t rsrc = __builtin_amdgcn_make_buffer_rsrc(const_cast<float*>(a.x), 0, (int)a.x_bytes, 0x00020000);
 
     int nb, img, gyi, gxi;
@@ -141,8 +146,9 @@
     unsigned ubyte3;
     auto setup = [&](int item) {
         const int bid = xcd_remap(item, total);
-        nb = bid / a.groups;
-        const int g = bid - nb * a.groups;
+        nb = bid / groups;
+        int g = bid - nb * groups;
+        if constexpr (LIST) g = min(max(a.glist[g], 0), a.groups - 1);
         img = g / gpi;
         const int gr = g - img * gpi;
         gyi = gr / a.gx;
@@ -486,6 +492,10 @@
 __global__ __launch_bounds__(256, 2) void wino32b_kernel(Args a) { wino_body<1, true, NCH>(a); }
 template __global__ void wino32b_kernel<1>(Args);
 template __global__ void wino32b_kernel<2>(Args);
+template <int NCH>
+__global__ __launch_bounds__(256, 2) void wino32b_list_kernel(Args a) { wino_body<1, true, NCH, true>(a); }
+template __global__ void wino32b_list_kernel<1>(Args);
+template __global__ void wino32b_list_kernel<2>(Args);
 
 }
 
@@ -539,24 +549,31 @@
     return items >= 2 * kNumCU ? 64 : 32;
 }
 
-int conv2d_winograd(const dc_conv_desc* d, hipStream_t s) {
-    wino::Args a;
+static int wino_args(const dc_conv_desc* d, bool b3, bool big, wino::Args& a) {
     a.x = d->x;
-    const bool b3 = wino_b3(d);
     a.u = b3 ? reinterpret_cast<const f4*>(d->w_wino_b3) : reinterpret_cast<const f4*>(d->w_wino);
     a.y = d->y;
     a.scale = d->scale;
     a.shift = d->shift;
     a.N = d->N; a.H = d->H; a.W = d->W; a.Cin = d->Cin; a.Cout = d->Cout; a.relu = d->relu;
-    const int th = (d->H + 1) / 2, tw = (d->W + 1) / 2;
     const size_t x_bytes = (size_t)d->N * d->H * d->W * d->Cin * sizeof(float);
     DC_REQUIRE(x_bytes < (1ull << 31), DC_EINVAL, "dc_conv2d (winograd): the input tensor has %zu bytes, the kernel addresses < 2 GiB", x_bytes);
     a.x_bytes = (unsigned)x_bytes;
     a.u_bytes = (unsigned)((size_t)16 * d->Cin * d->Cout * (b3 ? 6 : 4));
+    a.gy = big ? (wino_groups_y(d->H) + 1) / 2 : wino_groups_y(d->H);
+    a.gx = wino_groups_x(d->W);
+    a.groups = d->N * a.gy * a.gx;
+    a.glist = nullptr;
+    a.gcount = nullptr;
+    return DC_OK;
+}
+
+int conv2d_winograd(const dc_conv_desc* d, hipStream_t s) {
+    wino::Args a;
+    const bool b3 = wino_b3(d);
     const bool big = conv_winograd_tiles(d) == 64;
-    a.gy = (th + (big ? 8 : 4) - 1) / (big ? 8 : 4);
-    a.gx = (tw + 7) / 8;
-    a.groups = d->N * a.gy * a.gx;
+    const int rc = wino_args(d, b3, big, a);
+    if (rc) return rc;
     const bool wide = b3 && !big && conv_winograd_cout(d) == 64;
     const long items = (long)a.groups * (d->Cout / (wide ? 64 : 32));
     DC_REQUIRE(items < (1l << 31), DC_EINVAL, "dc_conv2d (winograd): grid too large");
@@ -583,9 +600,44 @@
     return check_launch("dc_conv2d (winograd)");
 }
 
+int conv2d_winograd_groups(const dc_conv_desc* d, const int* glist, const int* gcount, hipStream_t s) {
+    wino::Args a;
+    const int rc = wino_args(d, true, false, a);
+    if (rc) return rc;
+    a.glist = glist;
+    a.gcount = gcount;
+    const bool wide = wino_cout_force() == 64 && d->Cout % 64 == 0;
+    const long items = (long)a.groups * (d->Cout / (wide ? 64 : 32));
+    DC_REQUIRE(items < (1l << 31), DC_EINVAL, "dc_conv2d_winograd_groups: grid too large");
+    const long full = 2L * kNumCU;
+    const unsigned grid = items >= full ? (unsigned)full : (unsigned)std::max<long>(8, items / 8 * 8);
+    if (wide) {
+        DC_ENSURE_DYN_LDS((&wino::wino32b_list_kernel<2>), wino::wp::Cfg<1>::LDS_BYTES);
+        hipLaunchKernelGGL((wino::wino32b_list_kernel<2>), dim3(grid), dim3(wino::wp::Cfg<1>::NT), wino::wp::Cfg<1>::LDS_BYTES, s, a);
+    } else {
+        DC_ENSURE_DYN_LDS((&wino::wino32b_list_kernel<1>), wino::wp::Cfg<1>::LDS_BYTES);
+        hipLaunchKernelGGL((wino::wino32b_list_kernel<1>), dim3(grid), dim3(wino::wp::Cfg<1>::NT), wino::wp::Cfg<1>::LDS_BYTES, s, a);
+    }
+    return check_launch("dc_conv2d_winograd_groups_f32");
+}
+
 }
 
 using namespace dcap;
+
+extern "C" int dc_conv2d_winograd_groups_f32(const dc_conv_desc* d, const int32_t* groups, const int32_t* count, void* stream) {
+    DC_REQUIRE(d && d->x && d->y && groups && count, DC_EINVAL, "dc_conv2d_winograd_groups: null pointer");
+    DC_REQUIRE(d->N > 0 && d->H > 0 && d->W > 0, DC_EINVAL, "dc_conv2d_winograd_groups: bad N/H/W");
+    DC_REQUIRE(wino_b3(d), DC_EINVAL,
+               "dc_conv2d_winograd_groups: the layer must be one the split-bf16 Winograd kernel takes (3x3, stride 1, pad 1, Cin and Cout "
+               "multiples of 32, no residual, fp32 math, w_wino_b3 given, 16-byte aligned operands, input below 2 GiB)");
+    return conv2d_winograd_groups(d, groups, count, static_cast<hipStream_t>(stream));
+}
+
+extern "C" int dc_conv2d_winograd_group_count(int H, int W) {
+    if (H <= 0 || W <= 0) return 0;
+    return wino_groups_y(H) * wino_groups_x(W);
+}
 
 extern "C" size_t dc_conv2d_winograd_weight_bytes(int Cin, int Cout) {
     if (Cin <= 0 || Cout <= 0 || Cin % 32 || Cout % 32) return 0;
diff --git a/image-captioning_amd/csrc/dcap_internal.h b/image-captioning_amd/csrc/dcap_internal.h
--- a/image-captioning_amd/csrc/dcap_internal.h
+++ b/image-captioning_amd/csrc/dcap_internal.h
@@ -55,6 +55,11 @@
     return (xcd < r ? xcd * (q + 1) : r * (q + 1) + (xcd - r) * q) + bid / kNumXCD;
 }
 
+constexpr int kWinoTGY = 4, kWinoTGX = 8;
+constexpr int kWinoGroupH = 2 * kWinoTGY, kWinoGroupW = 2 * kWinoTGX;
+inline int wino_groups_y(int H) { return ((H + 1) / 2 + kWinoTGY - 1) / kWinoTGY; }
+inline int wino_groups_x(int W) { return ((W + 1) / 2 + kWinoTGX - 1) / kWinoTGX; }
+
 static __global__ __launch_bounds__(256) void zero_fill_kernel(unsigned* __restrict__ p, size_t words) {
     for (size_t i = (size_t)blockIdx.x * 256 + threadIdx.x; i < words; i += (size_t)gridDim.x * 256) p[i] = 0u;
 }
diff --git a/image-captioning_amd/csrc/roialign.hip b/image-captioning_amd/csrc/roialign.hip
--- a/image-captioning_amd/csrc/roialign.hip
+++ b/image-captioning_amd/csrc/roialign.hip
@@ -19,6 +19,31 @@
     if (!(lvl > -100.f)) return 2;
     const int r = (int)rintf(lvl);
     return min(5, max(2, 4 + r));
+}
+
+__device__ __forceinline__ float roi_sample(float lo, float hi, int p, int n, int pool) {
+    if (pool > 1) {
+        const float step = div_rn(mul_rn(sub_rn(hi, lo), (float)(n - 1)), (float)(pool - 1));
+        return add_rn(mul_rn(lo, (float)(n - 1)), mul_rn((float)p, step));
+    }
+    return mul_rn(mul_rn(0.5f, add_rn(lo, hi)), (float)(n - 1));
+}
+
+struct RoiBin {
+    float in_y, in_x;
+    bool ok;
+    int top, bot, left, right;
+};
+__device__ __forceinline__ RoiBin roi_bin(const float4& bx, int py, int px, int H, int W, int pool) {
+    RoiBin r;
+    r.in_y = roi_sample(bx.x, bx.z, py, H, pool);
+    r.in_x = roi_sample(bx.y, bx.w, px, W, pool);
+    r.ok = (r.in_y >= 0.f) && (r.in_y <= (float)(H - 1)) && (r.in_x >= 0.f) && (r.in_x <= (float)(W - 1));
+    r.top = (int)floorf(r.in_y);
+    r.bot = (int)ceilf(r.in_y);
+    r.left = (int)floorf(r.in_x);
+    r.right = (int)ceilf(r.in_x);
+    return r;
 }
 
 __global__ __launch_bounds__(256) void roi_align_kernel(dc_roialign_desc d) {
@@ -36,19 +61,13 @@
     const float* fm = d.maps[li] + (long)(box / d.R) * H * W * d.C;
     float4* out = reinterpret_cast<float4*>(d.out) + (long)wave * C4;
 
-    const float hs = (d.pool > 1) ? div_rn(mul_rn(sub_rn(bx.z, bx.x), (float)(H - 1)), (float)(d.pool - 1)) : 0.f;
-    const float ws = (d.pool > 1) ? div_rn(mul_rn(sub_rn(bx.w, bx.y), (float)(W - 1)), (float)(d.pool - 1)) : 0.f;
-    const float in_y = (d.pool > 1) ? add_rn(mul_rn(bx.x, (float)(H - 1)), mul_rn((float)py, hs))
-                                    : mul_rn(mul_rn(0.5f, add_rn(bx.x, bx.z)), (float)(H - 1));
-    const float in_x = (d.pool > 1) ? add_rn(mul_rn(bx.y, (float)(W - 1)), mul_rn((float)px, ws))
-                                    : mul_rn(mul_rn(0.5f, add_rn(bx.y, bx.w)), (float)(W - 1));
-    const bool ok = (in_y >= 0.f) && (in_y <= (float)(H - 1)) && (in_x >= 0.f) && (in_x <= (float)(W - 1));
-    if (!ok) {
+    const RoiBin sb = roi_bin(bx, py, px, H, W, d.pool);
+    if (!sb.ok) {
         for (int c = lane; c < C4; c += 64) out[c] = make_float4(0.f, 0.f, 0.f, 0.f);
         return;
     }
-    const int top = (int)floorf(in_y), bot = (int)ceilf(in_y), left = (int)floorf(in_x), right = (int)ceilf(in_x);
-    const float ly = in_y - (float)top, lx = in_x - (float)left;
+    const int top = sb.top, bot = sb.bot, left = sb.left, right = sb.right;
+    const float ly = sb.in_y - (float)top, lx = sb.in_x - (float)left;
     const float4* tl = reinterpret_cast<const float4*>(fm + ((long)top * W + left) * d.C);
     const float4* tr = reinterpret_cast<const float4*>(fm + ((long)top * W + right) * d.C);
     const float4* bl = reinterpret_cast<const float4*>(fm + ((long)bot * W + left) * d.C);
@@ -65,14 +84,6 @@
         DC_LERP(x) DC_LERP(y) DC_LERP(z) DC_LERP(w)
         out[c] = o;
     }
-}
-
-__device__ __forceinline__ float roi_sample(float lo, float hi, int p, int n, int pool) {
-    if (pool > 1) {
-        const float step = div_rn(mul_rn(sub_rn(hi, lo), (float)(n - 1)), (float)(pool - 1));
-        return add_rn(mul_rn(lo, (float)(n - 1)), mul_rn((float)p, step));
-    }
-    return mul_rn(mul_rn(0.5f, add_rn(lo, hi)), (float)(n - 1));
 }
 
 constexpr int RA_MAX_POOL = 16;
@@ -163,9 +174,97 @@
         }
 }
 
+constexpr int RG_THREADS = 1024, RG_WAVES = RG_THREADS / 64, RG_LDS_MARKS = 8192;
+struct RoiGroupsArgs {
+    dc_roi_groups_desc d;
+    int gy[4], gx[4], off[5];
+};
+
+__global__ __launch_bounds__(RG_THREADS) void roi_tile_groups_kernel(RoiGroupsArgs a) {
+    const dc_roi_groups_desc& d = a.d;
+    const int tid = threadIdx.x, lane = tid & 63, wave = tid >> 6;
+    __shared__ int lds_marks[RG_LDS_MARKS];
+    __shared__ int wsum[4][RG_WAVES];
+    const int nmarks = a.off[4];
+    int* marks = nmarks <= RG_LDS_MARKS ? lds_marks : d.marks;
+    for (int i = tid; i < nmarks; i += RG_THREADS) marks[i] = 0;
+    __syncthreads();
+    const int bins = d.pool * d.pool, samples = d.B * d.R * bins;
+    for (int s = tid; s < samples; s += RG_THREADS) {
+        const int box = s / bins, bin = s - box * bins;
+        const int py = bin / d.pool, px = bin - py * d.pool;
+        const float4 bx = reinterpret_cast<const float4*>(d.boxes)[box];
+        const int li = roi_level(bx.x, bx.y, bx.z, bx.w, d.image_area) - 2;
+        const RoiBin sb = roi_bin(bx, py, px, d.Hs[li], d.Ws[li], d.pool);
+        if (!sb.ok) continue;
+        int* m = marks + a.off[li] + (box / d.R) * a.gy[li] * a.gx[li];
+        const int gt = sb.top / kWinoGroupH * a.gx[li], gb = sb.bot / kWinoGroupH * a.gx[li];
+        const int gl = sb.left / kWinoGroupW, gr = sb.right / kWinoGroupW;
+        m[gt + gl] = 1;
+        m[gt + gr] = 1;
+        m[gb + gl] = 1;
+        m[gb + gr] = 1;
+    }
+    __syncthreads();
+    int below[4] = {0, 0, 0, 0};
+    for (int c0 = 0; c0 < nmarks; c0 += RG_THREADS) {
+        const int i = c0 + tid;
+        const bool on = i < nmarks && marks[i] != 0;
+        const int l = i >= a.off[3] ? 3 : (i >= a.off[2] ? 2 : (i >= a.off[1] ? 1 : 0));
+        const int first = l == 3 ? a.off[3] : (l == 2 ? a.off[2] : (l == 1 ? a.off[1] : 0));
+        const unsigned long long b = __ballot(on);
+        const unsigned long long b1 = __ballot(on && i < a.off[1]), b2 = __ballot(on && i < a.off[2]), b3 = __ballot(on && i < a.off[3]);
+        if (lane == 0) {
+            wsum[0][wave] = __popcll(b);
+            wsum[1][wave] = __popcll(b1);
+            wsum[2][wave] = __popcll(b2);
+            wsum[3][wave] = __popcll(b3);
+        }
+        __syncthreads();
+        int before = 0, add[4] = {0, 0, 0, 0};
+#pragma unroll
+        for (int w = 0; w < RG_WAVES; ++w) {
+            before += w < wave ? wsum[0][w] : 0;
+#pragma unroll
+            for (int k = 0; k < 4; ++k) add[k] += wsum[k][w];
+        }
+        const int rank = below[0] + before + __popcll(b & ((1ull << lane) - 1ull));
+        const int lower = l == 3 ? below[3] + add[3] : (l == 2 ? below[2] + add[2] : (l == 1 ? below[1] + add[1] : 0));
+        if (on) d.lists[l][rank - lower] = i - first;
+#pragma unroll
+        for (int k = 0; k < 4; ++k) below[k] += add[k];
+        __syncthreads();
+    }
+    if (tid < 4) {
+        const int lo = tid == 3 ? below[3] : (tid == 2 ? below[2] : (tid == 1 ? below[1] : 0));
+        const int hi = tid == 3 ? below[0] : (tid == 2 ? below[3] : (tid == 1 ? below[2] : below[1]));
+        d.counts[tid] = hi - lo;
+    }
+}
+
 }
 
 using namespace dcap;
+
+extern "C" int dc_roi_tile_groups(const dc_roi_groups_desc* d, void* stream) {
+    DC_REQUIRE(d && d->boxes && d->marks && d->counts, DC_EINVAL, "dc_roi_tile_groups: null pointer");
+    DC_REQUIRE(d->B > 0 && d->R > 0 && d->pool > 0, DC_EINVAL, "dc_roi_tile_groups: bad B/R/pool");
+    DC_REQUIRE(aligned16(d->boxes), DC_EALIGN, "dc_roi_tile_groups: boxes not 16-byte aligned");
+    RoiGroupsArgs a;
+    a.d = *d;
+    long off = 0;
+    for (int l = 0; l < 4; ++l) {
+        DC_REQUIRE(d->lists[l] && d->Hs[l] > 0 && d->Ws[l] > 0, DC_EINVAL, "dc_roi_tile_groups: bad level %d", l);
+        a.gy[l] = wino_groups_y(d->Hs[l]);
+        a.gx[l] = wino_groups_x(d->Ws[l]);
+        a.off[l] = (int)off;
+        off += (long)d->B * a.gy[l] * a.gx[l];
+    }
+    a.off[4] = (int)off;
+    DC_REQUIRE(off < (1l << 30) && (long)d->B * d->R * d->pool * d->pool < (1l << 30), DC_EINVAL, "dc_roi_tile_groups: too many groups / samples");
+    hipLaunchKernelGGL(roi_tile_groups_kernel, dim3(1), dim3(RG_THREADS), 0, static_cast<hipStream_t>(stream), a);
+    return check_launch("roi_tile_groups_kernel");
+}
 
 extern "C" int dc_roi_align_pyramid_bwd_f32(const dc_roialign_desc* d, void* stream) {
     DC_REQUIRE(d && d->boxes && d->out, DC_EINVAL, "dc_roi_align_pyramid_bwd: null pointer");
diff --git a/image-captioning_amd/encoder.py b/image-captioning_amd/encoder.py
--- a/image-captioning_amd/encoder.py
+++ b/image-captioning_amd/encoder.py
@@ -302,12 +302,19 @@
         P2, P3 = self._buf(H // 4, W // 4, 256), self._buf(H // 8, W // 8, 256)
         P4, P5 = self._buf(H // 16, W // 16, 256), self._buf(H // 32, W // 32, 256)
         rp = self.rpn is not None
+        self._n_lateral = len(self._ops)
         self._conv("fpn_p2", t2, P2, relu=False, bf16=rp)
         self._conv("fpn_p3", t3, P3, relu=False, bf16=rp)
         self._conv("fpn_p4", t4, P4, relu=False, bf16=rp)
         self._conv("fpn_p5", t5, P5, relu=False, bf16=rp)
         self.P = (P2, P3, P4, P5)
         self.pre = (t2, t3, t4, t5)
+        pops = self._ops[self._n_lateral:]
+        self.sparse_rois = (self.rpn is None and not self.fast_bf16 and not self.train_stages and not self._external_bn and len(pops) == 4 and
+                            all(op[0] == "conv" and op[2] == "fpn_p%d" % (2 + i) and op[2] not in self._external and op[1].w_wino_b3
+                                for i, op in enumerate(pops)))
+        self._roi_groups = None
+        self._roi_boxes = {}
         if self.rpn is not None:
             from .utils import generate_pyramid_anchors
             P6 = self._buf(H // 64, W // 64, 256)
@@ -465,6 +472,37 @@
             cs = self._steps[part] = step_graph.CapturedStep()
         cs.run(body, warm_calls=1, propagate=True)
 
+    def _run_rois(self, boxes):
+        g = ops.roi_tile_groups(boxes, self._roi_groups, float(self.H * self.W), 7)
+        stream = C.c_void_p(torch.cuda.current_stream().cuda_stream)
+        for l, op in enumerate(self._ops[self._n_lateral:]):
+            rc = self.lib.dc_conv2d_winograd_groups_f32(C.byref(op[1]), C.c_void_p(g.lists[l].data_ptr()), g.count_ptr(l), stream)
+            if rc:
+                check(rc, "dc_conv2d_winograd_groups_f32(%s)" % op[2])
+
+    def forward_rois(self, images_u8, boxes_norm, out=None, before_align=None):
+        if not self.sparse_rois:
+            self.forward(images_u8)
+            if before_align is not None:
+                before_align()
+            return self.roi_features(boxes_norm=boxes_norm.to(self.device, torch.float32).contiguous(), out=out)
+        if images_u8 is not None:
+            self.images.copy_(images_u8, non_blocking=bool(images_u8.is_cuda or images_u8.is_pinned()))
+        B, R = int(boxes_norm.shape[0]), int(boxes_norm.shape[1])
+        if B != self.B or tuple(boxes_norm.shape[2:]) != (4,):
+            raise ValueError("forward_rois: boxes must be [%d,R,4], got %s" % (self.B, tuple(boxes_norm.shape)))
+        if self._roi_groups is None:
+            self._roi_groups = ops.RoiTileGroups(self.B, [(p.shape[1], p.shape[2]) for p in self.P], self.device)
+        boxes = self._roi_boxes.get(R)
+        if boxes is None:
+            boxes = self._roi_boxes[R] = torch.zeros((self.B, R, 4), dtype=torch.float32, device=self.device)
+        boxes.copy_(boxes_norm, non_blocking=bool(boxes_norm.is_cuda or boxes_norm.is_pinned()))
+        self._run_part("lat", lambda: self._run_ops(0, self._n_lateral))
+        self._run_part("rois%d" % R, lambda: self._run_rois(boxes))
+        if before_align is not None:
+            before_align()
+        return ops.roi_align_pyramid(list(self.P), boxes, float(self.H * self.W), 7, out=out)
+
     def forward_trunk(self, images_u8=None):
         if self._external_bn:
             raise RuntimeError("forward_trunk: this plan folds trainable BatchNorm layers inside the backbone pass; use forward()")
@@ -555,6 +593,7 @@
         self.C = (x,)
         self.P = (x, x, x, x)
         self.pre = None
+        self.sparse_rois = False
         self._ws = torch.empty(max(self._ws_bytes, 16), dtype=torch.uint8, device=self.device)
 
     def _run_ops(self):
diff --git a/image-captioning_amd/modified_dense_model.py b/image-captioning_amd/modified_dense_model.py
--- a/image-captioning_amd/modified_dense_model.py
+++ b/image-captioning_amd/modified_dense_model.py
@@ -96,10 +96,12 @@
                                            self.config.MEAN_PIXEL, rpn=self._rpn_config(), math=self.conv_math)
         return self._plans[key]
 
-    def extract_features(self, images_u8, rois_px=None):
+    def extract_features(self, images_u8, rois_px=None, sparse=False):
         imgs = torch.as_tensor(images_u8)
         B, H, W, _ = imgs.shape
         p = self.plan(B, H, W)
+        if sparse and not self.use_generated_rois and p.sparse_rois:
+            return p.forward_rois(imgs, p.normalize_boxes(rois_px))
         p.forward(imgs)
         if self.use_generated_rois:
             self.last_proposals = p.proposals()
@@ -122,7 +124,7 @@
         assert len(images) == self.config.BATCH_SIZE, "len(images) must be equal to BATCH_SIZE"
         molded, metas, windows = self.mold_inputs(images)
         rois = None if self.use_generated_rois else np.asarray(rois, np.float32)
-        feats = self.extract_features(molded, rois)
+        feats = self.extract_features(molded, rois, sparse=True)
         feats = feats.clone() if device_features else feats.cpu().numpy()
         n = self.config.POST_NMS_ROIS_INFERENCE
         results = [{"features": feats[i][:n]} for i in range(len(images))]
diff --git a/image-captioning_amd/ops.py b/image-captioning_amd/ops.py
--- a/image-captioning_amd/ops.py
+++ b/image-captioning_amd/ops.py
@@ -7,7 +7,7 @@
 import torch
 
 from . import _lib
-from ._lib import (PwChainDesc, ConvBf16Desc, AmsgradDesc, DetectionTargetsDesc, BnReluDesc, ConvDesc, ConvWgradBf16Desc, GemmBf16Desc, VocabCeDesc, ProposalDesc, RpnLossDesc, GemmDesc, LstmBwdDesc, LstmFwdDesc, RoiAlignDesc,
+from ._lib import (PwChainDesc, ConvBf16Desc, AmsgradDesc, DetectionTargetsDesc, BnReluDesc, ConvDesc, ConvWgradBf16Desc, GemmBf16Desc, VocabCeDesc, ProposalDesc, RpnLossDesc, GemmDesc, LstmBwdDesc, LstmFwdDesc, RoiAlignDesc, RoiGroupsDesc,
                    SoftmaxCeDesc, VocabTop1Desc, VocabTopkDesc, VocabTop1Bf16Desc, VocabTopkBf16Desc, BeamSelectDesc, LstmStepDesc, check)
 
 
@@ -509,6 +509,63 @@
     return out
 
 
+class RoiTileGroups(object):
+
+    def __init__(self, B, hw, device):
+        lib = _lib.load()
+        self.B, self.hw = int(B), [(int(h), int(w)) for h, w in hw]
+        if len(self.hw) != 4:
+            raise _lib.DcapError("RoiTileGroups: four pyramid levels expected")
+        self.per_image = [lib.dc_conv2d_winograd_group_count(h, w) for h, w in self.hw]
+        self.lists = [torch.zeros(self.B * n, dtype=torch.int32, device=device) for n in self.per_image]
+        self.counts = torch.zeros(4, dtype=torch.int32, device=device)
+        self.marks = torch.zeros(self.B * sum(self.per_image), dtype=torch.int32, device=device)
+
+    def count_ptr(self, level):
+        return C.c_void_p(self.counts.data_ptr() + 4 * level)
+
+
+def roi_tile_groups(boxes, groups, image_area, pool=7):
+    lib = _lib.load()
+    _chk(boxes, name="boxes")
+    B, R, _ = boxes.shape
+    if not boxes.is_contiguous() or B != groups.B:
+        raise _lib.DcapError("roi_tile_groups: boxes must be contiguous [B,R,4] with the B the group buffers were made for")
+    d = RoiGroupsDesc()
+    d.B, d.R, d.pool = B, R, pool
+    for i, (h, w) in enumerate(groups.hw):
+        d.Hs[i], d.Ws[i] = h, w
+        d.lists[i] = groups.lists[i].data_ptr()
+    d.boxes, d.image_area = boxes.data_ptr(), float(image_area)
+    d.marks, d.counts = groups.marks.data_ptr(), groups.counts.data_ptr()
+    check(lib.dc_roi_tile_groups(C.byref(d), _stream()), "dc_roi_tile_groups")
+    return groups
+
+
+def conv2d_winograd_groups(x, w_packed, w_wino_b3, group_list, count, out, scale=None, shift=None, relu=False):
+    lib = _lib.load()
+    _chk(x, name="x"), _chk(w_packed, name="w"), _chk(out, name="out")
+    _chk(group_list, torch.int32, "group_list"), _chk(count, torch.int32, "count")
+    N, H, W, Cin = x.shape
+    Cout = w_packed.shape[0]
+    if not x.is_contiguous() or not out.is_contiguous() or tuple(out.shape) != (N, H, W, Cout):
+        raise _lib.DcapError("conv2d_winograd_groups: x and out must be contiguous [N,H,W,C]")
+    if not w_wino_b3.is_contiguous() or w_wino_b3.numel() != 48 * Cin * Cout:
+        raise _lib.DcapError("conv2d_winograd_groups: w_wino_b3 must be the contiguous winograd_pack_b3() of this layer's kernel")
+    if group_list.numel() < N * lib.dc_conv2d_winograd_group_count(H, W) or count.numel() < 1:
+        raise _lib.DcapError("conv2d_winograd_groups: the list must have room for every tile group of the layer")
+    d = ConvDesc()
+    d.N, d.H, d.W, d.Cin = N, H, W, Cin
+    d.Cout, d.kh, d.kw, d.stride, d.pad_t, d.pad_l, d.Ho, d.Wo = Cout, 3, 3, 1, 1, 1, H, W
+    d.x, d.w, d.y = x.data_ptr(), w_packed.data_ptr(), out.data_ptr()
+    d.scale = None if scale is None else scale.data_ptr()
+    d.shift = None if shift is None else shift.data_ptr()
+    d.relu = int(relu)
+    d.w_wino_b3 = _chk(w_wino_b3, torch.int16, "w_wino_b3").data_ptr()
+    check(lib.dc_conv2d_winograd_groups_f32(C.byref(d), _ptr(group_list), _ptr(count), _stream()), "dc_conv2d_winograd_groups_f32")
+    return out
+
+
 def subsample2(x, out=None):
     lib = _lib.load()
     _chk(x, name="x")
diff --git a/image-captioning_amd/pipeline.py b/image-captioning_amd/pipeline.py
--- a/image-captioning_amd/pipeline.py
+++ b/image-captioning_amd/pipeline.py
@@ -17,6 +17,7 @@
         self.pending = None
         self.n = 0
         self.late_wait = os.environ.get("DCAP_PIPE_LATE_WAIT", "1") != "0"
+        self.sparse_fpn = os.environ.get("DCAP_SPARSE_FPN", "1") != "0" and bool(getattr(plan, "sparse_rois", False))
         self._hold = []
         self.max_in_flight = 4
         cur = torch.cuda.current_stream(dev)
@@ -27,6 +28,11 @@
         with torch.cuda.stream(self.s_enc):
             if self.n >= 2 and not self.late_wait:
                 self.s_enc.wait_event(self.ev_free[slot])
+            if self.sparse_fpn:
+                late = (lambda: self.s_enc.wait_event(self.ev_free[slot])) if self.n >= 2 and self.late_wait else None
+                self.plan.forward_rois(images, boxes, out=self.feat[slot], before_align=late)
+                self.ev_feat[slot].record(self.s_enc)
+                return
             self.plan.forward(images)
             if self.n >= 2 and self.late_wait:
                 self.s_enc.wait_event(self.ev_free[slot])
diff --git a/include/dcap.h b/include/dcap.h
--- a/include/dcap.h
+++ b/include/dcap.h
@@ -176,6 +176,20 @@
 
 int dc_roi_align_pyramid_f32(const dc_roialign_desc* d, void* stream);
 
+typedef struct {
+    int B, R, pool;
+    int Hs[4], Ws[4];
+    const float* boxes;
+    float image_area;
+    int32_t* marks;
+    int32_t* lists[4];
+    int32_t* counts;
+} dc_roi_groups_desc;
+
+int dc_roi_tile_groups(const dc_roi_groups_desc* d, void* stream);
+int dc_conv2d_winograd_group_count(int H, int W);
+int dc_conv2d_winograd_groups_f32(const dc_conv_desc* d, const int32_t* groups, const int32_t* count, void* stream);
+
 int dc_subsample2_f32(const float* x, float* y, int N, int H, int W, int C, void* stream);
 
 typedef struct {
```
